# Tavish9/freegaussian

Hardware: AMD Instinct MI355X
Metric: Mpixels/s fwd+bwd @ 1M Gaussians 1080p (higher is better)
Workload: dtype f32; 1 GPU; north-star cfg4: 1000000 Gaussians, 1920x1080, SH degree 3, 1 view per rank per step, view = (rank + step) mod 8 around the 8-view ring, fwd+bwd, RGB, absgrad; layout=uniform, N=1000000, P=2073600, parallelism=view-dp1

## Files before the change

freegaussian_amd/_lib.py:

```python
from __future__ import annotations

import ctypes
import os
from ctypes import c_char_p, c_double, c_float, c_int, c_int64, c_size_t, c_void_p

_HERE = os.path.dirname(os.path.abspath(__file__))
LIB_PATH = os.path.join(_HERE, "libfgraster.so")

P = c_void_p

SIGNATURES = {
    "fg_abi_version": (c_int, []),
    "fg_error_string": (c_char_p, [c_int]),
    "fg_project_fwd": (c_int, [c_int, P, P, P, P, P, c_int, c_int, c_float, c_float, c_float, c_float, c_int,
                               P, P, P, P, P, P, P]),
    "fg_project_bwd": (c_int, [c_int, P, P, P, P, P, c_int, c_int, c_float, P, P, P, P, P, P, P, P, P, P, P]),
    "fg_sh_fwd": (c_int, [c_int, c_int, c_int, P, P, P, P, P, P]),
    "fg_sh_bwd": (c_int, [c_int, c_int, c_int, P, P, P, P, P, P, P, P, P]),
    "fg_scan_workspace_bytes": (c_size_t, [c_int]),
    "fg_scan_tiles": (c_int, [c_int, P, P, P, c_size_t, P]),
    "fg_tile_bin": (c_int, [c_int, P, P, P, P, c_int, c_int, c_int, P, P, P]),
    "fg_sort_workspace_bytes": (c_size_t, [c_int64]),
    "fg_sort_pairs": (c_int, [c_int64, P, P, c_int, P, c_size_t, P]),
    "fg_tile_ranges": (c_int, [c_int64, P, c_int, P, P]),
    "fg_sort32_workspace_bytes": (c_size_t, [c_int64]),
    "fg_sort_pairs32": (c_int, [c_int64, P, P, c_int, P, c_size_t, P]),
    "fg_bin_prepare_workspace_bytes": (c_size_t, [c_int]),
    "fg_bin_prepare": (c_int, [c_int, P, P, P, P, P, P, c_size_t, P]),
    "fg_bin_prepare_rects": (c_int, [c_int, P, P, P, c_int, c_int, c_int, P, P, P, P, c_size_t, P]),
    "fg_bin_prepare_keys": (c_int, [c_int, P, P, P, P, P, P, P, c_size_t, P]),
    "fg_bin_emit_workspace_bytes": (c_size_t, [c_int64]),
    "fg_bin_emit_sort": (c_int, [c_int, c_int64, P, P, P, P, P, c_int, c_int, c_int, P, P, P, P, c_size_t, P]),
    "fg_bin_emit_sort_capacity": (c_int, [c_int, c_int64, P, P, P, P, P, c_int, c_int, c_int, P, P, P, P, c_size_t,
                                          P]),
    "fg_stbin_supported": (c_int, [c_int, c_int, c_int]),
    "fg_stbin_count_workspace_bytes": (c_size_t, [c_int, c_int, c_int]),
    "fg_stbin_count": (c_int, [c_int, P, P, c_int, c_int, P, P, P, c_size_t, P]),
    "fg_stbin_fill_workspace_bytes": (c_size_t, [c_int64]),
    "fg_stbin_fill": (c_int, [c_int, P, P, P, c_int, c_int, c_int64, P, P, P, P, P, c_size_t, c_int, P]),
    "fg_stbin_fill_jobs": (c_int, [c_int, P, P, P, c_int, c_int, c_int64, P, P, P, P, P, c_size_t, c_int, c_int, c_int, P, P,
                                   c_int, P, c_int, P, P]),
    "fg_isect_keys": (c_int, [c_int64, P, P, P, P, P]),
    "fg_densify_stats": (c_int, [c_int, P, P, c_float, P, P, P, P]),
    "fg_adam_step_multi": (c_int, [c_int, P, P]),
    "fg_adam_step": (c_int, [c_int64, P, P, P, P, c_double, c_double, c_double, c_double, c_int64, P]),
    "fg_l1_ssim_workspace_floats": (c_size_t, [c_int, c_int, c_int]),
    "fg_l1_ssim_fwd": (c_int, [c_int, c_int, c_int, P, P, P, P, c_size_t, P, P]),
    "fg_l1_ssim_bwd": (c_int, [c_int, c_int, c_int, P, P, P, P, P, P]),
    "fg_pack_splats": (c_int, [c_int, c_int, P, P, P, P, P, P]),
    "fg_raster_config_init": (None, [P]),
    "fg_raster_fwd": (c_int, [c_int, c_int, c_int, c_int, P, P, P, P, P, P, P, P]),
    "fg_raster_bwd": (c_int, [c_int, c_int, c_int, c_int, P, P, P, P, P, P, P, P, P, P]),
    "fg_raster_composite_fwd": (c_int, [c_int, c_int, c_int, c_int, P, P, P, P, c_int, P, P, P, P, P, P]),
    "fg_raster_composite_bwd": (c_int, [c_int, c_int, c_int, c_int, P, P, P, P, c_int, P, P, P, P, P, P, P, P]),
    "fg_raster_jobs_words": (c_int64, [c_int, c_int, c_int, P]),
    "fg_raster_build_jobs": (c_int, [c_int, c_int, c_int, P, P, P, c_int, P, P]),
    "fg_raster_jobs_fwd": (c_int, [c_int, c_int, c_int, c_int, P, P, P, P, P, c_int, P, P, P, P, P, P, P, c_int64, P, P, P]),
    "fg_raster_seg_ckpt_floats": (c_int64, [c_int, c_int, c_int, c_int, c_int64, P]),
    "fg_raster_jobs_bwd": (c_int, [c_int, c_int, c_int, c_int, P, P, P, P, P, c_int, P, P, P, P, P, P, P, P, P, P, P]),
    "fg_unpack_grads": (c_int, [c_int, c_int, P, P, P, P, P, P, P]),
    "fg_preprocess_fwd": (c_int, [c_int, P, P, P, P, P, c_int, c_int, c_int, c_int, P, c_int, P, P, c_int, c_int,
                                  c_float, c_float, c_float, c_float, c_int, c_int, P, P, P, P, P, P, P, P, P, P, P, P]),
    "fg_viewmat_bwd_workspace_bytes": (c_size_t, [c_int]),
    "fg_viewmat_bwd": (c_int, [c_int, c_int, P, P, P, P, P, P, P, P, c_int, c_int, c_int, c_int, c_int, P, P, c_int, c_int,
                               c_float, c_int, P, P, P, c_int, P, P, P, P, P, c_size_t, P]),
    "fg_sh_pack_fwd": (c_int, [c_int, P, P, P, c_int, c_int, c_int, c_int, P, c_int, P, c_int, P, P, P, P, P, P, P]),
    "fg_preprocess_bwd": (c_int, [c_int, P, P, P, P, P, c_int, c_int, c_int, c_int, c_int, P, P, c_int, c_int,
                                  c_float, c_int, P, P, P, c_int, P, P, P, P, P, P, P, P, P, P]),
    "fg_preprocess_raw_fwd": (c_int, [c_int, P, P, P, P, P, P, P, P, c_int, c_int, c_int, P, c_int, P, P, c_int,
                                      c_int, c_float, c_float, c_float, c_float, c_int, c_int, P, P, P, P, P, P, P,
                                      P, P, P, P, P]),
    "fg_preprocess_raw_bwd": (c_int, [c_int, P, P, P, P, P, P, P, P, c_int, c_int, c_int, c_int, P, P, c_int, c_int,
                                      c_float, c_int, P, P, P, c_int, P, P, P, P, P, P, P, P, P, P, P, P, P]),
    "fg_preprocess_bwd_factored": (c_int, [c_int, P, P, P, P, P, c_int, c_int, c_int, c_int, P, P, c_int, c_int,
                                           c_float, c_int, P, P, P, c_int, P, P, P, P, P, P, P, c_int, P, P, P]),
    "fg_sh_grad_accumulate": (c_int, [c_int, c_int, c_int, c_int, P, P, c_int64, c_int, c_float, P, P]),
    "fg_payload_compact": (c_int, [c_int, c_int, P, P, c_int64, P, P]),
    "fg_payload_expand": (c_int, [c_int, c_int, c_int, P, c_int64, c_int64, P, c_int64, P]),
    "fg_step_layout_query": (c_int, [P, P, P]),
    "fg_step_fwd": (c_int, [P, P, P, P, P, P, P]),
    "fg_step_bwd": (c_int, [P, P, P, P, P, P]),
    "fg_sh_grad_accumulate_split": (c_int, [c_int, c_int, c_int, c_int, P, P, c_int64, c_int, c_float, P, P, P]),
    "fg_preprocess_raw_bwd_factored": (c_int, [c_int, P, P, P, P, P, P, P, P, c_int, c_int, c_int, c_int, P, P, c_int, c_int,
                                               c_float, c_int, P, P, P, c_int, P, P, P, P, P, P, P, P, P, c_int, P, P, P]),
    "fg_densify_flags": (c_int, [c_int, c_int, c_float, c_float, c_float, c_float, c_float, c_float, c_float, P, P, P,
                                 P, P, P, P]),
    "fg_densify_map": (c_int, [c_int, P, P, P, P, P, c_int, c_int, c_int, c_int, P, P, P]),
    "fg_gather_rows": (c_int, [c_int64, c_int, P, P, c_int64, P, P]),
    "fg_split_children": (c_int, [c_int, c_int, P, P, P, P, P, P]),
    "fg_mask_backproject": (c_int, [c_int, P, P, P, P, c_int, c_int, P, P, c_int, c_int, P, P]),
    "fg_camera_flow": (c_int, [c_int, c_int, P, P, P, P, P, P]),
    "fg_reprojection_flow": (c_int, [c_int, c_int, P, P, P, P, c_float, P, P]),
    "fg_flow_fwd": (c_int, [c_int, P, P, P, P, P, P, P, P, P, P]),
    "fg_flow_bwd": (c_int, [c_int, P, P, P, P, P, P, P, P, P, P, P, P, P]),
    "fg_knn_workspace_bytes": (c_size_t, [c_int64]),
    "fg_knn": (c_int, [c_int64, P, c_int, P, P, P, c_size_t, P]),
}

_EXTRA = {"fg_debug_wave_reduce16": (c_int, [P, P, P]), "fg_debug_knn_grid": (c_int, [c_int64, P, c_int, P, P])}

ABI_VERSION = 10
KNN_MAX_K = 8
STBIN_LONG_SEGMENTS = 1
STBIN_TEST_SMALL_SLABS = 4
STEP_NO_FOOTPRINT_MASKS = 2
SH_JAC_FLOATS = 10
_lib = None


class FgRasterError(RuntimeError):
    pass


class RasterConfig(ctypes.Structure):

    _fields_ = [(n, ctypes.c_int32) for n in (
        "size", "ppt_fwd", "ppt_bwd", "tile_order", "bands_nx", "tail4_fwd", "tail2_fwd", "tail4_bwd", "tail2_bwd",
        "split4_fwd", "split2_fwd", "split4_bwd", "split2_bwd", "use_liveness", "seg_parts", "seg_tail", "seg_parts2",
        "seg_tail2", "debug_only_xcd", "debug_k_mod", "balance_bands", "heavy_tiles", "seg_slots", "prio_fwd", "prio_bwd",
        "heavy_wide", "seg_fine")]

    FIELDS = tuple(n for n, _ in _fields_)[1:]

    @classmethod
    def defaults(cls) -> "RasterConfig":
        cfg = cls()
        load().fg_raster_config_init(ctypes.byref(cfg))
        return cfg

    def ptr(self) -> int:
        return ctypes.addressof(self)


STEP_BUFFERS = ("radii", "means2d", "depths", "conics", "comp", "tiles", "splats", "depth_keys", "tile_rects", "tile_masks", "sh_jac",
                "tile_offsets", "list_offsets", "flatten_ids", "jobs", "live", "seg_ckpt", "v_splats", "render", "alphas",
                "last_ids", "clamp_mask", "count_ws", "fill_ws")
STEP_BUFFER = {n: i for i, n in enumerate(STEP_BUFFERS)}


class StepDesc(ctypes.Structure):

    _fields_ = [(n, ctypes.c_int32) for n in (
        "size", "N", "width", "height", "tile_size", "raw", "sh_degree", "k_stored", "n_color", "with_depth", "n_extra",
        "antialiased", "n_clamp", "want_backward", "list_shares", "flags")] + [
        (n, ctypes.c_float) for n in ("eps2d", "near_plane", "far_plane", "radius_clip")] + [("capacity", ctypes.c_int64)]


class StepIO(ctypes.Structure):

    _fields_ = [(n, ctypes.c_void_p) for n in (
        "means", "quats", "d_quats", "scales", "d_scales", "opacities", "colors", "features_rest", "extra", "viewmat", "K",
        "background", "count_out", "v_render", "v_alphas", "v_depths", "v_conics", "v_means", "v_quats", "v_d_quats",
        "v_scales", "v_d_scales", "v_opacities", "v_colors", "v_features_rest", "v_extra", "v_rgb")] + [
        ("v_rgb_floats", ctypes.c_int32), ("ev_raster_begin", ctypes.c_void_p), ("ev_raster_end", ctypes.c_void_p),
        ("ckpt_need_out", ctypes.c_void_p)]


class StepLayout(ctypes.Structure):

    _fields_ = [("keep_bytes", ctypes.c_int64), ("tmp_bytes", ctypes.c_int64),
                ("offset", ctypes.c_int64 * len(STEP_BUFFERS)), ("nbytes", ctypes.c_int64 * len(STEP_BUFFERS)),
                ("jobs_words", ctypes.c_int64), ("seg_ckpt_floats", ctypes.c_int64), ("channels", ctypes.c_int32)]


def load() -> ctypes.CDLL:
    global _lib
    if _lib is not None:
        return _lib
    if not os.path.exists(LIB_PATH):
        raise FgRasterError(
            f"{LIB_PATH} is missing: build it with `python -c 'import __graft_entry__ as g; g.build()'` "
            "or `make -C freegaussian_amd/csrc`.  There is no CPU fallback."
        )
    lib = ctypes.CDLL(os.environ.get("FG_RASTER_LIB", LIB_PATH))
    for name, (res, args) in {**SIGNATURES, **_EXTRA}.items():
        fn = getattr(lib, name)
        fn.restype = res
        fn.argtypes = args
    if lib.fg_abi_version() != ABI_VERSION:
        raise FgRasterError(f"ABI mismatch: library {lib.fg_abi_version()} vs binding {ABI_VERSION}")
    _lib = lib
    return lib


def check(code: int, what: str) -> None:
    if code != 0:
        msg = load().fg_error_string(code).decode()
        raise FgRasterError(f"{what} failed: {msg} ({code})")
```

freegaussian_amd/csrc/stbin.hip:

```cpp
#include <atomic>

#include "fg_common.h"
#include "jobs_build.h"

namespace {

constexpr int SB_BLOCK = 256;
constexpr int SB_CHUNK = 4096;
constexpr int SC_BLOCK = 1024, SC_WAVES = SC_BLOCK / 64, SC_PER = SB_CHUNK / SC_BLOCK;
__host__ __device__ __forceinline__ int chunk_rounds(int N) { return N <= 320 * 1024 ? 1 : (N <= 640 * 1024 ? 2 : SC_PER); }
#ifndef FG_SB_SMALL_WAVES
#define FG_SB_SMALL_WAVES 8
#endif
#ifndef FG_SB_SMALL_KPT
#define FG_SB_SMALL_KPT 6
#endif
constexpr int SB_SMALL_WAVES = FG_SB_SMALL_WAVES, SB_LARGE_WAVES = 16;
constexpr int SB_SMALL_KPT = FG_SB_SMALL_KPT, SB_LARGE_KPT = 8;
constexpr int SB_LARGE_GRID = 512;
constexpr int SB_SMALL_BUCKET_BITS = 11, SB_LARGE_BUCKET_BITS = 12;
constexpr int SB_MAX_LDS_WORDS = 12288;
constexpr int SB_SCATTER_LDS_BYTES = 124 * 1024;
constexpr int SB_MIN_STAGE = 4096;
#ifndef FG_SB_SKEW_MAX
#define FG_SB_SKEW_MAX 96
#endif
constexpr int SB_SKEW_MAX = FG_SB_SKEW_MAX;
constexpr int SB_LONG_MIN = 64 * 16 * 8 - 256;
#ifndef FG_SB_LONG_SPLIT
#define FG_SB_LONG_SPLIT 3072
#endif
constexpr int SB_LONG_SPLIT = FG_SB_LONG_SPLIT;
static_assert(SB_LONG_SPLIT <= SB_LONG_MIN && SB_LONG_SPLIT >= 2 * 1536, "long segments: at least two buckets, at most the large sort's capacity");
constexpr int LG_T = 1536;
constexpr int LG_KMAX = 1008;
constexpr int LG_SA = 32;
constexpr int LG_BLOCK = 512, LG_PER = 8, LG_CHUNK = LG_BLOCK * LG_PER;
constexpr int LG_GRID = 1024, LG_SORT_GRID = 1024;
constexpr int SB_LONG_OVER_GRID = 64;
constexpr int SB_LONG_SLAB = SB_LONG_SPLIT;
__host__ __device__ __forceinline__ int long_buckets(int n) {
  const int k = (n + LG_T - 1) / LG_T;
  return k > LG_KMAX ? LG_KMAX : (k < 2 ? 2 : k);
}
__host__ __device__ __forceinline__ int long_samples(int k, int cap) {
  const int s = LG_SA * k;
  return s > cap ? cap : s;
}
struct LongTables {
  uint64_t* split;
  uint32_t* cnt;
  uint32_t* cursor;
  uint4* tcnt;
  int4* chunk_seg;
  int4* bucket_seg;
  int32_t* over_list;
  int over_cap;
  uint64_t* arena;
};
__device__ __forceinline__ int n_slots_cap(const LongTables& lt) { return lt.over_cap; }

struct Geo {
  int tile_w, tile_h, sw, sh;
};
__host__ __device__ __forceinline__ Geo geo_of(int tile_w, int tile_h) {
  Geo g;
  g.tile_w = tile_w;
  g.tile_h = tile_h;
  g.sw = (tile_w + 1) >> 1;
  g.sh = (tile_h + 1) >> 1;
  return g;
}
__host__ __device__ __forceinline__ int count_band_rows(const Geo& g) {
  const int per = 2 * (g.tile_w + 1) + (g.sw + 1), fixed = (g.tile_w + 1) + (g.sw + 1);
  const int rows = (SB_MAX_LDS_WORDS - fixed) / per;
  return rows < g.sh ? (rows > 0 ? rows : 0) : g.sh;
}
__host__ __device__ __forceinline__ int scatter_band_rows(const Geo& g) {
  const int rows = SB_MAX_LDS_WORDS / g.sw;
  return rows < g.sh ? rows : g.sh;
}

__device__ __forceinline__ uint32_t wave_incl_scan(uint32_t v, int lane) {
#pragma unroll
  for (int d = 1; d < 64; d <<= 1) {
    const uint32_t o = __shfl_up(v, d);
    if (lane >= d) v += o;
  }
  return v;
}

__device__ __forceinline__ void marks_to_counts(int32_t* gt, int ntr, int tile_w, uint32_t* __restrict__ out_t,
                                                int32_t* gs, int nsr, int sw, uint32_t* __restrict__ out_s,
                                                bool rowwise = false) {
  const int lane = fg::lane_id(), wave = threadIdx.x >> 6;
  for (int r = wave; r < ntr + nsr; r += SC_WAVES) {
    const bool tiles = r < ntr;
    int32_t* row = tiles ? gt + r * (tile_w + 1) : gs + (r - ntr) * (sw + 1);
    const int cols = tiles ? tile_w : sw;
    int carry = 0;
    for (int x = 0; x < cols; x += 64) {
      const int v = x + lane < cols ? row[x + lane] : 0;
      const int incl = (int)wave_incl_scan((uint32_t)v, lane) + carry;
      if (x + lane < cols) row[x + lane] = incl;
      carry = __builtin_amdgcn_readlane(incl, 63);
    }
  }
  __syncthreads();
  for (int c = threadIdx.x; c < tile_w + sw; c += SC_BLOCK) {
    const bool tiles = c < tile_w;
    const int x = tiles ? c : c - tile_w, cols = tiles ? tile_w : sw, rows = tiles ? ntr : nsr;
    const int32_t* col = (tiles ? gt : gs) + x;
    uint32_t* out = (tiles ? out_t : out_s) + x;
    int run = 0, row = 0;
    if (rowwise) {
      for (; row + 4 <= rows; row += 4) {
        int v[4];
#pragma unroll
        for (int k = 0; k < 4; ++k) v[k] = col[(row + k) * (cols + 1)];
#pragma unroll
        for (int k = 0; k < 4; ++k) out[(size_t)(row + k) * cols] = (uint32_t)v[k];
      }
      for (; row < rows; ++row) out[(size_t)row * cols] = (uint32_t)col[row * (cols + 1)];
      continue;
    }
    for (; row + 4 <= rows; row += 4) {
      int v[4];
#pragma unroll
      for (int k = 0; k < 4; ++k) v[k] = col[(row + k) * (cols + 1)];
#pragma unroll
      for (int k = 0; k < 4; ++k) {
        run += v[k];
        out[(size_t)(row + k) * cols] = (uint32_t)run;
      }
    }
    for (; row < rows; ++row) {
      run += col[row * (cols + 1)];
      out[(size_t)row * cols] = (uint32_t)run;
    }
  }
}

template <typename F>
__device__ __forceinline__ void for_bit_runs(uint32_t bits, F f) {
  bits &= 0xFFu;
  if (bits == 0u) return;
  {
    const int s = __builtin_ctz(bits), e = 32 - __builtin_clz(bits);
    if (bits == (((1u << (e - s)) - 1u) << s)) {
      f(s, e);
      return;
    }
  }
  while (bits) {
    const int s = __builtin_ctz(bits);
    const int len = __builtin_ctz(~(bits >> s));
    f(s, s + len);
    bits &= ~(((1u << len) - 1u) << s);
  }
}
__global__ void __launch_bounds__(SC_BLOCK)
sb_count_kernel(int N, int per, const int2* __restrict__ rects, const unsigned long long* __restrict__ masks, int tile_w,
                int tile_h, int band_rows, uint32_t* __restrict__ table_t, uint32_t* __restrict__ table_s,
                unsigned long long* __restrict__ area_part) {
  extern __shared__ int32_t s_grid[];
  __shared__ int4 s_cq[SC_WAVES][64];
  __shared__ uint32_t s_cqx[SC_WAVES][64];
  __shared__ unsigned long long s_cmarks[SC_WAVES];
  const Geo g = geo_of(tile_w, tile_h);
  const int chunk = blockIdx.x;
  const int gwt = tile_w + 1, gws = g.sw + 1;
  const int T = tile_w * tile_h, S = g.sw * g.sh;
  const int lane = fg::lane_id(), wave = threadIdx.x >> 6;
  const int chunk_n = per * SC_BLOCK;
  const int g0 = masks ? chunk * chunk_n + wave * (chunk_n / SC_WAVES) + lane : chunk * chunk_n + (int)threadIdx.x;
  const int gstep = masks ? 64 : SC_BLOCK;
  int2 rc[SC_PER];
  unsigned long long mk[SC_PER];
#pragma unroll
  for (int r = 0; r < SC_PER; ++r) {
    const bool in = r < per && g0 + r * gstep < N;
    rc[r] = in ? rects[g0 + r * gstep] : make_int2(0, 0);
    mk[r] = in && masks ? masks[g0 + r * gstep] : 0ull;
  }
  const uint64_t lt_mask = (lane == 0) ? 0ull : (~0ull >> (64 - lane));
  {
    __shared__ unsigned long long s_area[SC_WAVES];
    unsigned long long area = 0;
#pragma unroll
    for (int r = 0; r < SC_PER; ++r) area += (unsigned long long)((rc[r].y & 0xFFFF) * (rc[r].y >> 16));
#pragma unroll
    for (int m = 1; m < 64; m <<= 1) area += __shfl_xor(area, m);
    if (lane == 0) s_area[wave] = area;
    __syncthreads();
    if (threadIdx.x == 0) {
      unsigned long long all = 0;
#pragma unroll
      for (int w = 0; w < SC_WAVES; ++w) all += s_area[w];
      area_part[chunk] = all;
    }
  }
  for (int sr0 = 0; sr0 < g.sh; sr0 += band_rows) {
    const int sr1 = min(sr0 + band_rows, g.sh), tr0 = 2 * sr0, tr1 = min(2 * sr1, tile_h);
    const int ntr = tr1 - tr0, nsr = sr1 - sr0;
    int32_t* gt = s_grid;
    int32_t* gs = s_grid + (ntr + 1) * gwt;
    for (int i = threadIdx.x; i < (ntr + 1) * gwt + (nsr + 1) * gws; i += SC_BLOCK) s_grid[i] = 0;
    __syncthreads();
    if (masks) {
      int4* q = s_cq[wave];
      uint32_t* qx = s_cqx[wave];
      unsigned long long* marks = &s_cmarks[wave];
#pragma unroll
      for (int r = 0; r < SC_PER; ++r) {
        if (r >= per) break;
        const int w = rc[r].y & 0xFFFF, h = rc[r].y >> 16, y0 = rc[r].x >> 16;
        const int Ra = max(y0 >> 1, sr0), Rb = min(((y0 + h - 1) >> 1) + 1, sr1);
        const bool hit = w > 0 && h > 0 && Rb > Ra;
        const uint32_t cnt = hit ? (uint32_t)(Rb - Ra) : 0u;
        const uint32_t incl = wave_incl_scan(cnt, lane);
        const int total = (int)__builtin_amdgcn_readlane((int)incl, 63);
        const uint64_t hm = __ballot(hit);
        const int ci = __popcll(hm & lt_mask);
        if (hit) {
          q[ci] = make_int4(rc[r].x, rc[r].y, (int)(uint32_t)mk[r], (int)(uint32_t)(mk[r] >> 32));
          qx[ci] = ((incl - cnt) << 10) | (uint32_t)Ra;
        }
        __builtin_amdgcn_wave_barrier();
        for (int s0 = 0; s0 < total; s0 += 64) {
          if (lane == 0) *marks = 0ull;
          __builtin_amdgcn_wave_barrier();
          const int endpos = (int)incl - 1 - s0;
          if (hit && endpos >= 0 && endpos < 64) atomicOr(marks, 1ull << endpos);
          __builtin_amdgcn_wave_barrier();
          const uint64_t em = __hip_atomic_load(marks, __ATOMIC_RELAXED, __HIP_MEMORY_SCOPE_WAVEFRONT);
          const int before = __popcll(__ballot(hit && (int)incl <= s0));
          const int slot = s0 + lane;
          if (slot < total) {
            const int lo = before + __popcll(em & lt_mask);
            const int4 o = q[lo];
            const uint32_t ox = qx[lo];
            const unsigned long long m = ((unsigned long long)(uint32_t)o.w << 32) | (uint32_t)o.z;
            const int ow = o.y & 0xFFFF, oh = o.y >> 16, ox0 = o.x & 0xFFFF, oy0 = o.x >> 16;
            const int R = (int)(ox & 1023u) + (slot - (int)(ox >> 10));
            const int sh = 31 - __builtin_clz((unsigned)fg::footprint_block(ow, oh)), bs = 1 << sh;
            uint32_t both = 0;
#pragma unroll
            for (int i = 0; i < 2; ++i) {
              const int ty = 2 * R + i;
              if (ty < oy0 || ty >= oy0 + oh) continue;
              const uint32_t bits = (uint32_t)(m >> (8 * ((ty - oy0) >> sh))) & 0xFFu;
              both |= bits;
              for_bit_runs(bits, [&](int a0, int a1) {
                atomicAdd(&gt[(ty - tr0) * gwt + ox0 + a0 * bs], 1);
                atomicAdd(&gt[(ty - tr0) * gwt + min(ox0 + a1 * bs, ox0 + ow)], -1);
              });
            }
            for_bit_runs(both, [&](int a0, int a1) {
              atomicAdd(&gs[(R - sr0) * gws + ((ox0 + a0 * bs) >> 1)], 1);
              atomicAdd(&gs[(R - sr0) * gws + ((min(ox0 + a1 * bs, ox0 + ow) - 1) >> 1) + 1], -1);
            });
          }
        }
        __builtin_amdgcn_wave_barrier();
      }
    } else {
#pragma unroll
      for (int r = 0; r < SC_PER; ++r) {
        const int w = rc[r].y & 0xFFFF, h = rc[r].y >> 16, x0 = rc[r].x & 0xFFFF, y0 = rc[r].x >> 16;
        const int ya = max(y0, tr0), yb = min(y0 + h, tr1);
        if (w > 0 && yb > ya) {
          const int ra = ya - tr0, rb = yb - tr0;
          atomicAdd(&gt[ra * gwt + x0], 1);
          atomicAdd(&gt[ra * gwt + x0 + w], -1);
          atomicAdd(&gt[rb * gwt + x0], -1);
          atomicAdd(&gt[rb * gwt + x0 + w], 1);
          const int sxa = x0 >> 1, sxb = ((x0 + w - 1) >> 1) + 1;
          const int sya = (ya >> 1) - sr0, syb = ((yb - 1) >> 1) + 1 - sr0;
          atomicAdd(&gs[sya * gws + sxa], 1);
          atomicAdd(&gs[sya * gws + sxb], -1);
          atomicAdd(&gs[syb * gws + sxa], -1);
          atomicAdd(&gs[syb * gws + sxb], 1);
        }
      }
    }
    __syncthreads();
    marks_to_counts(gt, ntr, tile_w, table_t + (size_t)chunk * T + tr0 * tile_w, gs, nsr, g.sw,
                    table_s + (size_t)chunk * S + sr0 * g.sw, masks != nullptr);
    __syncthreads();
  }
}

constexpr int SC_COLS = 16, SC_SLICES = SB_BLOCK / SC_COLS;
__global__ void __launch_bounds__(SB_BLOCK)
sb_columns_kernel(int T, int S, int n_chunks, int wg_t, const uint32_t* __restrict__ table_t,
                  uint32_t* __restrict__ table_s, int32_t* __restrict__ tile_offsets, int32_t* __restrict__ st_offsets) {
  __shared__ uint32_t part[SC_SLICES][SC_COLS];
  const bool tiles = (int)blockIdx.x < wg_t;
  const int n = tiles ? T : S;
  const int cl = threadIdx.x % SC_COLS, qd = threadIdx.x / SC_COLS;
  const int col = ((int)blockIdx.x - (tiles ? 0 : wg_t)) * SC_COLS + cl;
  const int cq = (n_chunks + SC_SLICES - 1) / SC_SLICES, c0 = min(qd * cq, n_chunks), c1 = min(c0 + cq, n_chunks);
  const uint32_t* src = tiles ? table_t : table_s;
  constexpr int U = 16;
  uint32_t v[U], s = 0;
  const bool small = c1 - c0 <= U;
  if (col < n) {
    if (small) {
#pragma unroll
      for (int u = 0; u < U; ++u) v[u] = c0 + u < c1 ? src[(size_t)(c0 + u) * n + col] : 0u;
#pragma unroll
      for (int u = 0; u < U; ++u) s += v[u];
    } else {
      for (int c = c0; c < c1; ++c) s += src[(size_t)c * n + col];
    }
  }
  part[qd][cl] = s;
  __syncthreads();
  uint32_t run = 0, total = 0;
#pragma unroll
  for (int k = 0; k < SC_SLICES; ++k) {
    const uint32_t p = part[k][cl];
    if (k < qd) run += p;
    total += p;
  }
  if (col >= n) return;
  if (tiles) {
    if (qd == 0) tile_offsets[col + 1] = (int32_t)total;
    return;
  }
  if (small) {
#pragma unroll
    for (int u = 0; u < U; ++u) {
      if (c0 + u < c1) table_s[(size_t)(c0 + u) * n + col] = run;
      run += v[u];
    }
  } else {
    for (int c = c0; c < c1; ++c) {
      const uint32_t x = table_s[(size_t)c * n + col];
      table_s[(size_t)c * n + col] = run;
      run += x;
    }
  }
  if (qd == 0) st_offsets[col + 1] = (int32_t)total;
}

constexpr int SO_BLOCK = 1024, SO_WAVES = SO_BLOCK / 64, SO_PER = 8;
__device__ __forceinline__ uint64_t scan_counts_in_place(int n, int32_t* __restrict__ offs, uint32_t* buf,
                                                         uint32_t* wave_tot, uint32_t* largest = nullptr,
                                                         uint32_t over_thr = 0xFFFFFFFFu, uint32_t* n_over = nullptr) {
  const int lane = fg::lane_id(), wave = threadIdx.x >> 6;
  uint32_t carry = 0, big = 0, over = 0;
  uint64_t total = 0;
  for (int base = 0; base < n; base += SO_BLOCK * SO_PER) {
    uint32_t in[SO_PER];
#pragma unroll
    for (int k = 0; k < SO_PER; ++k) {
      const int i = base + k * SO_BLOCK + threadIdx.x;
      in[k] = i < n ? (uint32_t)offs[i + 1] : 0u;
    }
#pragma unroll
    for (int k = 0; k < SO_PER; ++k) {
      buf[k * SO_BLOCK + threadIdx.x] = in[k];
      big = max(big, in[k]);
      over += in[k] > over_thr ? 1u : 0u;
    }
    __syncthreads();
    uint32_t v[SO_PER], sum = 0;
#pragma unroll
    for (int k = 0; k < SO_PER; k += 4) {
      const uint4 x = *reinterpret_cast<const uint4*>(&buf[threadIdx.x * SO_PER + k]);
      v[k] = x.x; v[k + 1] = x.y; v[k + 2] = x.z; v[k + 3] = x.w;
    }
#pragma unroll
    for (int k = 0; k < SO_PER; ++k) sum += v[k];
    const uint32_t incl = wave_incl_scan(sum, lane);
    if (lane == 63) wave_tot[wave] = incl;
    __syncthreads();
    uint32_t run = carry + incl - sum, all = 0;
#pragma unroll
    for (int k = 0; k < SO_WAVES; ++k) {
      const uint32_t t = wave_tot[k];
      if (k < wave) run += t;
      all += t;
    }
#pragma unroll
    for (int k = 0; k < SO_PER; ++k) {
      run += v[k];
      v[k] = run;
    }
#pragma unroll
    for (int k = 0; k < SO_PER; k += 4)
      *reinterpret_cast<uint4*>(&buf[threadIdx.x * SO_PER + k]) = make_uint4(v[k], v[k + 1], v[k + 2], v[k + 3]);
    __syncthreads();
#pragma unroll
    for (int k = 0; k < SO_PER; ++k) {
      const int i = base + k * SO_BLOCK + threadIdx.x;
      if (i < n) offs[i + 1] = (int32_t)buf[k * SO_BLOCK + threadIdx.x];
    }
    carry += all;
    total += all;
    __syncthreads();
  }
  if (threadIdx.x == 0) offs[0] = 0;
  if (largest) {
#pragma unroll
    for (int m = 1; m < 64; m <<= 1) big = max(big, (uint32_t)__shfl_xor((int)big, m));
    __syncthreads();
    if (lane == 0) wave_tot[wave] = big;
    __syncthreads();
#pragma unroll
    for (int k = 0; k < SO_WAVES; ++k) big = max(big, wave_tot[k]);
    *largest = big;
  }
  if (n_over) {
#pragma unroll
    for (int m = 1; m < 64; m <<= 1) over += (uint32_t)__shfl_xor((int)over, m);
    __syncthreads();
    if (lane == 0) wave_tot[wave] = over;
    __syncthreads();
    over = 0;
#pragma unroll
    for (int k = 0; k < SO_WAVES; ++k) over += wave_tot[k];
    *n_over = over;
  }
  return total;
}
__global__ void __launch_bounds__(SO_BLOCK)
sb_offsets_kernel(int T, int S, int32_t* __restrict__ tile_offsets, int32_t* __restrict__ st_offsets,
                  int64_t* __restrict__ count_out, const unsigned long long* __restrict__ area_part, int n_chunks) {
  __shared__ alignas(16) uint32_t buf[SO_BLOCK * SO_PER];
  __shared__ uint32_t wave_tot[SO_WAVES];
  if (blockIdx.x == 1) {
    uint32_t longest = 0, n_over = 0;
    scan_counts_in_place(S, st_offsets, buf, wave_tot, &longest, (uint32_t)SB_LONG_SPLIT, &n_over);
    if (count_out) {
      __shared__ unsigned long long s_sum[SO_WAVES];
      unsigned long long a = 0;
      for (int c = threadIdx.x; c < n_chunks; c += SO_BLOCK) a += area_part[c];
#pragma unroll
      for (int m = 1; m < 64; m <<= 1) a += __shfl_xor(a, m);
      if ((threadIdx.x & 63) == 0) s_sum[threadIdx.x >> 6] = a;
      __syncthreads();
      if (threadIdx.x == 0) {
        unsigned long long all = 0;
#pragma unroll
        for (int w = 0; w < SO_WAVES; ++w) all += s_sum[w];
        __hip_atomic_store(count_out + 14, (int64_t)all, __ATOMIC_RELAXED, __HIP_MEMORY_SCOPE_SYSTEM);
      }
    }
    if (threadIdx.x == 0 && count_out) {
      __hip_atomic_store(count_out + 3, (int64_t)n_over, __ATOMIC_RELAXED, __HIP_MEMORY_SCOPE_SYSTEM);
      __hip_atomic_store(count_out + 1, (int64_t)longest, __ATOMIC_RELAXED, __HIP_MEMORY_SCOPE_SYSTEM);
      __threadfence_system();
    }
    return;
  }
  uint32_t longest_tile = 0;
  const uint64_t total = scan_counts_in_place(T, tile_offsets, buf, wave_tot, &longest_tile);
  if (threadIdx.x == 0 && count_out) {
    __hip_atomic_store(count_out + 2, (int64_t)longest_tile, __ATOMIC_RELAXED, __HIP_MEMORY_SCOPE_SYSTEM);
    __hip_atomic_store(count_out, (int64_t)total, __ATOMIC_RELAXED, __HIP_MEMORY_SCOPE_SYSTEM);
    __threadfence_system();
  }
}

template <int NTH>
__device__ __forceinline__ void build_segment_lists(int S, const int32_t* __restrict__ st_offsets, int small_max,
                                                    int32_t* __restrict__ large_list, int4* __restrict__ long_list,
                                                    bool long_mode, int4* __restrict__ chunk_seg,
                                                    int4* __restrict__ bucket_seg, int32_t* __restrict__ over_list = nullptr) {
  constexpr int NWV = NTH / 64;
  __shared__ int s_large;
  if (long_mode && over_list && threadIdx.x == 0) over_list[0] = over_list[1] = 0;
  __shared__ uint32_t s_tot[3][NWV];
  const int lane = fg::lane_id(), wave = threadIdx.x >> 6;
  if (threadIdx.x == 0) s_large = 0;
  __syncthreads();
  const int per = (S + NTH - 1) / NTH, i0 = min((int)threadIdx.x * per, S), i1 = min(i0 + per, S);
  uint32_t mine[3] = {0, 0, 0};
  for (int i = i0; i < i1; ++i) {
    const int n = st_offsets[i + 1] - st_offsets[i];
    if (long_mode && n > SB_LONG_SPLIT) {
      mine[0] += 1;
      mine[1] += (uint32_t)((n + LG_CHUNK - 1) / LG_CHUNK);
      mine[2] += (uint32_t)long_buckets(n);
    } else if (n > small_max) {
      large_list[1 + atomicAdd(&s_large, 1)] = i;
    }
  }
  uint32_t incl[3];
#pragma unroll
  for (int f = 0; f < 3; ++f) {
    incl[f] = wave_incl_scan(mine[f], lane);
    if (lane == 63) s_tot[f][wave] = incl[f];
  }
  __syncthreads();
  if (threadIdx.x == 0) large_list[0] = s_large;
  if (!long_mode) {
    if (threadIdx.x == 0) long_list[0] = make_int4(0, 0, 0, 0);
    return;
  }
  uint32_t run[3], all[3];
#pragma unroll
  for (int f = 0; f < 3; ++f) {
    run[f] = incl[f] - mine[f];
    all[f] = 0;
#pragma unroll
    for (int w = 0; w < NWV; ++w) {
      const uint32_t t = s_tot[f][w];
      if (w < wave) run[f] += t;
      all[f] += t;
    }
  }
  for (int i = i0; i < i1; ++i) {
    const int n = st_offsets[i + 1] - st_offsets[i];
    if (n > SB_LONG_SPLIT) {
      long_list[1 + run[0]] = make_int4(i, (int)run[1], (int)run[2], n);
      const int nch = (n + LG_CHUNK - 1) / LG_CHUNK, nb = long_buckets(n);
      const int off = st_offsets[i];
      for (int c = 0; c < nch; ++c) chunk_seg[run[1] + c] = make_int4((int)run[2], off, n, c);
      for (int b = 0; b < nb; ++b) bucket_seg[run[2] + b] = make_int4((int)run[2], off, i, b);
      run[0] += 1;
      run[1] += (uint32_t)nch;
      run[2] += (uint32_t)nb;
    }
  }
  if (threadIdx.x == 0) {
    long_list[0] = make_int4((int)all[0], (int)all[1], (int)all[2], 0);
    long_list[1 + all[0]] = make_int4(-1, (int)all[1], (int)all[2], 0);
  }
}
template <bool STAGE>
__global__ void __launch_bounds__(SC_BLOCK)
sb_scatter_kernel(int N, int per, const int2* __restrict__ rects, const unsigned long long* __restrict__ masks,
                  const uint32_t* __restrict__ depth_keys, int tile_w,
                  int tile_h, int band_rows, int stage_cap, const uint32_t* __restrict__ table_s,
                  const int32_t* __restrict__ tile_offsets, const int32_t* __restrict__ st_offsets,
                  uint64_t* __restrict__ entries, long long capacity, int small_max, int32_t* __restrict__ large_list,
                  int4* __restrict__ long_list, int long_mode, int4* __restrict__ chunk_seg,
                  int4* __restrict__ bucket_seg, int job_blocks, fgjobs::JobBuild jb, int32_t* __restrict__ over_list) {
  if constexpr (STAGE) {
    const int first = (int)gridDim.x - 1 - job_blocks;
    if ((int)blockIdx.x == (int)gridDim.x - 1) {
      const Geo gg = geo_of(tile_w, tile_h);
      if ((long long)tile_offsets[tile_w * tile_h] <= capacity)
        build_segment_lists<SC_BLOCK>(gg.sw * gg.sh, st_offsets, small_max, large_list, long_list, long_mode != 0, chunk_seg,
                                      bucket_seg, over_list);
      return;
    }
    if ((int)blockIdx.x >= first) {
      extern __shared__ uint32_t s_dyn[];
      fgjobs::build_jobs_block<SC_BLOCK>((int)blockIdx.x - first, jb, tile_offsets, s_dyn);
      return;
    }
  }
  extern __shared__ uint32_t s_cur[];
  __shared__ uint32_t s_wave_tot[SC_WAVES];
  __shared__ int4 s_q[SC_WAVES][64];
  __shared__ unsigned long long s_qm[SC_WAVES][64];
  __shared__ int32_t s_excl[SC_WAVES][64];
  __shared__ unsigned long long s_marks[SC_WAVES];
  const Geo g = geo_of(tile_w, tile_h);
  const int chunk = blockIdx.x, S = g.sw * g.sh;
  if ((long long)tile_offsets[tile_w * tile_h] > capacity) return;
  const int lane = fg::lane_id(), wave = threadIdx.x >> 6;
  if constexpr (!STAGE) {
    if (chunk == 0)
      build_segment_lists<SC_BLOCK>(S, st_offsets, small_max, large_list, long_list, long_mode != 0, chunk_seg, bucket_seg,
                                    over_list);
  }
  const uint64_t lt_mask = (lane == 0) ? 0ull : (~0ull >> (64 - lane));
  int4* q = s_q[wave];
  unsigned long long* qm = s_qm[wave];
  int32_t* ex = s_excl[wave];
  unsigned long long* marks = &s_marks[wave];
  const int chunk_n = per * SC_BLOCK;
  const int g0 = chunk * chunk_n + wave * (chunk_n / SC_WAVES) + lane;
  int2 rc[SC_PER];
  uint32_t dk[SC_PER];
  unsigned long long mk[SC_PER];
#pragma unroll
  for (int r = 0; r < SC_PER; ++r) {
    const bool in = r < per && g0 + r * 64 < N;
    rc[r] = in ? rects[g0 + r * 64] : make_int2(0, 0);
    dk[r] = in ? depth_keys[g0 + r * 64] : 0u;
    mk[r] = in && masks ? masks[g0 + r * 64] : 0ull;
  }
  const int s_pad = (S + 1) & ~1;
  uint32_t* s_gd = s_cur + s_pad;
  uint64_t* stage = reinterpret_cast<uint64_t*>(s_gd + s_pad);
  uint16_t* stage_st = reinterpret_cast<uint16_t*>(stage + stage_cap);
  uint32_t chunk_pairs = 0;
  if (STAGE) {
    const uint32_t* row = table_s + (size_t)chunk * S;
    const bool last = (chunk + 1) * chunk_n >= N;
    auto count_of = [&](int i) {
      return (last ? (uint32_t)(st_offsets[i + 1] - st_offsets[i]) : row[S + i]) - row[i];
    };
    const int per = (S + SC_BLOCK - 1) / SC_BLOCK, i0 = min((int)threadIdx.x * per, S), i1 = min(i0 + per, S);
    uint32_t sum = 0;
    for (int i = i0; i < i1; ++i) sum += count_of(i);
    const uint32_t incl = wave_incl_scan(sum, lane);
    if (lane == 63) s_wave_tot[wave] = incl;
    __syncthreads();
    uint32_t base = incl - sum;
#pragma unroll
    for (int w = 0; w < SC_WAVES; ++w) {
      const uint32_t t = s_wave_tot[w];
      if (w < wave) base += t;
      chunk_pairs += t;
    }
    for (int i = i0; i < i1; ++i) {
      s_cur[i] = base;
      s_gd[i] = (uint32_t)st_offsets[i] + row[i] - base;
      base += count_of(i);
    }
  }
  for (int sr0 = 0; sr0 < g.sh; sr0 += band_rows) {
    const int sr1 = min(sr0 + band_rows, g.sh), tr0 = 2 * sr0, tr1 = min(2 * sr1, tile_h);
    const int sb0 = sr0 * g.sw, nbs = (sr1 - sr0) * g.sw;
    if (!STAGE) {
      const uint32_t* row = table_s + (size_t)chunk * S + sb0;
      for (int i = threadIdx.x; i < nbs; i += SC_BLOCK) s_cur[i] = (uint32_t)st_offsets[sb0 + i] + row[i];
    }
    __syncthreads();
#pragma unroll
    for (int r = 0; r < SC_PER; ++r) {
      if (r >= per) break;
      const int w = rc[r].y & 0xFFFF, h = rc[r].y >> 16, x0 = rc[r].x & 0xFFFF, y0 = rc[r].x >> 16;
      const int ya = max(y0, tr0), yb = min(y0 + h, tr1);
      const bool hit = w > 0 && yb > ya;
      const int sxa = x0 >> 1, snx = ((x0 + w - 1) >> 1) + 1 - sxa;
      const int sya = ya >> 1, sny = ((yb - 1) >> 1) + 1 - sya;
      const uint32_t cnt = hit ? (uint32_t)(snx * sny) : 0u;
      const uint32_t incl = wave_incl_scan(cnt, lane);
      const int total = (int)__builtin_amdgcn_readlane((int)incl, 63);
      const uint64_t hm = __ballot(hit);
      const int ci = __popcll(hm & lt_mask);
      if (hit) {
        q[ci] = make_int4(g0 + r * 64, (int)dk[r], rc[r].x, rc[r].y);
        if (masks) qm[ci] = mk[r];
        ex[ci] = (int)(incl - cnt);
      }
      __builtin_amdgcn_wave_barrier();
      for (int s0 = 0; s0 < total; s0 += 64) {
        if (lane == 0) *marks = 0ull;
        __builtin_amdgcn_wave_barrier();
        const int endpos = (int)incl - 1 - s0;
        if (hit && endpos >= 0 && endpos < 64) atomicOr(marks, 1ull << endpos);
        __builtin_amdgcn_wave_barrier();
        const uint64_t m = __hip_atomic_load(marks, __ATOMIC_RELAXED, __HIP_MEMORY_SCOPE_WAVEFRONT);
        const int before = __popcll(__ballot(hit && (int)incl <= s0));
        const int slot = s0 + lane;
        if (slot < total) {
          const int lo = before + __popcll(m & lt_mask);
          const int4 o = q[lo];
          const int t = slot - ex[lo];
          const int ow = o.w & 0xFFFF, oh = o.w >> 16, ox0 = o.z & 0xFFFF, oy0 = o.z >> 16;
          const int oxa = ox0 >> 1, onx = ((ox0 + ow - 1) >> 1) + 1 - oxa;
          const int oya = max(oy0, tr0) >> 1;
          int ty = (int)((float)t * __builtin_amdgcn_rcpf((float)onx));
          ty -= (ty * onx > t);
          ty += ((ty + 1) * onx <= t);
          const int tx = t - ty * onx;
          const int local = (oya + ty - sr0) * g.sw + oxa + tx;
          const int c0 = 2 * (oxa + tx), r0 = 2 * (oya + ty);
          const uint32_t cols = (uint32_t)(c0 >= ox0) | ((uint32_t)(c0 + 1 < ox0 + ow) << 1);
          const uint32_t rows = (uint32_t)(r0 >= oy0) | ((uint32_t)(r0 + 1 < oy0 + oh) << 1);
          uint32_t mask = ((rows & 1u) ? cols : 0u) | ((rows & 2u) ? cols << 2 : 0u);
          if (masks) {
            const unsigned long long om = qm[lo];
            const int sh = 31 - __builtin_clz((unsigned)fg::footprint_block(ow, oh));
            const int bx0 = ((c0 - ox0) >> sh) & 7, bx1 = ((c0 + 1 - ox0) >> sh) & 7;
            const int by0 = ((r0 - oy0) >> sh) & 7, by1 = ((r0 + 1 - oy0) >> sh) & 7;
            const uint32_t ra = (uint32_t)(om >> (8 * by0)), rb = (uint32_t)(om >> (8 * by1));
            mask &= ((ra >> bx0) & 1u) | (((ra >> bx1) & 1u) << 1) | (((rb >> bx0) & 1u) << 2) | (((rb >> bx1) & 1u) << 3);
          }
          if (mask != 0u) {
            const uint32_t pos = atomicAdd(&s_cur[local], 1u);
            const uint64_t element = ((uint64_t)(uint32_t)o.y << 32) | ((uint64_t)(uint32_t)o.x << 4) | mask;
            if (!STAGE) {
              entries[pos] = element;
            } else if (pos < (uint32_t)stage_cap) {
              stage[pos] = element;
              stage_st[pos] = (uint16_t)local;
            } else {
              entries[pos + s_gd[local]] = element;
            }
          }
        }
      }
      __builtin_amdgcn_wave_barrier();
    }
    __syncthreads();
  }
  if (STAGE) {
    const uint32_t n_staged = min(chunk_pairs, (uint32_t)stage_cap);
    for (uint32_t i = threadIdx.x; i < n_staged; i += SC_BLOCK) entries[i + s_gd[stage_st[i]]] = stage[i];
  }
}

__device__ __forceinline__ uint64_t same_digit_lanes(unsigned d, int nbits, bool in) {
  const uint64_t in_mask = __ballot(in);
  uint32_t lo = (uint32_t)in_mask, hi = (uint32_t)(in_mask >> 32);
  for (int bit = 0; bit < nbits; ++bit) {
    const int sel = (int)(d << (31 - bit)) >> 31;
    const uint64_t m = __ballot(sel != 0);
    lo = __builtin_amdgcn_bitop3_b32(lo, (uint32_t)m, (uint32_t)sel, 0x90);
    hi = __builtin_amdgcn_bitop3_b32(hi, (uint32_t)(m >> 32), (uint32_t)sel, 0x90);
  }
  return ((uint64_t)hi << 32) | lo;
}
template <int NW>
__device__ __forceinline__ void digit_starts(uint32_t (*wave_cnt)[256], uint32_t* scan_tmp) {
  const int lane = fg::lane_id(), wave = threadIdx.x >> 6;
  const bool own = threadIdx.x < 256;
  uint32_t c[NW], tot = 0, incl = 0;
  if (own) {
#pragma unroll
    for (int w = 0; w < NW; ++w) {
      c[w] = wave_cnt[w][threadIdx.x];
      tot += c[w];
    }
    incl = wave_incl_scan(tot, lane);
    if (lane == 63) scan_tmp[wave] = incl;
  }
  __syncthreads();
  if (own) {
    uint32_t run = incl - tot;
#pragma unroll
    for (int w = 0; w < 4; ++w)
      if (w < wave) run += scan_tmp[w];
#pragma unroll
    for (int w = 0; w < NW; ++w) {
      wave_cnt[w][threadIdx.x] = run;
      run += c[w];
    }
  }
  __syncthreads();
}
template <int NW>
__device__ __forceinline__ void block_min_max(uint32_t lo, uint32_t hi, uint32_t* red, uint32_t& kmin, uint32_t& kmax) {
#pragma unroll
  for (int m = 1; m < 64; m <<= 1) {
    lo = min(lo, (uint32_t)__shfl_xor((int)lo, m));
    hi = max(hi, (uint32_t)__shfl_xor((int)hi, m));
  }
  const int wave = threadIdx.x >> 6;
  if (fg::lane_id() == 0) {
    red[wave] = lo;
    red[NW + wave] = hi;
  }
  __syncthreads();
  kmin = red[0];
  kmax = red[NW];
#pragma unroll
  for (int w = 1; w < NW; ++w) {
    kmin = min(kmin, red[w]);
    kmax = max(kmax, red[NW + w]);
  }
  __syncthreads();
}
template <typename Ptr>
__device__ __forceinline__ int run_position(Ptr cur, int n, int i, uint64_t e, uint32_t kmin, int low) {
  const uint32_t key = ((uint32_t)(e >> 32) - kmin) >> low;
  const bool left = i > 0 && (((uint32_t)(cur[i - 1] >> 32) - kmin) >> low) == key;
// ... 216 lines not shown
#pragma unroll
    for (int k = 0; k < PER; ++k) {
      const uint32_t x = c[k];
      c[k] = run;
      run += x;
    }
    if constexpr (PER >= 4) {
#pragma unroll
      for (int k = 0; k < PER; k += 4) *reinterpret_cast<uint4*>(&sh.bucket[gt * PER + k]) = make_uint4(c[k], c[k + 1], c[k + 2], c[k + 3]);
    } else {
#pragma unroll
      for (int k = 0; k < PER; ++k) sh.bucket[gt * PER + k] = c[k];
    }
    if (gt == NT - 1) sh.bucket[NB] = run;
    __syncthreads();
    return mx;
  };
  const uint32_t fullest = scan_buckets();
  if (!SKEW && defer_skew && fullest > SB_SKEW_MAX) return true;
  if (SKEW && fullest > SB_SKEW_MAX) {
    using Sh = SortShared<NW, KPT, BB>;
    const int ns = min(Sh::NSP, n >> 2);
    SB_FOR_ROUNDS(q)
      if ((valid >> q) & 1u) sh.img[ibase + q * 64] = e[q];
    if constexpr (PER >= 4) {
#pragma unroll
      for (int k = 0; k < PER; k += 4) *reinterpret_cast<uint4*>(&sh.bucket[gt * PER + k]) = make_uint4(0, 0, 0, 0);
    } else {
#pragma unroll
      for (int k = 0; k < PER; ++k) sh.bucket[gt * PER + k] = 0;
    }
    __syncthreads();
    uint64_t x = 0;
    if (gt < ns) {
      x = sh.img[(gt * n) / ns];
      sh.sp[gt] = x;
    }
    __syncthreads();
    int smaller = 0;
    if (gt < ns)
      for (int u = 0; u < ns; ++u) smaller += sh.sp[u] < x;
    __syncthreads();
    if (gt < ns) sh.sp[smaller] = x;
    __syncthreads();
    SB_FOR_ROUNDS(q) {
      uint32_t b = 0;
#pragma unroll
      for (int step = 64; step >= 1; step >>= 1) {
        const uint32_t t = b + (uint32_t)step;
        const uint64_t v = sh.sp[min(t, (uint32_t)ns) - 1];
        b = (t <= (uint32_t)ns && v <= e[q]) ? t : b;
      }
      bk[q] = b;
      if ((valid >> q) & 1u) rk[q] = atomicAdd(&sh.bucket[b], 1u);
    }
    __syncthreads();
    (void)scan_buckets();
  }
  SB_FOR_ROUNDS(q)
    if ((valid >> q) & 1u) sh.img[sh.bucket[bk[q]] + rk[q]] = e[q];
  __syncthreads();
  int pos[KPT];
#pragma unroll
  for (int q = 0; q < KPT; ++q) pos[q] = -1;
  SB_FOR_ROUNDS(q) {
    if ((valid >> q) & 1u) {
      const int s0 = (int)sh.bucket[bk[q]], s1 = (int)sh.bucket[bk[q] + 1];
      if (s1 - s0 > 1) {
        int smaller = 0;
        for (int j = s0; j < s1; ++j) smaller += sh.img[j] < e[q];
        pos[q] = s0 + smaller;
      }
    }
  }
  __syncthreads();
  SB_FOR_ROUNDS(q)
    if (pos[q] >= 0) sh.img[pos[q]] = e[q];
  __syncthreads();
  if constexpr (!EMIT) return false;
  uint32_t idm[KPT], ranks[KPT];
  uint32_t pre[KPT][4], c[4] = {0, 0, 0, 0};
#pragma unroll
  for (int q = 0; q < KPT; ++q) idm[q] = 0;
  SB_FOR_ROUNDS(q)
    if ((valid >> q) & 1u) idm[q] = (uint32_t)sh.img[ibase + q * 64];
  SB_FOR_ROUNDS(q) {
    ranks[q] = 0;
#pragma unroll
    for (int j = 0; j < 4; ++j) {
      const uint64_t bal = __ballot((idm[q] >> j) & 1u);
      ranks[q] |= (uint32_t)__popcll(bal & lt_mask) << (8 * j);
      pre[q][j] = c[j];
      c[j] += (uint32_t)__popcll(bal);
    }
  }
  if (lane == 0) *reinterpret_cast<uint4*>(sh.tcnt[gw]) = make_uint4(c[0], c[1], c[2], c[3]);
  __syncthreads();
  uint32_t base[4];
  {
    uint4 t = make_uint4(0, 0, 0, 0);
    if (lane < gw) t = *reinterpret_cast<const uint4*>(sh.tcnt[lane]);
    uint32_t v[4] = {t.x, t.y, t.z, t.w};
#pragma unroll
    for (int j = 0; j < 4; ++j) {
#pragma unroll
      for (int m = 1; m < (NW > 1 ? NW : 2); m <<= 1) v[j] += (uint32_t)__shfl_xor((int)v[j], m);
      base[j] = (uint32_t)tile_base[j] + (uint32_t)__builtin_amdgcn_readfirstlane((int)v[j]);
    }
  }
  SB_FOR_ROUNDS(q) {
    const uint32_t id = idm[q] >> 4;
#pragma unroll
    for (int j = 0; j < 4; ++j)
      if ((idm[q] >> j) & 1u) flatten_ids[base[j] + pre[q][j] + ((ranks[q] >> (8 * j)) & 0xFFu)] = (int32_t)id;
  }
  return false;
}
#undef SB_FOR_ROUNDS

__device__ __forceinline__ void supertile_tile_bases(int st, int tile_w, int tile_h, const int32_t* __restrict__ tile_offsets,
                                                     int (&tile_base)[4], int (&tile_id)[4]) {
  const Geo g = geo_of(tile_w, tile_h);
  const int sy = st / g.sw, sx = st - sy * g.sw;
#pragma unroll
  for (int j = 0; j < 4; ++j) {
    const int tx = 2 * sx + (j & 1), ty = 2 * sy + (j >> 1);
    const bool inside = tx < tile_w && ty < tile_h;
    tile_id[j] = inside ? ty * tile_w + tx : -1;
    tile_base[j] = inside ? tile_offsets[tile_id[j]] : 0;
  }
}

template <int NW, int KPT, int BB, bool SMALL>
__device__ __forceinline__ bool sort_supertile(SortShared<NW, KPT, BB>& sh, int st, int tile_w, int tile_h,
                                               const int32_t* __restrict__ tile_offsets,
                                               const int32_t* __restrict__ st_offsets, uint64_t* __restrict__ entries,
                                               uint64_t* __restrict__ scratch, bool over, int total,
                                               int32_t* __restrict__ flatten_ids, int32_t* __restrict__ list_offsets,
                                               bool defer_skew = false) {
  constexpr int MAXN = SortShared<NW, KPT, BB>::MAXN;
  uint32_t(*wave_cnt)[256] = reinterpret_cast<uint32_t(*)[256]>(sh.bucket);
  static_assert((1 << BB) >= NW * 256, "the fallback's counters live in the bucket array");
  const int T = tile_w * tile_h;
  int tile_base[4], tile_id[4];
  supertile_tile_bases(st, tile_w, tile_h, tile_offsets, tile_base, tile_id);
#pragma unroll
  for (int j = 0; j < 4; ++j) {
    if (SMALL && tile_id[j] >= 0 && threadIdx.x == 0) {
      list_offsets[tile_id[j]] = over ? 0 : tile_base[j];
      if (tile_id[j] == T - 1) list_offsets[T] = over ? 0 : total;
    }
  }
  const int off = st_offsets[st], n = st_offsets[st + 1] - off;
  if (over || n <= 0) return false;
  if (SMALL && n > MAXN) return false;
  if constexpr (!SMALL) {
    if (n > MAXN) {
      const uint64_t* fin = sort_segment_global<NW>(entries + off, scratch + off, n, wave_cnt, sh.scan_tmp, sh.red);
      emit_tiles<NW>(fin, n, tile_base, flatten_ids, sh.tcnt);
      return false;
    }
  }
  const uint64_t* __restrict__ src = entries + off;
  return sort_emit_lds<NW, KPT, BB, true, !SMALL>(sh, (int)threadIdx.x, [src](int i) { return src[i]; }, n, tile_base,
                                                  flatten_ids, defer_skew);
}

__global__ void __launch_bounds__(1024)
sb_build_jobs_kernel(fgjobs::JobBuild jb, const int32_t* __restrict__ tile_offsets) {
  __shared__ uint32_t s_rows[fgjobs::FG_BAND_MAX_ROWS];
  fgjobs::build_jobs_block<1024>((int)blockIdx.x, jb, tile_offsets, s_rows);
}

template <int NW, int KPT, int BB>
__device__ __forceinline__ void sample_long_segment(SortShared<NW, KPT, BB>& sh, const uint64_t* __restrict__ src, int n,
                                                    int bucket_base, const LongTables& lt) {
  constexpr int NT = 64 * NW;
  const int k = long_buckets(n), s = long_samples(k, SortShared<NW, KPT, BB>::MAXN);
  const uint64_t step = ((uint64_t)n << 16) / (uint64_t)s;
  sort_emit_lds<NW, KPT, BB, false>(sh, (int)threadIdx.x, [src, step](int i) { return src[((uint64_t)i * step) >> 16]; }, s,
                                    nullptr, nullptr);
  for (int t = threadIdx.x; t < k; t += NT) {
    if (t + 1 < k) lt.split[bucket_base + t] = sh.img[(int)(((long long)(t + 1) * s) / k)];
    lt.cnt[bucket_base + t] = 0u;
    lt.cursor[bucket_base + t] = 0u;
    lt.tcnt[bucket_base + t] = make_uint4(0, 0, 0, 0);
  }
  __syncthreads();
}

__global__ void __launch_bounds__(64 * SB_LARGE_WAVES)
sb_sort_large_kernel(int tile_w, int tile_h, const int32_t* __restrict__ tile_offsets,
                     const int32_t* __restrict__ st_offsets, const int32_t* __restrict__ large_list,
                     const int4* __restrict__ long_list, LongTables lt, uint64_t* __restrict__ entries,
                     uint64_t* __restrict__ scratch, long long capacity, int32_t* __restrict__ flatten_ids) {
  __shared__ SortShared<SB_LARGE_WAVES, SB_LARGE_KPT, SB_LARGE_BUCKET_BITS> sh;
  static_assert(SortShared<SB_LARGE_WAVES, SB_LARGE_KPT, SB_LARGE_BUCKET_BITS>::MAXN == SB_LONG_MIN, "long = beyond this launch's LDS sort");
  constexpr int job_blocks = 0;
  const int total = tile_offsets[tile_w * tile_h];
  if ((long long)total > capacity) return;
  const int n_long = long_list[0].x, count = large_list[0];
  for (int k = (int)blockIdx.x - job_blocks; k < n_long + count; k += (int)gridDim.x - job_blocks) {
    if (k < n_long) {
      const int4 ls = long_list[1 + k];
      sample_long_segment(sh, entries + st_offsets[ls.x], ls.w, ls.z, lt);
    } else {
      sort_supertile<SB_LARGE_WAVES, SB_LARGE_KPT, SB_LARGE_BUCKET_BITS, false>(
          sh, large_list[1 + k - n_long], tile_w, tile_h, tile_offsets, st_offsets, entries, scratch, false, total,
          flatten_ids, nullptr);
    }
    __syncthreads();
  }
}

__device__ __forceinline__ int long_bucket_of(const uint64_t* s_split, int k, uint64_t e) {
  int b = 0;
#pragma unroll
  for (int step = 512; step >= 1; step >>= 1) {
    const int t = b + step;
    const uint64_t v = s_split[min(t, k - 1) - 1];
    b = (t <= k - 1 && v <= e) ? t : b;
  }
  return b;
}
static_assert(LG_KMAX <= 1024, "long_bucket_of bisects 10 levels");

static_assert(LG_CHUNK < 65536, "16-bit per-chunk tile counters");

__global__ void __launch_bounds__(LG_BLOCK)
sb_long_scatter_kernel(const int32_t* __restrict__ tile_offsets, int n_tiles, long long capacity,
                       const int32_t* __restrict__ st_offsets, const int4* __restrict__ long_list,
                       const uint64_t* __restrict__ entries, uint64_t* __restrict__ scratch, LongTables lt, int slab_limit) {
  __shared__ uint64_t s_split[LG_KMAX];
  __shared__ uint32_t s_hist[LG_KMAX], s_base[LG_KMAX];
  __shared__ unsigned long long s_tc[LG_KMAX];
  if ((long long)tile_offsets[n_tiles] > capacity) return;
  const int4 hdr = long_list[0];
  int cur = -1;
  for (int w = blockIdx.x; w < hdr.y; w += gridDim.x) {
    const int4 ci = lt.chunk_seg[w];
    const int slot0 = ci.x, n = ci.z, k = long_buckets(n), c = ci.w;
    const uint64_t* __restrict__ src = entries + ci.y;
    if (slot0 != cur) {
      __syncthreads();
      for (int t = threadIdx.x; t < k - 1; t += LG_BLOCK) s_split[t] = lt.split[slot0 + t];
      cur = slot0;
    }
    for (int t = threadIdx.x; t < k; t += LG_BLOCK) {
      s_hist[t] = 0u;
      s_tc[t] = 0ull;
    }
    __syncthreads();
    uint64_t e[LG_PER];
    int bk[LG_PER];
    uint32_t rk[LG_PER];
#pragma unroll
    for (int q = 0; q < LG_PER; ++q) {
      const int i = c * LG_CHUNK + q * LG_BLOCK + (int)threadIdx.x;
      e[q] = src[min(i, n - 1)];
    }
#pragma unroll
    for (int q = 0; q < LG_PER; ++q) {
      const int i = c * LG_CHUNK + q * LG_BLOCK + (int)threadIdx.x;
      bk[q] = -1;
      rk[q] = 0u;
      if (i < n) {
        bk[q] = long_bucket_of(s_split, k, e[q]);
        rk[q] = atomicAdd(&s_hist[bk[q]], 1u);
        const uint32_t m = (uint32_t)e[q] & 15u;
        atomicAdd(&s_tc[bk[q]], (unsigned long long)(m & 1u) | ((unsigned long long)((m >> 1) & 1u) << 16) |
                                    ((unsigned long long)((m >> 2) & 1u) << 32) | ((unsigned long long)((m >> 3) & 1u) << 48));
      }
    }
    __syncthreads();
    for (int t = threadIdx.x; t < k; t += LG_BLOCK) {
      const uint32_t h = s_hist[t];
      if (h) {
        s_base[t] = atomicAdd(&lt.cursor[slot0 + t], h);
        const unsigned long long tc = s_tc[t];
        uint32_t* tg = reinterpret_cast<uint32_t*>(&lt.tcnt[slot0 + t]);
#pragma unroll
        for (int j = 0; j < 4; ++j) {
          const uint32_t v = (uint32_t)(tc >> (16 * j)) & 0xFFFFu;
          if (v) atomicAdd(&tg[j], v);
        }
      }
    }
    __syncthreads();
#pragma unroll
    for (int q = 0; q < LG_PER; ++q)
      if (bk[q] >= 0) {
        const uint32_t pos = s_base[bk[q]] + rk[q];
        if (pos < (uint32_t)slab_limit) scratch[(size_t)(slot0 + bk[q]) * SB_LONG_SLAB + pos] = e[q];
      }
    __syncthreads();
  }
}

__global__ void __launch_bounds__(64 * SB_SMALL_WAVES)
sb_sort_small_kernel(int tile_w, int tile_h, const int32_t* __restrict__ tile_offsets,
                     const int32_t* __restrict__ st_offsets, uint64_t* __restrict__ entries,
                     uint64_t* __restrict__ scratch, long long capacity, int32_t* __restrict__ flatten_ids,
                     int32_t* __restrict__ list_offsets, int32_t* __restrict__ over_list, int job_blocks,
                     fgjobs::JobBuild jb, const int4* __restrict__ long_list, LongTables lt) {
  __shared__ SortShared<SB_SMALL_WAVES, SB_SMALL_KPT, SB_SMALL_BUCKET_BITS> sh;
  if ((int)blockIdx.x < job_blocks) {
    static_assert(sizeof(sh.img) >= fgjobs::FG_BAND_MAX_ROWS * sizeof(uint32_t), "row sums in the element buffer");
    fgjobs::build_jobs_block<64 * SB_SMALL_WAVES>((int)blockIdx.x + 8, jb, tile_offsets, reinterpret_cast<uint32_t*>(sh.img));
    return;
  }
  const int st = (int)blockIdx.x - job_blocks;
  if (st >= ((tile_w + 1) >> 1) * ((tile_h + 1) >> 1)) return;
  const int total = tile_offsets[tile_w * tile_h];
  const bool skewed = sort_supertile<SB_SMALL_WAVES, SB_SMALL_KPT, SB_SMALL_BUCKET_BITS, true>(
      sh, st, tile_w, tile_h, tile_offsets, st_offsets, entries, scratch, (long long)total > capacity, total, flatten_ids,
      list_offsets, over_list != nullptr);
  if (skewed && threadIdx.x == 0) over_list[2 + atomicAdd(over_list, 1)] = -(st + 1);
  if (over_list && (long long)total <= capacity) {
    using Sh = SortShared<SB_SMALL_WAVES, SB_SMALL_KPT, SB_SMALL_BUCKET_BITS>;
    static_assert(Sh::MAXN == SB_LONG_SPLIT, "in long mode no segment is left for the large launch");
    const int n = st_offsets[st + 1] - st_offsets[st];
    if (n > Sh::MAXN) {
      __shared__ int s_long;
      if (threadIdx.x == 0) s_long = -1;
      __syncthreads();
      const int n_long = long_list[0].x;
      for (int t = threadIdx.x; t < n_long; t += 64 * SB_SMALL_WAVES)
        if (long_list[1 + t].x == st) s_long = t;
      __syncthreads();
      if (s_long >= 0) {
        const int4 ls = long_list[1 + s_long];
        sample_long_segment(sh, entries + st_offsets[st], ls.w, ls.z, lt);
      }
    }
  }
}

__global__ void __launch_bounds__(64 * SB_SMALL_WAVES) __attribute__((amdgpu_waves_per_eu(8, 8)))
sb_long_sort_kernel(int tile_w, int tile_h, long long capacity, const int32_t* __restrict__ tile_offsets,
                    const int32_t* __restrict__ st_offsets, const int4* __restrict__ long_list, LongTables lt,
                    const uint64_t* __restrict__ entries, const uint64_t* __restrict__ scratch,
                    int32_t* __restrict__ flatten_ids, int slab_limit) {
  using Sh = SortShared<SB_SMALL_WAVES, SB_SMALL_KPT, SB_SMALL_BUCKET_BITS>;
  __shared__ Sh sh;
  __shared__ int s_tile_base[4];
  constexpr int NT = 64 * SB_SMALL_WAVES;
  static_assert(2 * LG_T <= Sh::MAXN && SB_LONG_SLAB == Sh::MAXN, "a bucket's slab is what the LDS sort takes: twice the target");
  if ((long long)tile_offsets[tile_w * tile_h] > capacity) return;
  const int lane = fg::lane_id(), wave = threadIdx.x >> 6;
  const int n_slots = long_list[0].z, n_items = n_slots + lt.over_list[0];
  for (int item = blockIdx.x; item < n_items; item += gridDim.x) {
    const uint64_t* src;
    int n, st;
    uint32_t pre[4] = {0, 0, 0, 0};
    if (item >= n_slots) {
      st = -lt.over_list[2 + item - n_slots] - 1;
      const int off = st_offsets[st];
      n = st_offsets[st + 1] - off;
      src = entries + off;
    } else {
      const int4 bi = lt.bucket_seg[item];
      st = bi.z;
      const int b = bi.w;
      for (int t = threadIdx.x; t < b; t += NT) {
        const uint4 tc = lt.tcnt[bi.x + t];
        pre[0] += tc.x; pre[1] += tc.y; pre[2] += tc.z; pre[3] += tc.w;
      }
#pragma unroll
      for (int f = 0; f < 4; ++f) {
#pragma unroll
        for (int m = 1; m < 64; m <<= 1) pre[f] += (uint32_t)__shfl_xor((int)pre[f], m);
        if (lane == 0) sh.bucket[f * SB_SMALL_WAVES + wave] = pre[f];
      }
      __syncthreads();
#pragma unroll
      for (int f = 0; f < 4; ++f) {
        pre[f] = 0;
#pragma unroll
        for (int w = 0; w < SB_SMALL_WAVES; ++w) pre[f] += sh.bucket[f * SB_SMALL_WAVES + w];
      }
      n = (int)lt.cursor[item];
      src = scratch + (size_t)item * SB_LONG_SLAB;
      if (n > slab_limit) {
        if (threadIdx.x == 0) lt.over_list[2 + n_slots_cap(lt) + atomicAdd(lt.over_list + 1, 1)] = item;
        n = 0;
      }
    }
    {
      int tile_base[4], tile_id[4];
      supertile_tile_bases(st, tile_w, tile_h, tile_offsets, tile_base, tile_id);
      __syncthreads();
      if (threadIdx.x < 4) s_tile_base[threadIdx.x] = tile_base[threadIdx.x] + (int)pre[threadIdx.x];
    }
    if (n > 0)
      sort_emit_lds<SB_SMALL_WAVES, SB_SMALL_KPT, SB_SMALL_BUCKET_BITS>(sh, (int)threadIdx.x, [src](int i) { return src[i]; }, n,
                                                                         s_tile_base, flatten_ids);
    __syncthreads();
  }
}

__global__ void __launch_bounds__(64 * SB_LARGE_WAVES)
sb_long_overflow_kernel(int tile_w, int tile_h, long long capacity, const int32_t* __restrict__ tile_offsets,
                        const int32_t* __restrict__ st_offsets, LongTables lt, uint64_t* __restrict__ entries,
                        uint64_t* __restrict__ scratch, int32_t* __restrict__ flatten_ids, int whole_limit) {
  using Sh = SortShared<SB_LARGE_WAVES, SB_LARGE_KPT, SB_LARGE_BUCKET_BITS>;
  __shared__ Sh sh;
  __shared__ int s_tile_base[4];
  __shared__ uint32_t s_n;
  __shared__ int s_mine;
  constexpr int NT = 64 * SB_LARGE_WAVES;
  if ((long long)tile_offsets[tile_w * tile_h] > capacity) return;
  const int lane = fg::lane_id(), wave = threadIdx.x >> 6;
  const int count = lt.over_list[1];
  uint32_t(*wave_cnt)[256] = reinterpret_cast<uint32_t(*)[256]>(sh.bucket);
  for (int v = blockIdx.x; v < count; v += gridDim.x) {
    const int slot = lt.over_list[2 + n_slots_cap(lt) + v];
    const int4 bi = lt.bucket_seg[slot];
    const int st = bi.z, b = bi.w, off = bi.y, n_seg = st_offsets[st + 1] - st_offsets[st], k = long_buckets(n_seg);
    const uint64_t lo = b > 0 ? lt.split[bi.x + b - 1] : 0ull, hi = b + 1 < k ? lt.split[bi.x + b] : ~0ull;
    uint64_t* tmp = lt.arena + (size_t)blockIdx.x * Sh::MAXN;
    int tile_base[4], tile_id[4];
    supertile_tile_bases(st, tile_w, tile_h, tile_offsets, tile_base, tile_id);
    const uint32_t limit = whole_limit >= 0 ? (uint32_t)whole_limit : (st & 1) ? (uint32_t)Sh::MAXN : (uint32_t)(LG_T + 192);
    int big = 0;
    for (int t = threadIdx.x; t < k; t += NT) big |= lt.cursor[bi.x + t] > limit ? 1 : 0;
    if (threadIdx.x == 0) s_n = 0u;
    const int whole = __syncthreads_or(big);
    if (whole) {
      if (threadIdx.x == 0) s_mine = atomicCAS(lt.cnt + bi.x, 0u, 0xFFFFFFFFu) == 0u ? 1 : 0;
      __syncthreads();
      if (s_mine) {
        const uint64_t* fin = sort_segment_global<SB_LARGE_WAVES>(entries + off, scratch + off, n_seg, wave_cnt,
                                                                   sh.scan_tmp, sh.red);
        emit_tiles<SB_LARGE_WAVES>(fin, n_seg, tile_base, flatten_ids, sh.tcnt);
      }
      __syncthreads();
      continue;
    }
    for (int i = threadIdx.x; i < n_seg; i += NT) {
      const uint64_t e = entries[(size_t)off + i];
      if (e >= lo && (b + 1 >= k || e < hi)) {
        const uint32_t pos = atomicAdd(&s_n, 1u);
        if (pos < (uint32_t)Sh::MAXN) tmp[pos] = e;
      }
    }
    __syncthreads();
    const int n_b = min((int)s_n, Sh::MAXN);
    uint32_t pre[4] = {0, 0, 0, 0};
    for (int t = threadIdx.x; t < b; t += NT) {
      const uint4 tc = lt.tcnt[bi.x + t];
      pre[0] += tc.x; pre[1] += tc.y; pre[2] += tc.z; pre[3] += tc.w;
    }
#pragma unroll
    for (int f = 0; f < 4; ++f) {
#pragma unroll
      for (int m = 1; m < 64; m <<= 1) pre[f] += (uint32_t)__shfl_xor((int)pre[f], m);
      if (lane == 0) sh.bucket[f * SB_LARGE_WAVES + wave] = pre[f];
    }
    __syncthreads();
#pragma unroll
    for (int f = 0; f < 4; ++f) {
      pre[f] = 0;
#pragma unroll
      for (int w = 0; w < SB_LARGE_WAVES; ++w) pre[f] += sh.bucket[f * SB_LARGE_WAVES + w];
    }
    __syncthreads();
    if (threadIdx.x < 4) s_tile_base[threadIdx.x] = tile_base[threadIdx.x] + (int)pre[threadIdx.x];
    const uint64_t* src = tmp;
    sort_emit_lds<SB_LARGE_WAVES, SB_LARGE_KPT, SB_LARGE_BUCKET_BITS>(sh, (int)threadIdx.x, [src](int i) { return src[i]; }, n_b,
                                                                       s_tile_base, flatten_ids);
    __syncthreads();
  }
}

size_t al256(size_t x) { return (x + 255) & ~(size_t)255; }
int n_chunks_of(int N) {
  const int c = chunk_rounds(N) * SC_BLOCK;
  return (N + c - 1) / c;
}

struct CountWs {
  uint32_t *table_t, *table_s;
  int32_t* st_offsets;
  int32_t* large_list;
  int4* long_list;
  unsigned long long* area_part;
  size_t bytes;
};
template <typename T>
T* ws_at(void* base, size_t offset) {
  return base ? reinterpret_cast<T*>(static_cast<char*>(base) + offset) : nullptr;
}
CountWs count_ws(void* base, int N, const Geo& g) {
  const size_t nc = (size_t)n_chunks_of(N > 0 ? N : 1), T = (size_t)g.tile_w * g.tile_h, S = (size_t)g.sw * g.sh;
  CountWs w;
  size_t o = 0;
  w.table_t = ws_at<uint32_t>(base, o);
  o += al256(nc * T * 4);
  w.table_s = ws_at<uint32_t>(base, o);
  o += al256(nc * S * 4);
  w.st_offsets = ws_at<int32_t>(base, o);
  o += al256((S + 1) * 4);
  w.large_list = ws_at<int32_t>(base, o);
  o += al256((S + 1) * 4);
  w.long_list = ws_at<int4>(base, o);
  o += al256((S + 2) * 16);
  w.area_part = ws_at<unsigned long long>(base, o);
  o += al256(nc * 8);
  w.bytes = o;
  return w;
}
size_t count_lds_bytes(const Geo& g) {
  const int nsr = count_band_rows(g);
  return ((size_t)(2 * nsr + 1) * (g.tile_w + 1) + (size_t)(nsr + 1) * (g.sw + 1)) * 4;
}

}

extern "C" int fg_stbin_supported(int N, int tile_w, int tile_h) {
  if (N < 0 || N >= (1 << 28) || tile_w <= 0 || tile_h <= 0 || tile_w > 1023 || tile_h > 1023) return 0;
  const Geo g = geo_of(tile_w, tile_h);
  return count_band_rows(g) > 0 && scatter_band_rows(g) > 0 ? 1 : 0;
}

extern "C" size_t fg_stbin_count_workspace_bytes(int N, int tile_w, int tile_h) {
  if (N < 0 || tile_w <= 0 || tile_h <= 0) return 0;
  return count_ws(nullptr, N, geo_of(tile_w, tile_h)).bytes;
}

extern "C" int fg_stbin_count(int N, const int32_t* tile_rects, const uint64_t* tile_masks, int tile_w, int tile_h,
                              int32_t* tile_offsets, int64_t* count_out, void* workspace, size_t workspace_bytes,
                              fg_stream_t stream) {
  if (N <= 0 || tile_w <= 0 || tile_h <= 0 || !tile_rects || !tile_offsets || !workspace) return FG_ERR_INVALID_ARG;
  if (!fg_stbin_supported(N, tile_w, tile_h)) return FG_ERR_UNSUPPORTED;
  const Geo g = geo_of(tile_w, tile_h);
  const CountWs w = count_ws(workspace, N, g);
  if (workspace_bytes < w.bytes) return FG_ERR_WORKSPACE;
  hipStream_t s = fg_hip_stream(stream);
  const int T = tile_w * tile_h, S = g.sw * g.sh, nc = n_chunks_of(N);
  hipLaunchKernelGGL(sb_count_kernel, dim3(nc), dim3(SC_BLOCK), count_lds_bytes(g), s, N, chunk_rounds(N),
                     reinterpret_cast<const int2*>(tile_rects), reinterpret_cast<const unsigned long long*>(tile_masks), tile_w,
                     tile_h, count_band_rows(g), w.table_t, w.table_s, w.area_part);
  const int wg_t = (T + SC_COLS - 1) / SC_COLS, wg_s = (S + SC_COLS - 1) / SC_COLS;
  hipLaunchKernelGGL(sb_columns_kernel, dim3(wg_t + wg_s), dim3(SB_BLOCK), 0, s, T, S, nc, wg_t, w.table_t, w.table_s,
                     tile_offsets, w.st_offsets);
  hipLaunchKernelGGL(sb_offsets_kernel, dim3(2), dim3(SO_BLOCK), 0, s, T, S, tile_offsets, w.st_offsets, count_out, w.area_part, nc);
  FG_RETURN_IF_LAUNCH_FAILED();
  return FG_OK;
}

namespace {
size_t long_buckets_max(size_t capacity) { return capacity / LG_T + capacity / SB_LONG_SPLIT + 2; }
struct FillWs {
  uint64_t *entries, *scratch;
  LongTables lt;
  size_t bytes;
};
FillWs fill_ws(void* base, size_t capacity) {
  const size_t kb = long_buckets_max(capacity);
  FillWs w;
  size_t o = 0;
  w.entries = ws_at<uint64_t>(base, o);
  o += al256(capacity * 8);
  w.scratch = ws_at<uint64_t>(base, o);
  o += al256((kb * (size_t)SB_LONG_SLAB > capacity ? kb * (size_t)SB_LONG_SLAB : capacity) * 8);
  w.lt.split = ws_at<uint64_t>(base, o);
  o += al256(kb * 8);
  w.lt.tcnt = ws_at<uint4>(base, o);
  o += al256(kb * 16);
  w.lt.cnt = ws_at<uint32_t>(base, o);
  o += al256(kb * 4);
  w.lt.cursor = ws_at<uint32_t>(base, o);
  o += al256(kb * 4);
  w.lt.bucket_seg = ws_at<int4>(base, o);
  o += al256(kb * 16);
  w.lt.over_cap = (int)(capacity / SB_SKEW_MAX + 2);
  w.lt.over_list = ws_at<int32_t>(base, o);
  o += al256((2 + (size_t)w.lt.over_cap + kb) * 4);
  w.lt.chunk_seg = ws_at<int4>(base, o);
  o += al256((capacity / LG_CHUNK + capacity / SB_LONG_SPLIT + 2) * 16);
  w.lt.arena = ws_at<uint64_t>(base, o);
  o += al256((size_t)SB_LONG_OVER_GRID * SB_LONG_MIN * 8);
  w.bytes = o;
  return w;
}
}

extern "C" size_t fg_stbin_fill_workspace_bytes(int64_t capacity) {
  return fill_ws(nullptr, (size_t)(capacity > 0 ? capacity : 1)).bytes;
}

namespace {

int stbin_fill(int N, const uint32_t* depth_keys, const int32_t* tile_rects, const uint64_t* tile_masks, int tile_w, int tile_h,
               int64_t capacity,
               const int32_t* tile_offsets, const void* count_workspace, int32_t* flatten_ids, int32_t* list_offsets,
               void* workspace, size_t workspace_bytes, const fgjobs::JobBuild* jobs, int flags, fg_stream_t stream) {
  if (N <= 0 || capacity <= 0 || tile_w <= 0 || tile_h <= 0) return FG_ERR_INVALID_ARG;
  if (!depth_keys || !tile_rects || !tile_offsets || !count_workspace || !flatten_ids || !list_offsets || !workspace)
    return FG_ERR_INVALID_ARG;
  if (flags & ~(FG_STBIN_LONG_SEGMENTS | FG_STBIN_TEST_SMALL_SLABS)) return FG_ERR_INVALID_ARG;
  if (!fg_stbin_supported(N, tile_w, tile_h)) return FG_ERR_UNSUPPORTED;
  if (workspace_bytes < fg_stbin_fill_workspace_bytes(capacity)) return FG_ERR_WORKSPACE;
  hipStream_t s = fg_hip_stream(stream);
  const Geo g = geo_of(tile_w, tile_h);
  const CountWs w = count_ws(const_cast<void*>(count_workspace), N, g);
  const FillWs fw = fill_ws(workspace, (size_t)capacity);
  const int nc = n_chunks_of(N);
  uint64_t* entries = fw.entries;
  uint64_t* scratch = fw.scratch;
  const int band_rows = scatter_band_rows(g), S = g.sw * g.sh, T = tile_w * tile_h;
  const int long_mode = (flags & FG_STBIN_LONG_SEGMENTS) ? 1 : 0;
  constexpr int small_max = SortShared<SB_SMALL_WAVES, SB_SMALL_KPT, SB_SMALL_BUCKET_BITS>::MAXN;
  const int s_pad = (S + 1) & ~1;
  int stage_cap = band_rows == g.sh && S <= 65535 ? ((int)SB_SCATTER_LDS_BYTES - 8 * s_pad) / 10 : 0;
  stage_cap = stage_cap >= SB_MIN_STAGE ? (stage_cap & ~63) : 0;
  bool want_jobs = jobs && (jobs->jobs_fwd || jobs->jobs_bwd), bwd_jobs_in_sort = false;
  if (stage_cap) {
    static std::atomic<uint64_t> attr_devices{0};
    int dev = 0;
    if (hipGetDevice(&dev) != hipSuccess || dev < 0 || dev >= 64) {
      stage_cap = 0;
    } else if (!((attr_devices.load(std::memory_order_relaxed) >> dev) & 1u)) {
      if (hipFuncSetAttribute(reinterpret_cast<const void*>(sb_scatter_kernel<true>),
                              hipFuncAttributeMaxDynamicSharedMemorySize, (int)SB_SCATTER_LDS_BYTES) == hipSuccess) {
        attr_devices.fetch_or(1ull << dev, std::memory_order_relaxed);
      } else {
        (void)hipGetLastError();
        stage_cap = 0;
      }
    }
  }
  if (stage_cap) {
    const size_t lds = (size_t)8 * s_pad + (size_t)10 * stage_cap;
    hipLaunchKernelGGL(sb_scatter_kernel<true>, dim3(nc + (want_jobs ? 8 : 0) + 1), dim3(SC_BLOCK), lds, s, N, chunk_rounds(N),
                       reinterpret_cast<const int2*>(tile_rects), reinterpret_cast<const unsigned long long*>(tile_masks),
                       depth_keys, tile_w, tile_h, band_rows, stage_cap, w.table_s,
                       tile_offsets, w.st_offsets, entries, (long long)capacity, small_max, w.large_list, w.long_list,
                       long_mode, fw.lt.chunk_seg, fw.lt.bucket_seg, want_jobs ? 8 : 0, want_jobs ? *jobs : fgjobs::JobBuild{},
                       fw.lt.over_list);
    want_jobs = false;
    bwd_jobs_in_sort = jobs && jobs->jobs_bwd;
  } else {
    hipLaunchKernelGGL(sb_scatter_kernel<false>, dim3(nc), dim3(SC_BLOCK), (size_t)band_rows * g.sw * 4, s, N, chunk_rounds(N),
                       reinterpret_cast<const int2*>(tile_rects), reinterpret_cast<const unsigned long long*>(tile_masks),
                       depth_keys, tile_w, tile_h, band_rows, 0, w.table_s,
                       tile_offsets, w.st_offsets, entries, (long long)capacity, small_max, w.large_list, w.long_list,
                       long_mode, fw.lt.chunk_seg, fw.lt.bucket_seg, 0, fgjobs::JobBuild{}, fw.lt.over_list);
  }
  if (want_jobs) hipLaunchKernelGGL(sb_build_jobs_kernel, dim3(fgjobs::FG_JOB_BLOCKS), dim3(1024), 0, s, *jobs, tile_offsets);
  if (!long_mode)
    hipLaunchKernelGGL(sb_sort_large_kernel, dim3(S < SB_LARGE_GRID ? S : SB_LARGE_GRID), dim3(64 * SB_LARGE_WAVES), 0, s,
                       tile_w, tile_h, tile_offsets, w.st_offsets, w.large_list, w.long_list, fw.lt, entries, scratch,
                       (long long)capacity, flatten_ids);
  hipLaunchKernelGGL(sb_sort_small_kernel, dim3(S + (bwd_jobs_in_sort ? 8 : 0)), dim3(64 * SB_SMALL_WAVES), 0, s, tile_w, tile_h,
                     tile_offsets, w.st_offsets, entries, scratch, (long long)capacity, flatten_ids, list_offsets,
                     long_mode ? fw.lt.over_list : nullptr, bwd_jobs_in_sort ? 8 : 0,
                     bwd_jobs_in_sort ? *jobs : fgjobs::JobBuild{}, w.long_list, fw.lt);
  const int slab_limit = (flags & FG_STBIN_TEST_SMALL_SLABS) ? LG_T + 64 : SB_LONG_SLAB;
  if (long_mode) {
    hipLaunchKernelGGL(sb_long_scatter_kernel, dim3(LG_GRID), dim3(LG_BLOCK), 0, s, tile_offsets, T, (long long)capacity,
                       w.st_offsets, w.long_list, entries, scratch, fw.lt, slab_limit);
    hipLaunchKernelGGL(sb_long_sort_kernel, dim3(LG_SORT_GRID), dim3(64 * SB_SMALL_WAVES), 0, s, tile_w, tile_h,
                       (long long)capacity, tile_offsets, w.st_offsets, w.long_list, fw.lt, entries, scratch, flatten_ids, slab_limit);
    hipLaunchKernelGGL(sb_long_overflow_kernel, dim3(SB_LONG_OVER_GRID), dim3(64 * SB_LARGE_WAVES), 0, s, tile_w, tile_h, (long long)capacity,
                       tile_offsets, w.st_offsets, fw.lt, entries, scratch, flatten_ids,
                       (flags & FG_STBIN_TEST_SMALL_SLABS) ? -1 : SortShared<SB_LARGE_WAVES, SB_LARGE_KPT, SB_LARGE_BUCKET_BITS>::MAXN);
  }
  FG_RETURN_IF_LAUNCH_FAILED();
  return FG_OK;
}

}

extern "C" int fg_stbin_fill(int N, const uint32_t* depth_keys, const int32_t* tile_rects, const uint64_t* tile_masks,
                             int tile_w, int tile_h,
                             int64_t capacity, const int32_t* tile_offsets, const void* count_workspace,
                             int32_t* flatten_ids, int32_t* list_offsets, void* workspace, size_t workspace_bytes,
                             int flags, fg_stream_t stream) {
  return stbin_fill(N, depth_keys, tile_rects, tile_masks, tile_w, tile_h, capacity, tile_offsets, count_workspace, flatten_ids,
                    list_offsets, workspace, workspace_bytes, nullptr, flags, stream);
}

extern "C" int fg_stbin_fill_jobs(int N, const uint32_t* depth_keys, const int32_t* tile_rects, const uint64_t* tile_masks,
                                  int tile_w, int tile_h, int64_t capacity, const int32_t* tile_offsets, const void* count_workspace,
                                  int32_t* flatten_ids, int32_t* list_offsets, void* workspace, size_t workspace_bytes,
                                  int width, int height, int tile_size, int32_t* jobs_fwd, int32_t* jobs_bwd,
                                  int bwd_list_shares, const fg_raster_config* config, int flags, int64_t* ckpt_need_out,
                                  fg_stream_t stream) {
  if (width <= 0 || height <= 0 || tile_size <= 0) return FG_ERR_INVALID_ARG;
  if ((width + tile_size - 1) / tile_size != tile_w || (height + tile_size - 1) / tile_size != tile_h)
    return FG_ERR_INVALID_ARG;
  fgjobs::JobBuild jb;
  const int rc = fgjobs::plan_jobs(width, height, tile_size, jobs_fwd, jobs_bwd, bwd_list_shares, config, &jb);
  if (rc != FG_OK) return rc;
  jb.need_out = reinterpret_cast<long long*>(ckpt_need_out);
  return stbin_fill(N, depth_keys, tile_rects, tile_masks, tile_w, tile_h, capacity, tile_offsets, count_workspace, flatten_ids,
                    list_offsets, workspace, workspace_bytes, &jb, flags, stream);
}
```

freegaussian_amd/csrc/step.hip:

```cpp
#include <string.h>

#include "fg_common.h"

namespace {

size_t al256(size_t x) { return (x + 255) & ~(size_t)255; }

int channels_of(const fg_step_desc& d) {
  const int ncol = d.sh_degree >= 0 ? 3 : d.n_color;
  return ncol + (d.with_depth ? 1 : 0) + d.n_extra;
}

bool desc_ok(const fg_step_desc* d) {
  if (!d || d->size < (int32_t)sizeof(fg_step_desc)) return false;
  if (d->N <= 0 || d->width <= 0 || d->height <= 0 || d->tile_size != 16 || d->capacity <= 0) return false;
  if (d->raw && d->sh_degree < 0) return false;
  const int c = channels_of(*d);
  return c >= 1 && c <= FG_MAX_CHANNELS && d->n_clamp >= 0 && d->n_clamp <= c;
}

template <typename T>
T* at(void* base, const fg_step_layout* L, int which) {
  return L->nbytes[which] > 0 ? reinterpret_cast<T*>(static_cast<char*>(base) + L->offset[which]) : nullptr;
}

}

extern "C" int fg_step_layout_query(const fg_step_desc* d, const fg_raster_config* config, fg_step_layout* out) {
  if (!desc_ok(d) || !out) return FG_ERR_INVALID_ARG;
  const int N = d->N, W = d->width, H = d->height;
  const int tile_w = (W + 15) / 16, tile_h = (H + 15) / 16, T = tile_w * tile_h, C = channels_of(*d);
  if (!fg_stbin_supported(N, tile_w, tile_h)) return FG_ERR_UNSUPPORTED;
  memset(out, 0, sizeof(*out));
  out->channels = C;
  out->jobs_words = fg_raster_jobs_words(W, H, 16, config);
  if (out->jobs_words <= 0) return FG_ERR_UNSUPPORTED;
  out->seg_ckpt_floats = d->want_backward && d->list_shares ? fg_raster_seg_ckpt_floats(C, W, H, 16, d->capacity, config) : 0;
  size_t n[FG_STEP_BUFFERS] = {0};
  n[FG_STEP_RADII] = (size_t)N * 4;
  n[FG_STEP_MEANS2D] = (size_t)N * 8;
  n[FG_STEP_DEPTHS] = (size_t)N * 4;
  n[FG_STEP_CONICS] = (size_t)N * 12;
  n[FG_STEP_COMP] = d->antialiased ? (size_t)N * 4 : 0;
  n[FG_STEP_TILES] = (size_t)N * 4;
  n[FG_STEP_SPLATS] = (size_t)N * FG_SPLAT_FLOATS * 4;
  n[FG_STEP_DEPTH_KEYS] = (size_t)N * 4;
  n[FG_STEP_TILE_RECTS] = (size_t)N * 8;
  n[FG_STEP_TILE_MASKS] = (d->flags & FG_STEP_NO_FOOTPRINT_MASKS) ? 0 : (size_t)N * 8;
  n[FG_STEP_SH_JAC] = d->sh_degree >= 1 && d->want_backward ? (size_t)N * FG_SH_JAC_FLOATS * 4 : 0;
  n[FG_STEP_TILE_OFFSETS] = (size_t)(T + 1) * 4;
  n[FG_STEP_LIST_OFFSETS] = (size_t)(T + 1) * 4;
  n[FG_STEP_FLATTEN_IDS] = (size_t)d->capacity * 4;
  n[FG_STEP_JOBS] = (size_t)out->jobs_words * 4 * 2;
  n[FG_STEP_LIVE] = d->want_backward ? (size_t)d->capacity * 4 : 0;
  n[FG_STEP_SEG_CKPT] = (size_t)out->seg_ckpt_floats * 4;
  n[FG_STEP_V_SPLATS] = d->want_backward ? (size_t)N * FG_SPLAT_FLOATS * 4 : 0;
  n[FG_STEP_RENDER] = (size_t)W * H * C * 4;
  n[FG_STEP_ALPHAS] = (size_t)W * H * 4;
  n[FG_STEP_LAST_IDS] = (size_t)W * H * 4;
  n[FG_STEP_CLAMP_MASK] = d->n_clamp > 0 ? (size_t)W * H : 0;
  size_t o = 0;
  for (int b = 0; b < FG_STEP_COUNT_WS; ++b) {
    out->offset[b] = (int64_t)o;
    out->nbytes[b] = (int64_t)n[b];
    o += al256(n[b]);
  }
  out->keep_bytes = (int64_t)(o ? o : 256);
  n[FG_STEP_COUNT_WS] = fg_stbin_count_workspace_bytes(N, tile_w, tile_h);
  n[FG_STEP_FILL_WS] = fg_stbin_fill_workspace_bytes(d->capacity);
  o = 0;
  for (int b = FG_STEP_COUNT_WS; b < FG_STEP_BUFFERS; ++b) {
    out->offset[b] = (int64_t)o;
    out->nbytes[b] = (int64_t)n[b];
    o += al256(n[b]);
  }
  out->tmp_bytes = (int64_t)o;
  return FG_OK;
}

extern "C" int fg_step_fwd(const fg_step_desc* d, const fg_raster_config* config, const fg_step_io* io, void* keep,
                           void* tmp, const fg_step_layout* L, fg_stream_t stream) {
  if (!desc_ok(d) || !io || !keep || !tmp || !L) return FG_ERR_INVALID_ARG;
  const int N = d->N, W = d->width, H = d->height, C = channels_of(*d);
  if (C != L->channels || L->keep_bytes <= 0) return FG_ERR_INVALID_ARG;
  const int tile_w = (W + 15) / 16, tile_h = (H + 15) / 16;
  int32_t* radii = at<int32_t>(keep, L, FG_STEP_RADII);
  float* means2d = at<float>(keep, L, FG_STEP_MEANS2D);
  float* depths = at<float>(keep, L, FG_STEP_DEPTHS);
  float* conics = at<float>(keep, L, FG_STEP_CONICS);
  float* comp = at<float>(keep, L, FG_STEP_COMP);
  int32_t* tiles = at<int32_t>(keep, L, FG_STEP_TILES);
  float* splats = at<float>(keep, L, FG_STEP_SPLATS);
  uint32_t* depth_keys = at<uint32_t>(keep, L, FG_STEP_DEPTH_KEYS);
  int32_t* tile_rects = at<int32_t>(keep, L, FG_STEP_TILE_RECTS);
  uint64_t* tile_masks = at<uint64_t>(keep, L, FG_STEP_TILE_MASKS);
  float* sh_jac = at<float>(keep, L, FG_STEP_SH_JAC);
  int rc;
  if (d->raw)
    rc = fg_preprocess_raw_fwd(N, io->means, io->quats, io->d_quats, io->scales, io->d_scales, io->opacities, io->colors,
                               io->features_rest, d->sh_degree, d->k_stored, d->with_depth, io->extra, d->n_extra, io->viewmat,
                               io->K, W, H, d->eps2d, d->near_plane, d->far_plane, d->radius_clip, 16, d->antialiased, radii,
                               means2d, depths, conics, comp, tiles, splats, depth_keys, tile_rects, tile_masks, sh_jac, stream);
  else
    rc = fg_preprocess_fwd(N, io->means, io->quats, io->scales, io->opacities, io->colors, d->sh_degree, d->k_stored,
                           d->n_color, d->with_depth, io->extra, d->n_extra, io->viewmat, io->K, W, H, d->eps2d, d->near_plane,
                           d->far_plane, d->radius_clip, 16, d->antialiased, radii, means2d, depths, conics, comp, tiles,
                           splats, depth_keys, tile_rects, tile_masks, sh_jac, stream);
  if (rc != FG_OK) return rc;
  int32_t* tile_offsets = at<int32_t>(keep, L, FG_STEP_TILE_OFFSETS);
  int32_t* list_offsets = at<int32_t>(keep, L, FG_STEP_LIST_OFFSETS);
  void* count_ws = at<char>(tmp, L, FG_STEP_COUNT_WS);
  rc = fg_stbin_count(N, tile_rects, tile_masks, tile_w, tile_h, tile_offsets, io->count_out, count_ws,
                      (size_t)L->nbytes[FG_STEP_COUNT_WS], stream);
  if (rc != FG_OK) return rc;
  int32_t* flatten_ids = at<int32_t>(keep, L, FG_STEP_FLATTEN_IDS);
  int32_t* jobs = at<int32_t>(keep, L, FG_STEP_JOBS);
  float* seg_ckpt = at<float>(keep, L, FG_STEP_SEG_CKPT);
  rc = fg_stbin_fill_jobs(N, depth_keys, tile_rects, tile_masks, tile_w, tile_h, d->capacity, tile_offsets, count_ws, flatten_ids,
                          list_offsets, at<char>(tmp, L, FG_STEP_FILL_WS), (size_t)L->nbytes[FG_STEP_FILL_WS], W, H, 16, jobs,
                          jobs + L->jobs_words, seg_ckpt != nullptr, config, d->flags & (FG_STBIN_LONG_SEGMENTS | FG_STBIN_TEST_SMALL_SLABS), io->ckpt_need_out,
                          stream);
  if (rc != FG_OK) return rc;
  float* v_splats = at<float>(keep, L, FG_STEP_V_SPLATS);
  if (io->ev_raster_begin && hipEventRecord(static_cast<hipEvent_t>(io->ev_raster_begin), fg_hip_stream(stream)) != hipSuccess)
    return FG_ERR_LAUNCH;
  rc = fg_raster_jobs_fwd(C, W, H, 16, splats, list_offsets, flatten_ids, jobs, io->background, d->n_clamp,
                          at<float>(keep, L, FG_STEP_RENDER), at<float>(keep, L, FG_STEP_ALPHAS),
                          at<int32_t>(keep, L, FG_STEP_LAST_IDS), at<uint8_t>(keep, L, FG_STEP_CLAMP_MASK), seg_ckpt,
                          at<uint32_t>(keep, L, FG_STEP_LIVE), v_splats, v_splats ? (int64_t)N * FG_SPLAT_FLOATS : 0,
                          io->ckpt_need_out ? io->ckpt_need_out + 9 : nullptr, config, stream);
  if (io->ev_raster_end && hipEventRecord(static_cast<hipEvent_t>(io->ev_raster_end), fg_hip_stream(stream)) != hipSuccess)
    return FG_ERR_LAUNCH;
  return rc;
}

extern "C" int fg_step_bwd(const fg_step_desc* d, const fg_raster_config* config, const fg_step_io* io, void* keep,
                           const fg_step_layout* L, fg_stream_t stream) {
  if (!desc_ok(d) || !io || !keep || !L || !d->want_backward) return FG_ERR_INVALID_ARG;
  if (!io->v_render || !io->v_means || !io->v_quats || !io->v_scales || !io->v_opacities) return FG_ERR_INVALID_ARG;
  const int N = d->N, W = d->width, H = d->height, C = channels_of(*d);
  float* v_splats = at<float>(keep, L, FG_STEP_V_SPLATS);
  const float* splats = at<float>(keep, L, FG_STEP_SPLATS);
  int32_t* jobs = at<int32_t>(keep, L, FG_STEP_JOBS);
  if (io->ev_raster_begin && hipEventRecord(static_cast<hipEvent_t>(io->ev_raster_begin), fg_hip_stream(stream)) != hipSuccess)
    return FG_ERR_LAUNCH;
  int rc = fg_raster_jobs_bwd(C, W, H, 16, splats, at<int32_t>(keep, L, FG_STEP_LIST_OFFSETS),
                              at<int32_t>(keep, L, FG_STEP_FLATTEN_IDS), jobs + L->jobs_words, io->background, d->n_clamp,
                              at<uint8_t>(keep, L, FG_STEP_CLAMP_MASK), at<float>(keep, L, FG_STEP_ALPHAS),
                              at<int32_t>(keep, L, FG_STEP_LAST_IDS), io->v_render, io->v_alphas, v_splats,
                              at<float>(keep, L, FG_STEP_SEG_CKPT), at<float>(keep, L, FG_STEP_RENDER),
                              at<uint32_t>(keep, L, FG_STEP_LIVE), config, stream);
  if (io->ev_raster_end && hipEventRecord(static_cast<hipEvent_t>(io->ev_raster_end), fg_hip_stream(stream)) != hipSuccess)
    return FG_ERR_LAUNCH;
  if (rc != FG_OK) return rc;
  const int32_t* radii = at<int32_t>(keep, L, FG_STEP_RADII);
  const float* sh_jac = at<float>(keep, L, FG_STEP_SH_JAC);
  if (d->raw) {
    if (io->v_rgb)
      return fg_preprocess_raw_bwd_factored(N, io->means, io->quats, io->d_quats, io->scales, io->d_scales, io->opacities,
                                            io->colors, io->features_rest, d->sh_degree, d->k_stored, d->with_depth, d->n_extra,
                                            io->viewmat, io->K, W, H, d->eps2d, d->antialiased, radii, v_splats, v_splats,
                                            FG_SPLAT_FLOATS, io->v_depths, io->v_conics, io->v_means, io->v_quats, io->v_d_quats,
                                            io->v_scales, io->v_d_scales, io->v_opacities, io->v_rgb, io->v_rgb_floats,
                                            io->v_extra, sh_jac, stream);
    return fg_preprocess_raw_bwd(N, io->means, io->quats, io->d_quats, io->scales, io->d_scales, io->opacities, io->colors,
                                 io->features_rest, d->sh_degree, d->k_stored, d->with_depth, d->n_extra, io->viewmat, io->K, W,
                                 H, d->eps2d, d->antialiased, radii, v_splats, v_splats, FG_SPLAT_FLOATS, io->v_depths,
                                 io->v_conics, io->v_means, io->v_quats, io->v_d_quats, io->v_scales, io->v_d_scales, io->v_opacities,
                                 io->v_colors, io->v_features_rest, io->v_extra, sh_jac, stream);
  }
  if (io->v_rgb)
    return fg_preprocess_bwd_factored(N, io->means, io->quats, io->scales, io->opacities, io->colors, d->sh_degree, d->k_stored,
                                      d->with_depth, d->n_extra, io->viewmat, io->K, W, H, d->eps2d, d->antialiased, radii,
                                      v_splats, v_splats, FG_SPLAT_FLOATS, io->v_depths, io->v_conics, io->v_means, io->v_quats,
                                      io->v_scales, io->v_opacities, io->v_rgb, io->v_rgb_floats, io->v_extra, sh_jac, stream);
  return fg_preprocess_bwd(N, io->means, io->quats, io->scales, io->opacities, io->colors, d->sh_degree, d->k_stored, d->n_color,
                           d->with_depth, d->n_extra, io->viewmat, io->K, W, H, d->eps2d, d->antialiased, radii, v_splats,
                           v_splats, FG_SPLAT_FLOATS, io->v_depths, io->v_conics, io->v_means, io->v_quats, io->v_scales, io->v_opacities,
                           io->v_colors, io->v_extra, sh_jac, stream);
}
```

freegaussian_amd/ops.py:

```python
from __future__ import annotations

from typing import Optional, Tuple

import ctypes
import os
import threading
import time

import torch

from . import _lib

TILE_SIZE = 16
SPLAT_FLOATS = 16
MAX_CHANNELS = 8


_STORAGE_USE_COUNT = getattr(torch._C, "_storage_Use_Count", None)


def _ptr(t: Optional[torch.Tensor]):
    return None if t is None else t.data_ptr()


def _stream():
    return torch._C._cuda_getCurrentRawStream(torch.cuda.current_device())


class StageTimer:

    def __init__(self, only=None, prewarm=0):
        self.events = {}
        self.only = only
        self._pool = []
        for _ in range(prewarm):
            a, b = torch.cuda.Event(enable_timing=True), torch.cuda.Event(enable_timing=True)
            a.record(), b.record()
            self._pool.append((a, b))

    def record(self, name):
        if self.only is not None and name not in self.only:
            return None
        pair = self._pool.pop() if self._pool else (torch.cuda.Event(enable_timing=True), torch.cuda.Event(enable_timing=True))
        self.events.setdefault(name, []).append(pair)
        return pair

    @staticmethod
    def handles(pair):
        for e in pair:
            if not e.cuda_event:
                e.record()
        return int(pair[0].cuda_event), int(pair[1].cuda_event)

    def summary(self):
        torch.cuda.synchronize()
        return {k: sum(a.elapsed_time(b) for a, b in v) / len(v) for k, v in self.events.items()}


def _env_flag(name: str, default: bool) -> bool:
    v = os.environ.get(name)
    return default if v is None else v != "0"


def launch_policy(**fields) -> "_lib.RasterConfig":
    cfg = _lib.RasterConfig.defaults()
    for k, v in fields.items():
        if k not in _lib.RasterConfig.FIELDS:
            raise ValueError(f"unknown launch-policy field {k!r}")
        setattr(cfg, k, int(v))
    return cfg


def launch_policy_from_env(env=None) -> "_lib.RasterConfig":
    env = os.environ if env is None else env
    f = {}

    def pair(name, a, b):
        v = env.get(name)
        if v is not None:
            parts = v.split(",")
            f[a] = int(parts[0])
            f[b] = int(parts[1]) if len(parts) > 1 else 0

    for name, field in (("FG_RASTER_PPT_FWD", "ppt_fwd"), ("FG_RASTER_PPT_BWD", "ppt_bwd"), ("FG_RASTER_BANDS", "bands_nx"),
                        ("FG_RASTER_SEG_PARTS", "seg_parts"), ("FG_RASTER_SEG_TAIL", "seg_tail"),
                        ("FG_DEBUG_ONLY_XCD", "debug_only_xcd"), ("FG_DEBUG_K_MOD", "debug_k_mod"),
                        ("FG_RASTER_BALANCE", "balance_bands"), ("FG_RASTER_HEAVY_WIDE", "heavy_wide"),
                        ("FG_RASTER_SEG_FINE", "seg_fine")):
        if env.get(name) is not None:
            f[field] = int(env[name])
    for name, field in (("FG_RASTER_PRIO_FWD", "prio_fwd"), ("FG_RASTER_PRIO_BWD", "prio_bwd")):
        if env.get(name) is not None:
            parts = [int(x) for x in env[name].split(",")]
            f[field] = parts[0] | ((parts[1] if len(parts) > 1 else 0) << 16)
    pair("FG_RASTER_TAIL_FWD", "tail4_fwd", "tail2_fwd")
    pair("FG_RASTER_TAIL_BWD", "tail4_bwd", "tail2_bwd")
    pair("FG_RASTER_SPLIT_FWD", "split4_fwd", "split2_fwd")
    pair("FG_RASTER_SPLIT_BWD", "split4_bwd", "split2_bwd")
    pair("FG_RASTER_SEG_GRADE", "seg_parts2", "seg_tail2")
    if env.get("FG_RASTER_LIVE") == "0":
        f["use_liveness"] = 0
    if env.get("FG_TILE_ORDER"):
        f["tile_order"] = {"r": 0, "b": 1, "c": 2, "s": 3, "x": 4, "y": 5}.get(env["FG_TILE_ORDER"][0], 1)
    return launch_policy(**f)


class RasterContext:

    def __init__(self, policy=None, env=None):
        e = os.environ if env is None else env
        self.policy = policy if policy is not None else launch_policy_from_env(e)
        self.stage_timer: Optional[StageTimer] = None
        self.speculative_binning = e.get("FG_SPECULATIVE_BINNING", "1") != "0"
        self.static_capacity: Optional[int] = None
        self.last_overflow: Optional[torch.Tensor] = None
        self.isect_capacity: dict = {}
        self.isect_n: dict = {}
        self.isect_recent: dict = {}
        self.capacity_redos = 0
        self.stagewise_raster_calls = 0
        self.full_ckpt_allocs = 0
        self.seg_slots_known = False
        self.tight_rects = e.get("FG_TIGHT_RECTS", "1") != "0"
        self.exact_tiles = e.get("FG_EXACT_TILES", "1") != "0"
        self.masks_always = e.get("FG_EXACT_TILES", "1") == "always"
        self.mask_keep_max = float(e.get("FG_MASK_KEEP_MAX", "1.01"))
        self.mask_keep = {}
        self.binning = e.get("FG_BINNING", "supertile")
        if self.binning not in ("supertile", "depthfirst"):
            raise ValueError(f"FG_BINNING={self.binning!r}: supertile | depthfirst")
        self.long_segments = e.get("FG_LONG_SEGMENTS", "auto")
        if self.long_segments not in ("auto", "always", "never"):
            raise ValueError(f"FG_LONG_SEGMENTS={self.long_segments!r}: auto | always | never")
        self.long_segment = int(e.get("FG_LONG_SEGMENT", "7936"))
        self.longest_segment_seen = 0
        self.long_many = int(e.get("FG_LONG_MANY", str(1 << 30)))
        self.long_cooldown = 64
        self.long_shapes = {}
        self.long_calls = 0
        self.test_small_slabs = False
        self.heavy_tiles = e.get("FG_HEAVY_TILES", "auto")
        if self.heavy_tiles not in ("auto", "always", "never"):
            raise ValueError(f"FG_HEAVY_TILES={self.heavy_tiles!r}: auto | always | never")
        self.heavy_tile_len = int(e.get("FG_HEAVY_TILE_LEN", "768"))
        self.heavy_flag_len = int(e.get("FG_HEAVY_FLAG_LEN", "2560"))
        self.heavy_cooldown = 64
        self.heavy_shapes = {}
        self.last_walk = 0
        self.long_walks = {}
        self.workspace_pool = e.get("FG_WORKSPACE_POOL", "1") != "0"
        self._workspaces = {}
        self.pool_fallback_calls = 0
        self.pool_new_buffers = 0
        self.plan_changes = 0
        self.plan_change_reasons = {}
        self._last_plan = {}
        if self.workspace_pool and _STORAGE_USE_COUNT is None:
            import warnings

            warnings.warn("freegaussian_amd: torch._C._storage_Use_Count is missing in this torch build -- the workspace pool is "
                          "off and every step allocates its 0.4-0.8 GB workspaces through the caching allocator (a device "
                          "allocation behind every refinement); RasterContext.pool_fallback_calls counts them", RuntimeWarning)
        sp = [int(x) for x in e.get("FG_UNEVEN_SPLIT_FWD", "8,5").split(",")]
        self.uneven_split_fwd = (sp[0], sp[1] if len(sp) > 1 else 0)
        self.uneven_split2_bwd = int(e.get("FG_UNEVEN_SPLIT2_BWD", "4"))
        self.uneven_interleave = e.get("FG_UNEVEN_INTERLEAVE", "1") != "0"
        self.heavy_calls = 0
        self._policy_copies = {}
        self.compact_slots = e.get("FG_COMPACT_SLOTS", "1") != "0"
        self.even_bands = e.get("FG_EVEN_BANDS", "1") != "0"
        self.even_calls = {}
        self.equal_stood = {}
        self.shape_calls = {}
        self.uneven_left = {}
        self.last_seg_slots = 0
        self.ckpt_need = {}
        self.ckpt_pending = {}
        self.direct_count = e.get("FG_DIRECT_COUNT", "1") != "0"
        self.fill_in_forward = e.get("FG_FILL_IN_FORWARD", "1") != "0"
        self.seg_ckpt_budget_bytes = int(float(e.get("FG_SEG_CKPT_BUDGET_MB", "2048")) * (1 << 20))
        self.overlap_pack = e.get("FG_OVERLAP_PACK", "0") == "1"
        self.sh_jacobian = e.get("FG_SH_JAC", "1") != "0"
        self.jobs_in_fill = e.get("FG_JOBS_IN_FILL", "1") != "0"
        self.step_calls = e.get("FG_STEP_CALLS", "1") != "0"
        self.grad_alloc = None
        self.color_grad_sink = None

    def workspace(self, kind: str, numel: int, dtype, dev) -> torch.Tensor:
        use_count = _STORAGE_USE_COUNT
        if not self.workspace_pool or use_count is None or (dev.type == "cuda" and torch.cuda.is_current_stream_capturing()):
            self.pool_fallback_calls += int(self.workspace_pool and use_count is None)
            return torch.empty(numel, dtype=dtype, device=dev)
        item = torch.empty(0, dtype=dtype).element_size()
        nbytes = numel * item
        stream_key = _stream() if dev.type == "cuda" else 0
        pool = self._workspaces.setdefault((kind, str(dev), stream_key), [])
        for i, (buf, idle) in enumerate(pool):
            if nbytes <= buf.numel() <= int(1.3 * nbytes) + (32 << 20) and use_count(buf.untyped_storage()._cdata) == idle:
                pool.append(pool.pop(i))
                return buf[:nbytes].view(dtype)
        buf = torch.empty((int(nbytes * 1.05) + (2 << 20) - 1) // (2 << 20) * (2 << 20), dtype=torch.uint8, device=dev)
        self.pool_new_buffers += 1
        pool.append((buf, use_count(buf.untyped_storage()._cdata)))
        if len(pool) > 4:
            for i, (old, idle) in enumerate(pool[:-1]):
                if use_count(old.untyped_storage()._cdata) == idle:
                    pool.pop(i)
                    break
            else:
                pool.pop(0)
        return buf[:nbytes].view(dtype)

    def masks_on(self, lkey) -> bool:
        if not self.exact_tiles:
            return False
        st = self.mask_keep.get(lkey)
        if self.masks_always or st is None or not st[0]:
            return True
        if sum(st[0]) / len(st[0]) <= self.mask_keep_max:
            return True
        if not self.even_shape(lkey):
            return True
        return st[1] >= 63

    def note_mask_ratio(self, lkey, masked: bool, n_isects: int, area: int) -> None:
        st = self.mask_keep.get(lkey)
        if st is None:
            if len(self.mask_keep) >= 256:
                self.mask_keep.pop(next(iter(self.mask_keep)))
            st = self.mask_keep[lkey] = [[], 0]
        if masked and area > 0:
            st[0].append(n_isects / area)
            del st[0][:-4]
            st[1] = 0
        else:
            st[1] += 1

    def heavy_lens(self, lkey):
        if lkey in self.long_walks:
            return self.heavy_flag_len, self.heavy_tile_len
        return max(self.heavy_flag_len, 3072), max(self.heavy_tile_len, 3072)

    def release_workspaces(self) -> int:
        freed = sum(buf.numel() for pool in self._workspaces.values() for buf, _ in pool)
        self._workspaces.clear()
        return freed

    def uneven_shape(self, lkey) -> bool:
        return self.uneven_left.get(lkey, 0) > 0

    def cfg(self, heavy: bool = False, seg_slots: int = 0, even: bool = False, uneven: bool = False, heavy_len: int = 0) -> int:
        return self.cfg_variant(heavy, seg_slots, even, uneven, heavy_len)[0]

    def cfg_variant(self, heavy: bool = False, seg_slots: int = 0, even: bool = False, uneven: bool = False, heavy_len: int = 0):
        heavy_len = (int(heavy_len) or self.heavy_tile_len) if heavy and self.policy.heavy_tiles <= 0 else 0
        if self.policy.seg_slots > 0:
            seg_slots = 0
        seg_slots = max(int(seg_slots), 0)
        even = bool(even) and self.policy.balance_bands in (-1, 1)
        split = self.uneven_split_fwd if uneven and not even and self.policy.split4_fwd < 0 and self.uneven_split_fwd[0] > 0 else None
        variant = (heavy_len, seg_slots, even, split)
        if not heavy_len and seg_slots <= 0 and not even and split is None:
            return self.policy.ptr(), variant
        key = (bytes(self.policy), heavy_len, int(seg_slots), even, split, self.uneven_split2_bwd, self.uneven_interleave)
        copy = self._policy_copies.get(key)
        if copy is None:
            copy = type(self.policy).from_buffer_copy(self.policy)
            if split is not None:
                copy.split4_fwd, copy.split2_fwd = split
                if self.policy.split4_bwd < 0 and self.uneven_split2_bwd > 0:
                    copy.split4_bwd, copy.split2_bwd = 20, self.uneven_split2_bwd
                if self.uneven_interleave and self.policy.balance_bands in (-1, 1):
                    copy.balance_bands = 3
            if heavy_len:
                copy.heavy_tiles = heavy_len
            if seg_slots > 0:
                copy.seg_slots = int(seg_slots)
            if even:
                copy.balance_bands = 2
            self._policy_copies[key] = copy
        return copy.ptr(), variant

    def capacity_for(self, key, N: int):
        if not self.speculative_binning:
            return None
        cap = self.isect_capacity.get(key)
        if cap is None:
            return None
        n_ref = self.isect_n.get(key, N)
        if n_ref == N:
            return cap
        if not (n_ref <= 2 * N and N <= 2 * n_ref):
            return None
        recent = self.isect_recent.get(key)
        if not recent:
            return min(int(cap * (N / n_ref) * 1.05) + 4096, 2**31 - 1)
        scaled = list_capacity_for([int(n * (N / n_i) * 1.05) for n, n_i in recent])
        return cap if scaled <= cap <= scaled + scaled // 4 else scaled

    def even_shape(self, lkey) -> bool:
        if not self.even_bands:
            return False
        if self.even_calls.get(lkey, 0) >= 8:
            return True
        n = self.shape_calls.get(lkey, 0)
        return self.equal_stood.get(lkey, 0) >= 8 and n % 64 != 0

    def seg_slots_for(self, lkey, capacity: int, n_tiles: int, N: int = 0) -> int:
        hist = self.ckpt_need.get(lkey) if self.compact_slots else None
        self.seg_slots_known = bool(hist)
        if not hist:
            return 0
        need = max(nd if (N <= 0 or n_i == N) else int(nd * (N / n_i) * 1.05) + 8 for nd, n_i in hist)
        per = int(need * 1.125) + 32
        slots = -(-8 * per // 4096) * 4096
        self.last_seg_slots = slots if slots < 0.9 * (capacity // 64 + n_tiles + 2) else 0
        return self.last_seg_slots


_default_context: Optional[RasterContext] = None
_tls = threading.local()


def _get_default() -> RasterContext:
    global _default_context
    if _default_context is None:
        _default_context = RasterContext()
    return _default_context


def current() -> RasterContext:
    stack = getattr(_tls, "stack", None)
    return stack[-1] if stack else _get_default()


class use:

    def __init__(self, ctx: Optional[RasterContext]):
        self.ctx = ctx

    def __enter__(self):
        if self.ctx is not None:
            if not hasattr(_tls, "stack"):
                _tls.stack = []
            _tls.stack.append(self.ctx)
        return self.ctx if self.ctx is not None else current()

    def __exit__(self, *exc):
        if self.ctx is not None:
            _tls.stack.pop()
        return False


def __getattr__(name):
    if name == "default_context":
        return _get_default()
    raise AttributeError(name)


def _call(name: str, *args, on=None, stage=None) -> None:
    fn = getattr(_lib.load(), name)
    stage_timer = current().stage_timer
    ev = stage_timer.record(stage or name) if stage_timer is not None else None
    if ev:
        ev[0].record(on) if on is not None else ev[0].record()
    rc = fn(*args)
    if ev:
        ev[1].record(on) if on is not None else ev[1].record()
    _lib.check(rc, name)


def _f32(t: torch.Tensor, name: str) -> torch.Tensor:
    if not t.is_cuda:
        raise _lib.FgRasterError(f"{name} must be a CUDA/HIP tensor: the raster path has no CPU fallback")
    if t.dtype != torch.float32:
        t = t.float()
    return t.contiguous()




class _Project(torch.autograd.Function):
    @staticmethod
    def forward(ctx, means, quats, scales, viewmat, K, width, height, eps2d, near, far, radius_clip, tile_size,
                calc_comp):
        ctx.rctx = current()
        lib = _lib.load()
        N = means.shape[0]
        dev = means.device
        radii = torch.empty(N, dtype=torch.int32, device=dev)
        means2d = torch.empty(N, 2, dtype=torch.float32, device=dev)
        depths = torch.empty(N, dtype=torch.float32, device=dev)
        conics = torch.empty(N, 3, dtype=torch.float32, device=dev)
        comp = torch.empty(N, dtype=torch.float32, device=dev) if calc_comp else None
        tiles = torch.empty(N, dtype=torch.int32, device=dev)
        _call("fg_project_fwd", N, _ptr(means), _ptr(quats), _ptr(scales), _ptr(viewmat), _ptr(K), width, height,
                               eps2d, near, far, radius_clip, tile_size, _ptr(radii), _ptr(means2d), _ptr(depths),
                               _ptr(conics), _ptr(comp), _ptr(tiles), _stream())
        ctx.save_for_backward(means, quats, scales, viewmat, K, radii, conics, comp)
        ctx.args = (width, height, eps2d)
        ctx.mark_non_differentiable(radii, tiles)
        if comp is None:
            comp = torch.empty(0, device=dev)
            ctx.mark_non_differentiable(comp)
        return radii, means2d, depths, conics, comp, tiles

    @staticmethod
    def backward(ctx, *grads):
        with use(ctx.rctx):
            return _Project._backward(ctx, *grads)

    @staticmethod
    def _backward(ctx, _v_radii, v_means2d, v_depths, v_conics, v_comp, _v_tiles):
        lib = _lib.load()
        means, quats, scales, viewmat, K, radii, conics, comp = ctx.saved_tensors
        width, height, eps2d = ctx.args
        N = means.shape[0]
        dev = means.device

        def z(shape):
            return torch.zeros(shape, dtype=torch.float32, device=dev)

        v_means2d = z((N, 2)) if v_means2d is None else v_means2d.contiguous()
        v_depths = z((N,)) if v_depths is None else v_depths.contiguous()
        v_conics = z((N, 3)) if v_conics is None else v_conics.contiguous()
        v_comp = None if (comp is None or v_comp is None or v_comp.numel() == 0) else v_comp.contiguous()
        v_means = torch.empty_like(means)
        v_quats = torch.empty_like(quats)
        v_scales = torch.empty_like(scales)
        _call("fg_project_bwd", N, _ptr(means), _ptr(quats), _ptr(scales), _ptr(viewmat), _ptr(K), width, height,
                               eps2d, _ptr(radii), _ptr(conics), _ptr(comp), _ptr(v_means2d), _ptr(v_depths),
                               _ptr(v_conics), _ptr(v_comp), _ptr(v_means), _ptr(v_quats), _ptr(v_scales),
                               _stream())
        return (v_means, v_quats, v_scales) + (None,) * 10


def project(means, quats, scales, viewmat, K, width, height, eps2d=0.3, near_plane=0.01, far_plane=1e10,
            radius_clip=0.0, tile_size=TILE_SIZE, calc_compensations=False):
    means, quats, scales = _f32(means, "means"), _f32(quats, "quats"), _f32(scales, "scales")
    viewmat, K = _f32(viewmat, "viewmat"), _f32(K, "K")
    return _Project.apply(means, quats, scales, viewmat, K, int(width), int(height), float(eps2d),
                          float(near_plane), float(far_plane), float(radius_clip), int(tile_size),
                          bool(calc_compensations))
# ... 772 lines not shown
        depths = torch.empty(N, dtype=torch.float32, device=dev)
        conics = torch.empty(N, 3, dtype=torch.float32, device=dev)
        comp = torch.empty(N, dtype=torch.float32, device=dev) if antialiased else None
        tiles = torch.empty(N, dtype=torch.int32, device=dev)
        splats = torch.empty(N, SPLAT_FLOATS, dtype=torch.float32, device=dev)
        depth_keys, tile_rects, tile_masks = _binning_side_outputs(N, tile_size, width, height, dev)
        sh_jac = None
        if sh_degree >= 1 and ctx.rctx.sh_jacobian:
            sh_jac = torch.empty(N, _lib.SH_JAC_FLOATS, dtype=torch.float32, device=dev)
        if ctx.rctx.color_grad_sink is not None:
            ctx.rctx.color_grad_sink("view", viewmat, dev)
        _call("fg_preprocess_raw_fwd", N, _ptr(means), _ptr(quats), _ptr(d_quats), _ptr(log_scales), _ptr(d_scales),
              _ptr(opacity_logits), _ptr(features_dc), _ptr(features_rest), sh_degree, k_stored, int(with_depth),
              _ptr(extra), n_extra, _ptr(viewmat), _ptr(K), width, height, eps2d, near, far, radius_clip, tile_size,
              int(antialiased), _ptr(radii), _ptr(means2d), _ptr(depths), _ptr(conics), _ptr(comp), _ptr(tiles),
              _ptr(splats), _ptr(depth_keys), _ptr(tile_rects), _ptr(tile_masks), _ptr(sh_jac), _stream())
        if depth_keys is not None:
            splats._fg_bin = (depth_keys, tile_rects, tile_masks)
        ctx.save_for_backward(means, quats, d_quats, log_scales, d_scales, opacity_logits, features_dc,
                              features_rest, extra, viewmat, K, radii, sh_jac)
        ctx.set_materialize_grads(False)
        ctx.cfg = cfg
        ctx.mark_non_differentiable(radii, tiles)
        return radii, means2d, depths, conics, tiles, splats

    @staticmethod
    def backward(ctx, *grads):
        with use(ctx.rctx):
            return _PreprocessRaw._backward(ctx, *grads)

    @staticmethod
    def _backward(ctx, _v_radii, v_means2d, v_depths, v_conics, _v_tiles, v_splats):
        (means, quats, d_quats, log_scales, d_scales, opacity_logits, features_dc, features_rest, extra, viewmat, K,
         radii, sh_jac) = ctx.saved_tensors
        (width, height, eps2d, near, far, radius_clip, tile_size, antialiased, sh_degree, with_depth) = ctx.cfg
        N = means.shape[0]
        dev = means.device
        k_stored = 1 + features_rest.shape[1]
        n_extra = 0 if extra is None else extra.shape[1]
        if v_splats is None:
            v_splats = torch.zeros(N, SPLAT_FLOATS, dtype=torch.float32, device=dev)
        if v_means2d is None:
            v_means2d = torch.zeros(N, 2, dtype=torch.float32, device=dev)
        v_means, v_quats, v_ls = _alloc_grad(means), _alloc_grad(quats), _alloc_grad(log_scales)
        v_ol = _alloc_grad(opacity_logits)
        v_dq = torch.empty_like(d_quats) if d_quats is not None else None
        v_ds = torch.empty_like(d_scales) if d_scales is not None else None
        v_extra = torch.empty_like(extra) if extra is not None else None
        v_means2d = v_means2d.reshape(N, 2)
        if v_means2d.stride(1) == 1 and v_means2d.stride(0) >= 2:
            m2_stride = v_means2d.stride(0)
        else:
            v_means2d, m2_stride = v_means2d.contiguous(), 2
        v_splats = v_splats.contiguous()

        def pose_grad():
            if not ctx.needs_input_grad[9]:
                return None
            return _viewmat_grad(True, means, quats, d_quats, log_scales, d_scales, opacity_logits, features_dc, features_rest,
                                 sh_degree, k_stored, 3, with_depth, n_extra, viewmat, K, width, height, eps2d, antialiased, radii,
                                 v_splats, v_means2d, m2_stride, None if v_depths is None else v_depths.contiguous(),
                                 None if v_conics is None else v_conics.contiguous(), sh_jac)

        color_grad_sink = ctx.rctx.color_grad_sink
        if color_grad_sink is not None:
            v_rgb = color_grad_sink("alloc", N, dev, means)
            _call("fg_preprocess_raw_bwd_factored", N, _ptr(means), _ptr(quats), _ptr(d_quats), _ptr(log_scales),
                  _ptr(d_scales), _ptr(opacity_logits), _ptr(features_dc), _ptr(features_rest), sh_degree, k_stored,
                  int(with_depth), n_extra, _ptr(viewmat), _ptr(K), width, height, eps2d, int(antialiased), _ptr(radii),
                  _ptr(v_splats.contiguous()), _ptr(v_means2d), m2_stride,
                  _ptr(None if v_depths is None else v_depths.contiguous()),
                  _ptr(None if v_conics is None else v_conics.contiguous()), _ptr(v_means), _ptr(v_quats), _ptr(v_dq),
                  _ptr(v_ls), _ptr(v_ds), _ptr(v_ol), _ptr(v_rgb), int(v_rgb.shape[1]), _ptr(v_extra), _ptr(sh_jac),
                  _stream())
            color_grad_sink("ready", v_rgb, means, viewmat, sh_degree, k_stored)
            return v_means, v_quats, v_dq, v_ls, v_ds, v_ol, None, None, v_extra, pose_grad(), None, None
        v_dc, v_rest = _alloc_grad(features_dc), _alloc_grad(features_rest)
        _call("fg_preprocess_raw_bwd", N, _ptr(means), _ptr(quats), _ptr(d_quats), _ptr(log_scales), _ptr(d_scales),
              _ptr(opacity_logits), _ptr(features_dc), _ptr(features_rest), sh_degree, k_stored, int(with_depth),
              n_extra, _ptr(viewmat), _ptr(K), width, height, eps2d, int(antialiased), _ptr(radii),
              _ptr(v_splats.contiguous()), _ptr(v_means2d), m2_stride,
              _ptr(None if v_depths is None else v_depths.contiguous()),
              _ptr(None if v_conics is None else v_conics.contiguous()), _ptr(v_means), _ptr(v_quats), _ptr(v_dq),
              _ptr(v_ls), _ptr(v_ds), _ptr(v_ol), _ptr(v_dc), _ptr(v_rest), _ptr(v_extra), _ptr(sh_jac),
              _stream())
        return v_means, v_quats, v_dq, v_ls, v_ds, v_ol, v_dc, v_rest, v_extra, pose_grad(), None, None


def preprocess_raw(means, quats, log_scales, opacity_logits, features_dc, features_rest, viewmat, K, width, height,
                   sh_degree, d_quats=None, d_scales=None, extra=None, eps2d=0.3, near_plane=0.01, far_plane=1e10,
                   radius_clip=0.0, tile_size=TILE_SIZE, antialiased=False, with_depth=False):
    means, quats, log_scales = _f32(means, "means"), _f32(quats, "quats"), _f32(log_scales, "scales")
    opacity_logits = _f32(opacity_logits.reshape(-1), "opacities")
    features_dc, features_rest = _f32(features_dc, "features_dc"), _f32(features_rest, "features_rest")
    viewmat, K = _f32(viewmat, "viewmat"), _f32(K, "K")
    N = means.shape[0]
    if features_dc.shape != (N, 3) or features_rest.dim() != 3 or features_rest.shape[0] != N:
        raise ValueError("features_dc[N,3] features_rest[N,K-1,3] expected")
    if sh_degree is None or not 0 <= sh_degree <= 3 or (sh_degree + 1) ** 2 > 1 + features_rest.shape[1]:
        raise ValueError("the raw-parameter path needs 0 <= sh_degree <= 3 within the stored coefficients")
    d_quats = None if d_quats is None else _f32(d_quats, "d_quats")
    d_scales = None if d_scales is None else _f32(d_scales, "d_scales")
    extra = None if extra is None else _f32(extra, "extra_channels")
    cfg = (int(width), int(height), float(eps2d), float(near_plane), float(far_plane), float(radius_clip),
           int(tile_size), bool(antialiased), int(sh_degree), bool(with_depth))
    return _PreprocessRaw.apply(means, quats, d_quats, log_scales, d_scales, opacity_logits, features_dc,
                                features_rest, extra, viewmat, K, cfg)


class _RasterSplats(torch.autograd.Function):

    @staticmethod
    def forward(ctx, splats, means2d, channels, width, height, tile_size, tile_offsets, flatten_ids, absgrad,
                background=None, n_clamp=0, expect_backward=False):
        ctx.rctx = current()
        dev = splats.device
        _wait_ready(splats)
        render = torch.empty(height, width, channels, dtype=torch.float32, device=dev)
        alphas = torch.empty(height, width, 1, dtype=torch.float32, device=dev)
        last_ids = torch.empty(height, width, dtype=torch.int32, device=dev)
        composite = background is not None or n_clamp > 0
        clamp_mask = torch.empty(height, width, dtype=torch.uint8, device=dev) if n_clamp > 0 else None
        prebuilt = getattr(tile_offsets, "_fg_jobs", None)
        key = (ctx.rctx, int(channels), int(width), int(height), int(tile_size))
        if prebuilt is not None and prebuilt[2] != key:
            prebuilt = None
        cfgp = prebuilt[3] if prebuilt is not None else ctx.rctx.cfg()
        words = int(_lib.load().fg_raster_jobs_words(int(width), int(height), int(tile_size), cfgp))
        jobs = seg_ckpt = live = v_splats = None
        if words > 0:
            n_ck = _seg_ckpt_floats(ctx.rctx, channels, width, height, tile_size, flatten_ids.numel(), cfgp)
            if n_ck > 0:
                seg_ckpt = torch.empty(n_ck, dtype=torch.float32, device=dev)
            live = torch.empty(max(int(flatten_ids.numel()), 1), dtype=torch.int32, device=dev)
            if ctx.rctx.fill_in_forward and expect_backward:
                v_splats = torch.empty(splats.shape[0], SPLAT_FLOATS, dtype=torch.float32, device=dev)
            if prebuilt is not None and prebuilt[1] == (seg_ckpt is not None):
                jobs = prebuilt[0]
            else:
                if prebuilt is not None:
                    cfgp = ctx.rctx.cfg()
                    words = int(_lib.load().fg_raster_jobs_words(int(width), int(height), int(tile_size), cfgp))
                jobs = torch.empty(2, words, dtype=torch.int32, device=dev)
                _call("fg_raster_build_jobs", width, height, tile_size, _ptr(tile_offsets), _ptr(jobs[0]), _ptr(jobs[1]),
                      int(seg_ckpt is not None), cfgp, _stream())
            _call("fg_raster_jobs_fwd", channels, width, height, tile_size, _ptr(splats), _ptr(tile_offsets),
                  _ptr(flatten_ids), _ptr(jobs[0]), _ptr(background), int(n_clamp), _ptr(render), _ptr(alphas),
                  _ptr(last_ids), _ptr(clamp_mask), _ptr(seg_ckpt), _ptr(live), _ptr(v_splats),
                  0 if v_splats is None else v_splats.numel(), None, cfgp, _stream(),
                  stage="fg_raster_composite_fwd" if composite else "fg_raster_fwd")
        elif composite:
            _call("fg_raster_composite_fwd", channels, width, height, tile_size, _ptr(splats), _ptr(tile_offsets),
                  _ptr(flatten_ids), _ptr(background), int(n_clamp), _ptr(render), _ptr(alphas), _ptr(last_ids),
                  _ptr(clamp_mask), cfgp, _stream())
        else:
            _call("fg_raster_fwd", channels, width, height, tile_size, _ptr(splats), _ptr(tile_offsets),
                  _ptr(flatten_ids), _ptr(render), _ptr(alphas), _ptr(last_ids), cfgp, _stream())
        ctx.save_for_backward(splats, tile_offsets, flatten_ids, alphas, last_ids, background, clamp_mask, seg_ckpt,
                              render if seg_ckpt is not None else None, live)
        ctx.jobs_bwd = jobs[1] if jobs is not None else None
        ctx.cfgp = cfgp
        ctx.v_splats_zeroed = v_splats
        ctx.set_materialize_grads(False)
        ctx.composite = (composite, int(n_clamp))
        ctx.geom = (channels, width, height, tile_size, absgrad, tuple(means2d.shape))
        ctx.means2d_ref = means2d if absgrad else None
        ctx.mark_non_differentiable(last_ids)
        return render, alphas, last_ids

    @staticmethod
    def backward(ctx, *grads):
        with use(ctx.rctx):
            return _RasterSplats._backward(ctx, *grads)

    @staticmethod
    def _backward(ctx, v_render, v_alphas, _v_last):
        (splats, tile_offsets, flatten_ids, alphas, last_ids, background, clamp_mask, seg_ckpt,
         image, live) = ctx.saved_tensors
        C, width, height, tile_size, absgrad, m2_shape = ctx.geom
        composite, n_clamp = ctx.composite
        N = splats.shape[0]
        v_render = torch.zeros(height, width, C, device=splats.device) if v_render is None else v_render
        v_alphas = None if v_alphas is None else v_alphas.contiguous()
        v_splats, ctx.v_splats_zeroed = ctx.v_splats_zeroed, None
        if v_splats is None:
            v_splats = torch.zeros(N, SPLAT_FLOATS, dtype=torch.float32, device=splats.device)
        if ctx.jobs_bwd is not None:
            _call("fg_raster_jobs_bwd", C, width, height, tile_size, _ptr(splats), _ptr(tile_offsets),
                  _ptr(flatten_ids), _ptr(ctx.jobs_bwd), _ptr(background), n_clamp, _ptr(clamp_mask), _ptr(alphas),
                  _ptr(last_ids), _ptr(v_render.contiguous()), _ptr(v_alphas), _ptr(v_splats), _ptr(seg_ckpt),
                  _ptr(image), _ptr(live), ctx.cfgp, _stream(),
                  stage="fg_raster_composite_bwd" if composite else "fg_raster_bwd")
            ctx.jobs_bwd = None
        elif composite:
            _call("fg_raster_composite_bwd", C, width, height, tile_size, _ptr(splats), _ptr(tile_offsets),
                  _ptr(flatten_ids), _ptr(background), n_clamp, _ptr(clamp_mask), _ptr(alphas), _ptr(last_ids),
                  _ptr(v_render.contiguous()), _ptr(v_alphas), _ptr(v_splats), ctx.cfgp, _stream())
        else:
            _call("fg_raster_bwd", C, width, height, tile_size, _ptr(splats), _ptr(tile_offsets), _ptr(flatten_ids),
                  _ptr(alphas), _ptr(last_ids), _ptr(v_render.contiguous()), _ptr(v_alphas),
                  _ptr(v_splats), ctx.cfgp, _stream())
        if ctx.rctx.color_grad_sink is not None and C >= 3:
            ctx.rctx.color_grad_sink("records", splats, v_splats)
        v_means2d = v_splats[:, 0:2].view(m2_shape)
        if absgrad and ctx.means2d_ref is not None:
            ctx.means2d_ref.absgrad = v_splats[:, 6:8].view(m2_shape)
            ctx.means2d_ref = None
        return v_splats, v_means2d, None, None, None, None, None, None, None, None, None, None


def rasterize_splats(splats, means2d, channels, width, height, tile_size, tile_offsets, flatten_ids, absgrad=False,
                     background=None, n_clamp=0):
    if background is not None:
        background = background.detach().to(device=splats.device, dtype=torch.float32).contiguous()
        if background.numel() != channels:
            raise ValueError(f"background must have {channels} values")
    if not 0 <= n_clamp <= channels:
        raise ValueError("n_clamp out of range")
    if tile_size != TILE_SIZE:
        raise ValueError("tile_size must be 16")
    if not 1 <= channels <= MAX_CHANNELS:
        raise ValueError(f"1..{MAX_CHANNELS} composited channels supported, got {channels}")
    expect_backward = torch.is_grad_enabled() and (splats.requires_grad or means2d.requires_grad)
    return _RasterSplats.apply(splats, means2d, int(channels), int(width), int(height), int(tile_size), tile_offsets,
                               flatten_ids, bool(absgrad), background, int(n_clamp), expect_backward)



_STEP_PLANS: dict = {}


def _step_plan(key, cfgp):
    plan = _STEP_PLANS.get(key)
    if plan is None:
        (dev, N, W, H, raw, sh_degree, k_stored, n_color, with_depth, n_extra, antialiased, n_clamp, want_backward,
         list_shares, flags, capacity, eps2d, near, far, radius_clip, _variant, _policy_bytes) = key
        d = _lib.StepDesc()
        d.size = ctypes.sizeof(_lib.StepDesc)
        d.N, d.width, d.height, d.tile_size, d.raw, d.sh_degree, d.k_stored, d.n_color = N, W, H, TILE_SIZE, raw, sh_degree, k_stored, n_color
        d.with_depth, d.n_extra, d.antialiased, d.n_clamp, d.want_backward, d.list_shares, d.flags = (
            with_depth, n_extra, antialiased, n_clamp, want_backward, list_shares, flags)
        d.eps2d, d.near_plane, d.far_plane, d.radius_clip, d.capacity = eps2d, near, far, radius_clip, capacity
        L = _lib.StepLayout()
        rc = _lib.load().fg_step_layout_query(ctypes.addressof(d), cfgp, ctypes.addressof(L))
        plan = (d, L, rc)
        if len(_STEP_PLANS) >= 512:
            _STEP_PLANS.pop(next(iter(_STEP_PLANS)))
        _STEP_PLANS[key] = plan
    return plan


def step_path_available(rctx, N, width, height, tile_size, dev) -> bool:
    if not rctx.step_calls or tile_size != TILE_SIZE or N <= 0:
        return False
    if (rctx.binning != "supertile" or not rctx.tight_rects or not rctx.direct_count or not rctx.jobs_in_fill
            or rctx.overlap_pack or not rctx.speculative_binning or not rctx.fill_in_forward or not rctx.sh_jacobian
            or rctx.static_capacity is not None or rctx.color_grad_sink is not None):
        return False
    st = rctx.stage_timer
    if st is not None and (st.only is None or not set(st.only) <= {"fg_raster_fwd", "fg_raster_bwd"}):
        return False
    tile_w, tile_h = (width + 15) // 16, (height + 15) // 16
    if rctx.capacity_for((dev, tile_w, tile_h, "fg_stbin"), N) is None:
        return False
    skey = (width, height, N >> 20, bytes(rctx.policy))
    ok = _STEP_SIZES.get(skey)
    if ok is None:
        lib = _lib.load()
        ok = bool(lib.fg_stbin_supported(N, tile_w, tile_h)) and int(lib.fg_raster_jobs_words(width, height, TILE_SIZE, rctx.cfg())) > 0
        if len(_STEP_SIZES) >= 512:
            _STEP_SIZES.clear()
        _STEP_SIZES[skey] = ok
    return ok


_STEP_SIZES: dict = {}


class _RasterStep(torch.autograd.Function):

    @staticmethod
    def forward(ctx, means, quats, d_quats, scales, d_scales, opacities, colors, features_rest, extra, viewmat, K,
                background, opts):
        rctx = current()
        ctx.rctx = rctx
        (raw, width, height, eps2d, near, far, radius_clip, antialiased, sh_degree, with_depth, n_clamp, absgrad,
         want_backward, batched) = opts
        N, dev = means.shape[0], means.device
        lib = _lib.load()
        tile_w, tile_h = (width + 15) // 16, (height + 15) // 16
        if raw:
            k_stored, n_color = 1 + features_rest.shape[1], 3
        elif sh_degree >= 0:
            k_stored, n_color = colors.shape[1], 3
        else:
            k_stored, n_color = 0, (0 if colors is None else colors.shape[1])
        n_extra = 0 if extra is None else extra.shape[1]
        channels = n_color + int(with_depth) + n_extra
        lkey, ckey = (dev, tile_w, tile_h), (dev, tile_w, tile_h, "fg_stbin")
        long_mode = rctx.long_segments == "always" or (rctx.long_segments == "auto" and rctx.long_shapes.get(lkey, 0) > 0)
        heavy = rctx.heavy_tiles == "always" or (rctx.heavy_tiles == "auto" and rctx.heavy_shapes.get(lkey, 0) > 0)
        capacity = rctx.capacity_for(ckey, N)
        masked = rctx.masks_on(lkey)
        while True:
            seg_slots = rctx.seg_slots_for(lkey, capacity, tile_w * tile_h, N) if channels == 3 and want_backward else 0
            cfgp, variant = rctx.cfg_variant(heavy, seg_slots, rctx.even_shape(lkey), rctx.uneven_shape(lkey), rctx.heavy_lens(lkey)[1])
            shares = want_backward and _seg_ckpt_floats(rctx, channels, width, height, TILE_SIZE, capacity, cfgp) > 0
            key = (dev, N, width, height, int(raw), sh_degree, k_stored, n_color, int(with_depth), n_extra, int(antialiased),
                   n_clamp, int(want_backward), int(shares),
                   ((_lib.STBIN_LONG_SEGMENTS | (_lib.STBIN_TEST_SMALL_SLABS if rctx.test_small_slabs else 0)) if long_mode else 0)
                   | (0 if masked else _lib.STEP_NO_FOOTPRINT_MASKS), capacity, eps2d,
                   near, far, radius_clip, variant, bytes(rctx.policy))
            d, L, rc = _step_plan(key, cfgp)
            _lib.check(rc, "fg_step_layout_query")
            last = rctx._last_plan.get(lkey)
            if last is not None and last != key:
                rctx.plan_changes += 1
                for name, i in (("N", 1), ("shares", 13), ("long_mode", 14), ("capacity", 15), ("variant", 20)):
                    if last[i] != key[i]:
                        rctx.plan_change_reasons[name] = rctx.plan_change_reasons.get(name, 0) + 1
            rctx._last_plan[lkey] = key
            keep = rctx.workspace("keep", (L.keep_bytes + 3) >> 2, torch.float32, dev)
            tmp = rctx.workspace("tmp", max(L.tmp_bytes, 8), torch.uint8, dev)
            count_slot, count_ptr = _count_slot()
            io = _lib.StepIO()
            io.means, io.quats, io.d_quats, io.scales, io.d_scales = _ptr(means), _ptr(quats), _ptr(d_quats), _ptr(scales), _ptr(d_scales)
            io.opacities, io.colors, io.features_rest, io.extra = _ptr(opacities), _ptr(colors), _ptr(features_rest), _ptr(extra)
            io.viewmat, io.K, io.background, io.count_out = _ptr(viewmat), _ptr(K), _ptr(background), count_ptr
            io.ckpt_need_out = count_ptr + 32 if shares else None
            st = rctx.stage_timer
            ev = st.record("fg_raster_fwd") if st is not None else None
            if ev:
                io.ev_raster_begin, io.ev_raster_end = StageTimer.handles(ev)
            _lib.check(lib.fg_step_fwd(ctypes.addressof(d), cfgp, ctypes.addressof(io), keep.data_ptr(), tmp.data_ptr(),
                                       ctypes.addressof(L), _stream()), "fg_step_fwd")
            rctx.long_calls += int(long_mode)
            rctx.heavy_calls += int(heavy and shares)
            rctx.full_ckpt_allocs += int(shares and rctx.compact_slots and seg_slots == 0 and not rctx.seg_slots_known and channels == 3)
            k32, i32 = keep, keep.view(torch.int32)
            strided, off, nb = torch.as_strided, L.offset, L.nbytes
            SB = _lib.STEP_BUFFER

            def view(base, name, shape, stride):
                i = SB[name]
                return None if nb[i] == 0 else strided(base, shape, stride, off[i] >> 2)

            if batched:
                render = view(k32, "render", (1, height, width, channels), (height * width * channels, width * channels, channels, 1))
                alphas = view(k32, "alphas", (1, height, width, 1), (height * width, width, 1, 1))
                means2d = view(k32, "means2d", (1, N, 2), (2 * N, 2, 1))
            else:
                render = view(k32, "render", (height, width, channels), (width * channels, channels, 1))
                alphas = view(k32, "alphas", (height, width, 1), (width, 1, 1))
                means2d = view(k32, "means2d", (N, 2), (2, 1))
            depths, conics = view(k32, "depths", (N,), (1,)), view(k32, "conics", (N, 3), (3, 1))
            radii, tiles = view(i32, "radii", (N,), (1,)), view(i32, "tiles", (N,), (1,))
            last_ids = view(i32, "last_ids", (height, width), (width, 1))
            splats = view(k32, "splats", (N, SPLAT_FLOATS), (SPLAT_FLOATS, 1))
            list_offsets = view(i32, "list_offsets", (tile_w * tile_h + 1,), (1,))
            n_isects = _note_counts(rctx, lkey, ckey, count_slot, shares, N, walks=shares, masked=masked)
            if n_isects <= capacity:
                break
            rctx.capacity_redos += 1
            capacity = max(n_isects, 1)
        flatten_ids = view(i32, "flatten_ids", (n_isects,), (1,))
        ctx.save_for_backward(means, quats, d_quats, scales, d_scales, opacities, colors, features_rest, extra, viewmat, K,
                              background, keep)
        ctx.plan = (d, L, cfgp, raw, N, sh_degree, absgrad)
        ctx.set_materialize_grads(False)
        ctx.mark_non_differentiable(last_ids, radii, tiles, splats, flatten_ids, list_offsets)
        return render, alphas, means2d, depths, conics, last_ids, radii, tiles, splats, flatten_ids, list_offsets

    @staticmethod
    def backward(ctx, *grads):
        with use(ctx.rctx):
            return _RasterStep._backward(ctx, *grads)

    @staticmethod
    def _backward(ctx, v_render, v_alphas, v_means2d, v_depths, v_conics, *_unused):
        (means, quats, d_quats, scales, d_scales, opacities, colors, features_rest, extra, viewmat, K, background,
         keep) = ctx.saved_tensors
        d, L, cfgp, raw, N, sh_degree, absgrad = ctx.plan
        rctx = ctx.rctx
        if not d.want_backward:
            raise _lib.FgRasterError("this step was rendered without gradient buffers (no input required a gradient)")

        v_splats = torch.as_strided(keep.data, (N, SPLAT_FLOATS), (SPLAT_FLOATS, 1), L.offset[_lib.STEP_BUFFER["v_splats"]] >> 2)
        ref = getattr(ctx, "means2d_ref", None)
        m2 = ref() if ref is not None else None
        earlier_m2_grad = None
        if getattr(ctx, "v_splats_consumed", False):
            if m2 is not None and m2.grad is not None:
                aliased = m2.grad.untyped_storage().data_ptr() == keep.untyped_storage().data_ptr()
                earlier_m2_grad = m2.grad.clone() if aliased else m2.grad
                if aliased and getattr(m2, "absgrad", None) is not None:
                    m2.absgrad = m2.absgrad.clone()
            v_splats.zero_()
        ctx.v_splats_consumed = True
        if v_means2d is not None:
            v_splats[:, 0:2] += v_means2d.reshape(N, 2)
        if v_render is None:
            H, W = d.height, d.width
            v_render = torch.zeros(H, W, L.channels, dtype=torch.float32, device=keep.device)
        io = _lib.StepIO()
        io.means, io.quats, io.d_quats, io.scales, io.d_scales = _ptr(means), _ptr(quats), _ptr(d_quats), _ptr(scales), _ptr(d_scales)
        io.opacities, io.colors, io.features_rest, io.extra = _ptr(opacities), _ptr(colors), _ptr(features_rest), _ptr(extra)
        io.viewmat, io.K, io.background = _ptr(viewmat), _ptr(K), _ptr(background)
        keepalive = [v_render.contiguous(), None if v_alphas is None else v_alphas.contiguous(),
                     None if v_depths is None else v_depths.contiguous(), None if v_conics is None else v_conics.contiguous()]
        io.v_render, io.v_alphas, io.v_depths, io.v_conics = (_ptr(t) for t in keepalive)
        v_means, v_quats, v_scales, v_opac = _alloc_grad(means), _alloc_grad(quats), _alloc_grad(scales), _alloc_grad(opacities)
        v_dq = torch.empty_like(d_quats) if d_quats is not None else None
        v_ds = torch.empty_like(d_scales) if d_scales is not None else None
        v_colors = _alloc_grad(colors) if colors is not None else None
        v_rest = _alloc_grad(features_rest) if features_rest is not None else None
        v_extra = torch.empty_like(extra) if extra is not None else None
        io.v_means, io.v_quats, io.v_d_quats, io.v_scales, io.v_d_scales = _ptr(v_means), _ptr(v_quats), _ptr(v_dq), _ptr(v_scales), _ptr(v_ds)
        io.v_opacities, io.v_colors, io.v_features_rest, io.v_extra = _ptr(v_opac), _ptr(v_colors), _ptr(v_rest), _ptr(v_extra)
        st = rctx.stage_timer
        ev = st.record("fg_raster_bwd") if st is not None else None
        if ev:
            io.ev_raster_begin, io.ev_raster_end = StageTimer.handles(ev)
        _lib.check(_lib.load().fg_step_bwd(ctypes.addressof(d), cfgp, ctypes.addressof(io), keep.data_ptr(),
                                           ctypes.addressof(L), _stream()), "fg_step_bwd")
        v_viewmat = None
        if ctx.needs_input_grad[9]:
            SBF = _lib.STEP_BUFFER

            def kept(name, dtype, shape):
                i = SBF[name]
                if L.nbytes[i] == 0:
                    return None
                base = keep.data if dtype is torch.float32 else keep.data.view(torch.int32)
                return torch.as_strided(base, shape, (shape[1], 1) if len(shape) == 2 else (1,), L.offset[i] >> 2)

            k_stored = (1 + features_rest.shape[1]) if raw else (colors.shape[1] if sh_degree >= 0 else 0)
            n_color = 3 if (raw or sh_degree >= 0) else (0 if colors is None else colors.shape[1])
            v_viewmat = _viewmat_grad(raw, means, quats, d_quats, scales, d_scales, opacities, colors, features_rest, sh_degree,
                                      k_stored, n_color, d.with_depth, d.n_extra, viewmat, K, d.width, d.height, d.eps2d,
                                      d.antialiased, kept("radii", torch.int32, (N,)), v_splats, v_splats, SPLAT_FLOATS,
                                      keepalive[2], keepalive[3], kept("sh_jac", torch.float32, (N, _lib.SH_JAC_FLOATS)))
        if m2 is not None:
            m2.grad = v_splats[:, 0:2].view(m2.shape)
            if earlier_m2_grad is not None:
                m2.grad = earlier_m2_grad + m2.grad
            if absgrad:
                m2.absgrad = v_splats[:, 6:8].view(m2.shape)
        return v_means, v_quats, v_dq, v_scales, v_ds, v_opac, v_colors, v_rest, v_extra, v_viewmat, None, None, None


def raster_step(means, quats, scales, opacities, colors, viewmat, K, width, height, *, raw=False, d_quats=None, d_scales=None,
                features_rest=None, extra=None, background=None, n_clamp=0, eps2d=0.3, near_plane=0.01, far_plane=1e10,
                radius_clip=0.0, antialiased=False, sh_degree=-1, with_depth=False, absgrad=False, batched=False):
    f = [None if t is None else _f32(t, "input") for t in (means, quats, d_quats, scales, d_scales, opacities, colors,
                                                           features_rest, extra, viewmat, K)]
    if f[5].dim() != 1:
        f[5] = f[5].reshape(-1)
    bg = None if background is None else background.detach().to(device=f[0].device, dtype=torch.float32).contiguous()
    want_backward = torch.is_grad_enabled() and any(t is not None and t.requires_grad for t in f[:10])
    opts = (bool(raw), int(width), int(height), float(eps2d), float(near_plane), float(far_plane), float(radius_clip),
            bool(antialiased), int(sh_degree), bool(with_depth), int(n_clamp), bool(absgrad), bool(want_backward),
            bool(batched))
    out = _RasterStep.apply(*f, bg, opts)
    return out + (out[0].grad_fn,)




def camera_flow(depth: torch.Tensor, K: torch.Tensor, veloc: torch.Tensor, omega: torch.Tensor) -> torch.Tensor:
    lib = _lib.load()
    depth, K = _f32(depth, "depth"), _f32(K, "K")
    veloc, omega = _f32(veloc, "veloc"), _f32(omega, "omega")
    H, W = depth.shape
    flow = torch.empty(H, W, 2, dtype=torch.float32, device=depth.device)
    _call("fg_camera_flow", W, H, _ptr(depth), _ptr(K), _ptr(veloc), _ptr(omega), _ptr(flow), _stream())
    return flow


def reprojection_flow(depth0: torch.Tensor, depth1: torch.Tensor, K: torch.Tensor, M: torch.Tensor,
                      sign: float = -1.0) -> torch.Tensor:
    depth0, depth1, K, M = _f32(depth0, "depth0"), _f32(depth1, "depth1"), _f32(K, "K"), _f32(M, "M")
    H, W = depth0.shape
    if depth1.shape != depth0.shape or M.numel() != 12:
        raise ValueError("depth maps of equal shape and a 3x4 matrix expected")
    flow = torch.empty(H, W, 2, dtype=torch.float32, device=depth0.device)
    _call("fg_reprojection_flow", W, H, _ptr(depth0), _ptr(depth1), _ptr(K), _ptr(M), float(sign), _ptr(flow), _stream())
    return flow


class _GaussianFlow(torch.autograd.Function):
    @staticmethod
    def forward(ctx, means2d, depths, vel, radii, K, veloc, omega):
        ctx.rctx = current()
        lib = _lib.load()
        N = depths.shape[0]
        u_gs = torch.empty(N, 2, dtype=torch.float32, device=depths.device)
        u_cam = torch.empty_like(u_gs)
        _call("fg_flow_fwd", N, _ptr(means2d), _ptr(depths), _ptr(radii), _ptr(vel), _ptr(K), _ptr(veloc), _ptr(omega),
                            _ptr(u_gs), _ptr(u_cam), _stream())
        ctx.save_for_backward(means2d, depths, vel, radii, K, veloc, omega)
        return u_gs, u_cam

    @staticmethod
    def backward(ctx, *grads):
        with use(ctx.rctx):
            return _GaussianFlow._backward(ctx, *grads)

    @staticmethod
    def _backward(ctx, v_gs, v_cam):
        lib = _lib.load()
        means2d, depths, vel, radii, K, veloc, omega = ctx.saved_tensors
        N = depths.shape[0]
        v_gs = torch.zeros(N, 2, device=depths.device) if v_gs is None else v_gs.contiguous()
        v_cam = torch.zeros(N, 2, device=depths.device) if v_cam is None else v_cam.contiguous()
        v_m = torch.empty_like(means2d)
        v_d = torch.empty_like(depths)
        v_v = torch.empty_like(vel)
        _call("fg_flow_bwd", N, _ptr(means2d), _ptr(depths), _ptr(radii), _ptr(vel), _ptr(K), _ptr(veloc), _ptr(omega),
                            _ptr(v_gs), _ptr(v_cam), _ptr(v_m), _ptr(v_d), _ptr(v_v), _stream())
        return v_m, v_d, v_v, None, None, None, None


def gaussian_flow(means2d, depths, vel, K, veloc, omega, radii=None) -> Tuple[torch.Tensor, torch.Tensor]:
    means2d, depths, vel = _f32(means2d, "means2d"), _f32(depths, "depths"), _f32(vel, "vel")
    K, veloc, omega = _f32(K, "K"), _f32(veloc, "veloc"), _f32(omega, "omega")
    return _GaussianFlow.apply(means2d.reshape(-1, 2), depths, vel, radii, K, veloc, omega)
```

include/fgraster.h:

```cpp
#ifndef FGRASTER_H
#define FGRASTER_H

#include <stddef.h>
#include <stdint.h>

#ifdef __cplusplus
extern "C" {
#endif

typedef void* fg_stream_t;

#define FG_OK 0
#define FG_ERR_INVALID_ARG (-1)
#define FG_ERR_LAUNCH (-2)
#define FG_ERR_WORKSPACE (-3)
#define FG_ERR_UNSUPPORTED (-4)

#define FG_MAX_CHANNELS 8
#define FG_SPLAT_FLOATS 16
#define FG_SH_JAC_FLOATS 10
#define FG_ABI_VERSION 10
#define FG_COUNT_OUT_WORDS 16

int fg_abi_version(void);
const char* fg_error_string(int code);

int fg_project_fwd(int N, const float* means, const float* quats, const float* scales,
                   const float* viewmat, const float* K, int width, int height, float eps2d,
                   float near_plane, float far_plane, float radius_clip, int tile_size,
                   int32_t* radii, float* means2d, float* depths, float* conics,
                   float* compensations, int32_t* tiles_touched, fg_stream_t stream);

int fg_project_bwd(int N, const float* means, const float* quats, const float* scales,
                   const float* viewmat, const float* K, int width, int height, float eps2d,
                   const int32_t* radii, const float* conics, const float* compensations,
                   const float* v_means2d, const float* v_depths, const float* v_conics,
                   const float* v_compensations, float* v_means, float* v_quats,
                   float* v_scales, fg_stream_t stream);

int fg_sh_fwd(int N, int degree, int k_stored, const float* means, const float* viewmat,
              const float* coeffs, const int32_t* radii, float* colors, fg_stream_t stream);
int fg_sh_bwd(int N, int degree, int k_stored, const float* means, const float* viewmat,
              const float* coeffs, const int32_t* radii, const float* colors,
              const float* v_colors, float* v_coeffs, float* v_means, fg_stream_t stream);

size_t fg_scan_workspace_bytes(int N);
int fg_scan_tiles(int N, const int32_t* tiles_touched, int64_t* cum_tiles, void* workspace,
                  size_t workspace_bytes, fg_stream_t stream);
int fg_tile_bin(int N, const float* means2d, const int32_t* radii, const float* depths,
                const int64_t* cum_tiles, int tile_size, int tile_w, int tile_h,
                int64_t* isect_ids, int32_t* flatten_ids, fg_stream_t stream);

size_t fg_sort_workspace_bytes(int64_t n);
int fg_sort_pairs(int64_t n, int64_t* keys, int32_t* vals, int end_bit, void* workspace,
                  size_t workspace_bytes, fg_stream_t stream);
int fg_tile_ranges(int64_t n, const int64_t* sorted_keys, int n_tiles, int32_t* tile_offsets,
                   fg_stream_t stream);

size_t fg_sort32_workspace_bytes(int64_t n);
int fg_sort_pairs32(int64_t n, uint32_t* keys, int32_t* vals, int end_bit, void* workspace,
                    size_t workspace_bytes, fg_stream_t stream);

size_t fg_bin_prepare_workspace_bytes(int N);
int fg_bin_prepare(int N, const float* depths, const int32_t* radii, const int32_t* tiles_touched,
                   int32_t* order, int64_t* cum_tiles, void* workspace, size_t workspace_bytes,
                   fg_stream_t stream);
int fg_bin_prepare_rects(int N, const float* depths, const int32_t* radii, const float* means2d,
                         int tile_size, int tile_w, int tile_h, int32_t* order, int64_t* cum_tiles,
                         int32_t* rects_sorted, void* workspace, size_t workspace_bytes,
                         fg_stream_t stream);
int fg_bin_prepare_keys(int N, uint32_t* depth_keys, const int32_t* tile_rects, int32_t* order,
                        int64_t* cum_tiles, int32_t* rects_sorted, int64_t* count_out, void* workspace,
                        size_t workspace_bytes, fg_stream_t stream);
int fg_stbin_supported(int N, int tile_w, int tile_h);
size_t fg_stbin_count_workspace_bytes(int N, int tile_w, int tile_h);
int fg_stbin_count(int N, const int32_t* tile_rects, const uint64_t* tile_masks, int tile_w, int tile_h,
                   int32_t* tile_offsets, int64_t* count_out, void* workspace, size_t workspace_bytes, fg_stream_t stream);
size_t fg_stbin_fill_workspace_bytes(int64_t capacity);
#define FG_STBIN_LONG_SEGMENTS 1
#define FG_STEP_NO_FOOTPRINT_MASKS 2
#define FG_STBIN_TEST_SMALL_SLABS 4
int fg_stbin_fill(int N, const uint32_t* depth_keys, const int32_t* tile_rects, const uint64_t* tile_masks, int tile_w,
                  int tile_h, int64_t capacity, const int32_t* tile_offsets, const void* count_workspace,
                  int32_t* flatten_ids, int32_t* list_offsets, void* workspace, size_t workspace_bytes,
                  int flags, fg_stream_t stream);

size_t fg_bin_emit_workspace_bytes(int64_t n_isects);
int fg_bin_emit_sort(int N, int64_t n_isects, const float* means2d, const int32_t* radii,
                     const int32_t* order, const int64_t* cum_tiles, const int32_t* rects_sorted,
                     int tile_size, int tile_w, int tile_h, uint32_t* tile_keys, int32_t* flatten_ids,
                     int32_t* tile_offsets, void* workspace, size_t workspace_bytes, fg_stream_t stream);
int fg_bin_emit_sort_capacity(int N, int64_t capacity, const float* means2d, const int32_t* radii,
                              const int32_t* order, const int64_t* cum_tiles,
                              const int32_t* rects_sorted, int tile_size, int tile_w, int tile_h,
                              uint32_t* tile_keys, int32_t* flatten_ids, int32_t* tile_offsets,
                              void* workspace, size_t workspace_bytes, fg_stream_t stream);
int fg_isect_keys(int64_t n_isects, const uint32_t* tile_keys, const int32_t* flatten_ids,
                  const float* depths, int64_t* isect_ids, fg_stream_t stream);

int fg_pack_splats(int N, int channels, const float* means2d, const float* conics,
                   const float* opacities, const float* features, float* splats,
                   fg_stream_t stream);
typedef struct fg_raster_config {
  int32_t size;
  int32_t ppt_fwd;
  int32_t ppt_bwd;
  int32_t tile_order;
  int32_t bands_nx;
  int32_t tail4_fwd;
  int32_t tail2_fwd;
  int32_t tail4_bwd;
  int32_t tail2_bwd;
  int32_t split4_fwd;
  int32_t split2_fwd;
  int32_t split4_bwd;
  int32_t split2_bwd;
  int32_t use_liveness;
  int32_t seg_parts;
  int32_t seg_tail;
  int32_t seg_parts2;
  int32_t seg_tail2;
  int32_t debug_only_xcd;
  int32_t debug_k_mod;
  int32_t balance_bands;
  int32_t heavy_tiles;
  int32_t seg_slots;
  int32_t prio_fwd;
  int32_t prio_bwd;
  int32_t heavy_wide;
  int32_t seg_fine;
} fg_raster_config;
void fg_raster_config_init(fg_raster_config* config);

int fg_raster_fwd(int channels, int width, int height, int tile_size, const float* splats,
                  const int32_t* tile_offsets, const int32_t* flatten_ids, float* render,
                  float* alphas, int32_t* last_ids, const fg_raster_config* config,
                    fg_stream_t stream);
int fg_raster_bwd(int channels, int width, int height, int tile_size, const float* splats,
                  const int32_t* tile_offsets, const int32_t* flatten_ids,
                  const float* alphas, const int32_t* last_ids, const float* v_render,
                  const float* v_alphas, float* v_splats, const fg_raster_config* config,
                    fg_stream_t stream);
int fg_raster_composite_fwd(int channels, int width, int height, int tile_size, const float* splats,
                            const int32_t* tile_offsets, const int32_t* flatten_ids,
                            const float* background, int n_clamp, float* image, float* alphas,
                            int32_t* last_ids, uint8_t* clamp_mask, const fg_raster_config* config,
                    fg_stream_t stream);
int fg_raster_composite_bwd(int channels, int width, int height, int tile_size, const float* splats,
                            const int32_t* tile_offsets, const int32_t* flatten_ids,
                            const float* background, int n_clamp, const uint8_t* clamp_mask,
                            const float* alphas, const int32_t* last_ids, const float* v_image,
                            const float* v_alphas, float* v_splats, const fg_raster_config* config,
                    fg_stream_t stream);
int64_t fg_raster_jobs_words(int width, int height, int tile_size, const fg_raster_config* config);
int fg_raster_build_jobs(int width, int height, int tile_size, const int32_t* tile_offsets,
                         int32_t* jobs_fwd, int32_t* jobs_bwd, int bwd_list_shares, const fg_raster_config* config,
                    fg_stream_t stream);
int fg_stbin_fill_jobs(int N, const uint32_t* depth_keys, const int32_t* tile_rects, const uint64_t* tile_masks,
                       int tile_w, int tile_h, int64_t capacity, const int32_t* tile_offsets, const void* count_workspace,
                       int32_t* flatten_ids, int32_t* list_offsets, void* workspace, size_t workspace_bytes,
                       int width, int height, int tile_size, int32_t* jobs_fwd, int32_t* jobs_bwd,
                       int bwd_list_shares, const fg_raster_config* config, int flags, int64_t* ckpt_need_out,
                       fg_stream_t stream);
int fg_raster_jobs_fwd(int channels, int width, int height, int tile_size, const float* splats,
                       const int32_t* tile_offsets, const int32_t* flatten_ids, const int32_t* jobs,
                       const float* background, int n_clamp, float* image, float* alphas,
                       int32_t* last_ids, uint8_t* clamp_mask, float* seg_ckpt, uint32_t* live_words,
                       float* zero_buf, int64_t zero_floats, int64_t* walk_out, const fg_raster_config* config,
                       fg_stream_t stream);
int64_t fg_raster_seg_ckpt_floats(int channels, int width, int height, int tile_size, int64_t n_isects, const fg_raster_config* config);
int fg_raster_jobs_bwd(int channels, int width, int height, int tile_size, const float* splats,
                       const int32_t* tile_offsets, const int32_t* flatten_ids, const int32_t* jobs,
                       const float* background, int n_clamp, const uint8_t* clamp_mask,
                       const float* alphas, const int32_t* last_ids, const float* v_image,
                       const float* v_alphas, float* v_splats, const float* seg_ckpt, const float* image,
                       const uint32_t* live_words, const fg_raster_config* config,
                    fg_stream_t stream);
int fg_unpack_grads(int N, int channels, const float* v_splats, float* v_means2d,
                    float* v_means2d_abs, float* v_conics, float* v_opacities,
                    float* v_features, fg_stream_t stream);

int fg_preprocess_fwd(int N, const float* means, const float* quats, const float* scales,
                      const float* opacities, const float* colors, int sh_degree, int k_stored,
                      int n_color, int with_depth, const float* extra, int n_extra,
                      const float* viewmat, const float* K, int width, int height, float eps2d,
                      float near_plane, float far_plane, float radius_clip, int tile_size,
                      int antialiased, int32_t* radii, float* means2d, float* depths, float* conics,
                      float* compensations, int32_t* tiles_touched, float* splats,
                      uint32_t* depth_keys, int32_t* tile_rects, uint64_t* tile_masks, float* sh_jac, fg_stream_t stream);
size_t fg_viewmat_bwd_workspace_bytes(int N);
int fg_viewmat_bwd(int N, int raw, const float* means, const float* quats, const float* d_quats, const float* scales,
                   const float* d_scales, const float* opacities, const float* colors, const float* features_rest,
                   int sh_degree, int k_stored, int n_color, int with_depth, int n_extra, const float* viewmat,
                   const float* K, int width, int height, float eps2d, int antialiased, const int32_t* radii,
                   const float* v_splats, const float* v_means2d, int v_means2d_stride, const float* v_depths,
                   const float* v_conics, const float* sh_jac, float* out, void* workspace, size_t workspace_bytes,
                   fg_stream_t stream);
int fg_sh_pack_fwd(int N, const float* means, const float* opacities, const float* colors, int sh_degree,
                   int k_stored, int n_color, int with_depth, const float* extra, int n_extra,
                   const float* viewmat, int antialiased, const int32_t* radii, const float* means2d,
                   const float* depths, const float* conics, const float* compensations, float* splats,
                   fg_stream_t stream);
int fg_preprocess_bwd(int N, const float* means, const float* quats, const float* scales,
                      const float* opacities, const float* colors, int sh_degree, int k_stored,
                      int n_color, int with_depth, int n_extra, const float* viewmat, const float* K,
                      int width, int height, float eps2d, int antialiased, const int32_t* radii,
                      const float* v_splats, const float* v_means2d, int v_means2d_stride,
                      const float* v_depths, const float* v_conics, float* v_means, float* v_quats,
                      float* v_scales, float* v_opacities, float* v_colors, float* v_extra,
                      const float* sh_jac, fg_stream_t stream);

int fg_preprocess_raw_fwd(int N, const float* means, const float* quats, const float* d_quats,
                          const float* log_scales, const float* d_scales,
                          const float* opacity_logits, const float* features_dc,
                          const float* features_rest, int sh_degree, int k_stored, int with_depth,
                          const float* extra, int n_extra, const float* viewmat, const float* K,
                          int width, int height, float eps2d, float near_plane, float far_plane,
                          float radius_clip, int tile_size, int antialiased, int32_t* radii,
                          float* means2d, float* depths, float* conics, float* compensations,
                          int32_t* tiles_touched, float* splats, uint32_t* depth_keys,
                          int32_t* tile_rects, uint64_t* tile_masks, float* sh_jac, fg_stream_t stream);
int fg_preprocess_raw_bwd(int N, const float* means, const float* quats, const float* d_quats,
                          const float* log_scales, const float* d_scales,
                          const float* opacity_logits, const float* features_dc,
                          const float* features_rest, int sh_degree, int k_stored, int with_depth,
                          int n_extra, const float* viewmat, const float* K, int width, int height,
                          float eps2d, int antialiased, const int32_t* radii, const float* v_splats,
                          const float* v_means2d, int v_means2d_stride, const float* v_depths,
                          const float* v_conics, float* v_means, float* v_quats, float* v_d_quats,
                          float* v_log_scales, float* v_d_scales, float* v_opacity_logits,
                          float* v_features_dc, float* v_features_rest, float* v_extra,
                          const float* sh_jac, fg_stream_t stream);

int fg_preprocess_bwd_factored(int N, const float* means, const float* quats, const float* scales,
                               const float* opacities, const float* colors, int sh_degree, int k_stored,
                               int with_depth, int n_extra, const float* viewmat, const float* K,
                               int width, int height, float eps2d, int antialiased, const int32_t* radii,
                               const float* v_splats, const float* v_means2d, int v_means2d_stride,
                               const float* v_depths, const float* v_conics, float* v_means,
                               float* v_quats, float* v_scales, float* v_opacities, float* v_rgb,
                               int v_rgb_floats, float* v_extra, const float* sh_jac, fg_stream_t stream);
int fg_sh_grad_accumulate(int N, int n_views, int sh_degree, int k_stored, const float* means,
                          const float* payload, int64_t view_stride, int payload_floats, float scale,
                          float* v_coeffs, fg_stream_t stream);
int fg_preprocess_raw_bwd_factored(
    int N, const float* means, const float* quats, const float* d_quats, const float* log_scales, const float* d_scales,
    const float* opacity_logits, const float* features_dc, const float* features_rest, int sh_degree, int k_stored,
    int with_depth, int n_extra, const float* viewmat, const float* K, int width, int height, float eps2d, int antialiased,
    const int32_t* radii, const float* v_splats, const float* v_means2d, int v_means2d_stride, const float* v_depths,
    const float* v_conics, float* v_means, float* v_quats, float* v_d_quats, float* v_log_scales, float* v_d_scales,
    float* v_opacity_logits, float* v_rgb, int v_rgb_floats, float* v_extra, const float* sh_jac, fg_stream_t stream);
int fg_sh_grad_accumulate_split(int N, int n_views, int sh_degree, int k_stored, const float* means,
                                const float* payload, int64_t view_stride, int payload_floats, float scale,
                                float* v_features_dc, float* v_features_rest, fg_stream_t stream);
int fg_payload_compact(int N, int payload_floats, const float* dense, const int32_t* incl_scan, int64_t capacity,
                       float* out, fg_stream_t stream);
int fg_payload_expand(int N, int payload_floats, int n_views, const float* compact, int64_t block_stride,
                      int64_t capacity, float* dense, int64_t dense_stride, fg_stream_t stream);

enum {
  FG_STEP_RADII, FG_STEP_MEANS2D, FG_STEP_DEPTHS, FG_STEP_CONICS, FG_STEP_COMP, FG_STEP_TILES, FG_STEP_SPLATS,
  FG_STEP_DEPTH_KEYS, FG_STEP_TILE_RECTS, FG_STEP_TILE_MASKS, FG_STEP_SH_JAC, FG_STEP_TILE_OFFSETS, FG_STEP_LIST_OFFSETS, FG_STEP_FLATTEN_IDS,
  FG_STEP_JOBS, FG_STEP_LIVE, FG_STEP_SEG_CKPT, FG_STEP_V_SPLATS, FG_STEP_RENDER, FG_STEP_ALPHAS, FG_STEP_LAST_IDS,
  FG_STEP_CLAMP_MASK, FG_STEP_COUNT_WS, FG_STEP_FILL_WS, FG_STEP_BUFFERS
};
typedef struct fg_step_desc {
  int32_t size;
  int32_t N, width, height, tile_size;
  int32_t raw;
  int32_t sh_degree;
  int32_t k_stored, n_color, with_depth, n_extra, antialiased;
  int32_t n_clamp;
  int32_t want_backward;
  int32_t list_shares;
  int32_t flags;
  float eps2d, near_plane, far_plane, radius_clip;
  int64_t capacity;
} fg_step_desc;
typedef struct fg_step_io {
  const float *means, *quats, *d_quats, *scales, *d_scales, *opacities, *colors, *features_rest, *extra, *viewmat, *K,
      *background;
  int64_t* count_out;
  const float *v_render, *v_alphas, *v_depths, *v_conics;
  float *v_means, *v_quats, *v_d_quats, *v_scales, *v_d_scales, *v_opacities, *v_colors, *v_features_rest, *v_extra;
  float* v_rgb;
  int32_t v_rgb_floats;
  void *ev_raster_begin, *ev_raster_end;
  int64_t* ckpt_need_out;
} fg_step_io;
typedef struct fg_step_layout {
  int64_t keep_bytes, tmp_bytes;
  int64_t offset[FG_STEP_BUFFERS], nbytes[FG_STEP_BUFFERS];
  int64_t jobs_words, seg_ckpt_floats;
  int32_t channels;
} fg_step_layout;
int fg_step_layout_query(const fg_step_desc* desc, const fg_raster_config* config, fg_step_layout* out);
int fg_step_fwd(const fg_step_desc* desc, const fg_raster_config* config, const fg_step_io* io, void* keep, void* tmp,
                const fg_step_layout* layout, fg_stream_t stream);
int fg_step_bwd(const fg_step_desc* desc, const fg_raster_config* config, const fg_step_io* io, void* keep,
                const fg_step_layout* layout, fg_stream_t stream);

int fg_densify_stats(int N, const float* absgrad, const int32_t* radii, float max_dim, float* xys_grad_norm,
                     float* vis_counts, float* max_2dsize, fg_stream_t stream);
int fg_densify_flags(int N, int do_densify, float max_dim, float densify_grad_thresh,
                     float densify_size_thresh, float split_screen_size, float cull_alpha_thresh,
                     float cull_scale_thresh, float cull_screen_size, const float* xys_grad_norm,
                     const float* vis_counts, const float* max_2dsize, const float* log_scales,
                     const float* opacity_logits, uint8_t* flags, fg_stream_t stream);
int fg_densify_map(int N, const uint8_t* flags, const int32_t* pos_old, const int32_t* pos_child,
                   const int32_t* pos_dup, const int32_t* rank_split, int n_old, int n_child,
                   int n_split_total, int n_split_samples, int32_t* src_index, int32_t* sample_index,
                   fg_stream_t stream);
int fg_gather_rows(int64_t n_rows, int row_floats, const float* src, const int32_t* src_index,
                   int64_t zero_from, float* dst, fg_stream_t stream);
int fg_split_children(int first_row, int n_rows, const int32_t* sample_index, const float* samples,
                      float* means, float* log_scales, const float* quats, fg_stream_t stream);

int fg_mask_backproject(int N, const float* means2d, const float* depths, const int32_t* radii,
                        const float* depth_map, int width, int height, const uint8_t* atrb_masks,
                        const uint8_t* mask_valids, int n_labels_stored, int n_attributes,
                        uint8_t* gaussian_masks, fg_stream_t stream);

int fg_camera_flow(int width, int height, const float* depth, const float* K,
                   const float* veloc, const float* omega, float* flow, fg_stream_t stream);
int fg_reprojection_flow(int width, int height, const float* depth0, const float* depth1,
                         const float* K, const float* M, float sign, float* flow, fg_stream_t stream);
int fg_flow_fwd(int N, const float* means2d, const float* depths, const int32_t* radii,
                const float* vel, const float* K, const float* veloc, const float* omega,
                float* u_gs, float* u_cam, fg_stream_t stream);
int fg_flow_bwd(int N, const float* means2d, const float* depths, const int32_t* radii,
                const float* vel, const float* K, const float* veloc, const float* omega,
                const float* v_u_gs, const float* v_u_cam, float* v_means2d, float* v_depths,
                float* v_vel, fg_stream_t stream);

size_t fg_l1_ssim_workspace_floats(int height, int width, int channels);
int fg_l1_ssim_fwd(int height, int width, int channels, const float* pred, const float* gt, float* maps,
                   float* workspace, size_t workspace_floats, float* out, fg_stream_t stream);
int fg_l1_ssim_bwd(int height, int width, int channels, const float* pred, const float* gt, const float* maps,
                   const float* v_out, float* v_pred, fg_stream_t stream);

int fg_adam_step(int64_t n, float* param, const float* grad, float* exp_avg, float* exp_avg_sq, double lr, double beta1,
                 double beta2, double eps, int64_t step, fg_stream_t stream);
#define FG_ADAM_MAX_TENSORS 16
typedef struct fg_adam_tensor {
  float* param;
  const float* grad;
  float* exp_avg;
  float* exp_avg_sq;
  int64_t n;
  double lr, beta1, beta2, eps;
  int64_t step;
} fg_adam_tensor;
int fg_adam_step_multi(int count, const fg_adam_tensor* tensors, fg_stream_t stream);

#define FG_KNN_MAX_K 8
size_t fg_knn_workspace_bytes(int64_t n);
int fg_knn(int64_t n, const float* xyz, int k, float* dist2_out, int32_t* idx_out, void* workspace,
           size_t workspace_bytes, fg_stream_t stream);

#ifdef __cplusplus
}
#endif
#endif
```

Before: 2768 Mpix/s.

## Fuse offset scan into columns kernel and skip large-sort launch when unneeded

The standalone offsets-scan kernel is replaced by a last-block-done ticket scheme inside the columns kernel, so the final block scans tile and supertile offsets and one launch plus its dependency gap disappear. Separately, the host learns per shape whether any supertile exceeds the small-sort limit. After several clean calls it drops the large-sort kernel launch and redoes the step if the guess proves wrong. In that mode the small-sort kernel zero-fills the lists of oversized segments so they stay defined. The costs are a cross-block ticket protocol that relies on agent-scope atomics, a shrunk 256-thread scan, and occasional redo work.

```diff
diff --git a/freegaussian_amd/_lib.py b/freegaussian_amd/_lib.py
--- a/freegaussian_amd/_lib.py
+++ b/freegaussian_amd/_lib.py
@@ -104,6 +104,7 @@
 STBIN_LONG_SEGMENTS = 1
 STBIN_TEST_SMALL_SLABS = 4
 STEP_NO_FOOTPRINT_MASKS = 2
+STBIN_NO_LARGE_SORT = 8
 SH_JAC_FLOATS = 10
 _lib = None
 
diff --git a/freegaussian_amd/csrc/stbin.hip b/freegaussian_amd/csrc/stbin.hip
--- a/freegaussian_amd/csrc/stbin.hip
+++ b/freegaussian_amd/csrc/stbin.hip
@@ -6,6 +6,8 @@
 namespace {
 
 constexpr int SB_BLOCK = 256;
+constexpr int SB_TICKET_GROUP = 32, SB_TICKET_STRIDE = 32;
+__host__ __device__ __forceinline__ int ticket_groups(int workgroups) { return (workgroups + SB_TICKET_GROUP - 1) / SB_TICKET_GROUP; }
 constexpr int SB_CHUNK = 4096;
 constexpr int SC_BLOCK = 1024, SC_WAVES = SC_BLOCK / 64, SC_PER = SB_CHUNK / SC_BLOCK;
 __host__ __device__ __forceinline__ int chunk_rounds(int N) { return N <= 320 * 1024 ? 1 : (N <= 640 * 1024 ? 2 : SC_PER); }
@@ -162,13 +164,15 @@
 __global__ void __launch_bounds__(SC_BLOCK)
 sb_count_kernel(int N, int per, const int2* __restrict__ rects, const unsigned long long* __restrict__ masks, int tile_w,
                 int tile_h, int band_rows, uint32_t* __restrict__ table_t, uint32_t* __restrict__ table_s,
-                unsigned long long* __restrict__ area_part) {
+                unsigned long long* __restrict__ area_part, uint32_t* __restrict__ tickets, int ticket_lines) {
   extern __shared__ int32_t s_grid[];
   __shared__ int4 s_cq[SC_WAVES][64];
   __shared__ uint32_t s_cqx[SC_WAVES][64];
   __shared__ unsigned long long s_cmarks[SC_WAVES];
   const Geo g = geo_of(tile_w, tile_h);
   const int chunk = blockIdx.x;
+  if (chunk == 0)
+    for (int i = threadIdx.x; i < ticket_lines; i += SC_BLOCK) tickets[i * SB_TICKET_STRIDE] = 0u;
   const int gwt = tile_w + 1, gws = g.sw + 1;
   const int T = tile_w * tile_h, S = g.sw * g.sh;
   const int lane = fg::lane_id(), wave = threadIdx.x >> 6;
@@ -291,11 +295,131 @@
   }
 }
 
+#ifndef FG_SB_SCAN_PER
+#define FG_SB_SCAN_PER 32
+#endif
+constexpr int SO_BLOCK = SB_BLOCK, SO_WAVES = SO_BLOCK / 64, SO_PER = FG_SB_SCAN_PER;
+__device__ __forceinline__ int so_slot(int j) { return j + (j >> 5); }
+constexpr int SO_WORDS = SO_BLOCK * SO_PER + ((SO_BLOCK * SO_PER) >> 5);
+__device__ __forceinline__ uint64_t scan_counts_in_place(int n, int32_t* offs, uint32_t* buf, uint32_t* wave_tot,
+                                                         uint32_t* largest = nullptr, uint32_t over_thr = 0xFFFFFFFFu,
+                                                         uint32_t* n_over = nullptr) {
+  const int lane = fg::lane_id(), wave = threadIdx.x >> 6;
+  uint32_t carry = 0, big = 0, over = 0;
+  uint64_t total = 0;
+  for (int base = 0; base < n; base += SO_BLOCK * SO_PER) {
+    uint32_t in[SO_PER];
+#pragma unroll
+    for (int k = 0; k < SO_PER; ++k) {
+      const int i = base + k * SO_BLOCK + threadIdx.x;
+      in[k] = i < n ? (uint32_t)__hip_atomic_load(&offs[i + 1], __ATOMIC_RELAXED, __HIP_MEMORY_SCOPE_AGENT) : 0u;
+    }
+#pragma unroll
+    for (int k = 0; k < SO_PER; ++k) {
+      buf[so_slot(k * SO_BLOCK + threadIdx.x)] = in[k];
+      big = max(big, in[k]);
+      over += in[k] > over_thr ? 1u : 0u;
+    }
+    __syncthreads();
+    uint32_t v[SO_PER], sum = 0;
+#pragma unroll
+    for (int k = 0; k < SO_PER; ++k) {
+      v[k] = buf[so_slot(threadIdx.x * SO_PER + k)];
+      sum += v[k];
+    }
+    const uint32_t incl = wave_incl_scan(sum, lane);
+    if (lane == 63) wave_tot[wave] = incl;
+    __syncthreads();
+    uint32_t run = carry + incl - sum, all = 0;
+#pragma unroll
+    for (int k = 0; k < SO_WAVES; ++k) {
+      const uint32_t t = wave_tot[k];
+      if (k < wave) run += t;
+      all += t;
+    }
+#pragma unroll
+    for (int k = 0; k < SO_PER; ++k) {
+      run += v[k];
+      buf[so_slot(threadIdx.x * SO_PER + k)] = run;
+    }
+    __syncthreads();
+#pragma unroll
+    for (int k = 0; k < SO_PER; ++k) {
+      const int i = base + k * SO_BLOCK + threadIdx.x;
+      if (i < n) offs[i + 1] = (int32_t)buf[so_slot(k * SO_BLOCK + threadIdx.x)];
+    }
+    carry += all;
+    total += all;
+    __syncthreads();
+  }
+  if (threadIdx.x == 0) offs[0] = 0;
+  if (largest || n_over) {
+#pragma unroll
+    for (int m = 1; m < 64; m <<= 1) {
+      big = max(big, (uint32_t)__shfl_xor((int)big, m));
+      over += (uint32_t)__shfl_xor((int)over, m);
+    }
+    __syncthreads();
+    if (lane == 0) {
+      wave_tot[wave] = big;
+      wave_tot[SO_WAVES + wave] = over;
+    }
+    __syncthreads();
+    over = 0;
+#pragma unroll
+    for (int k = 0; k < SO_WAVES; ++k) {
+      big = max(big, wave_tot[k]);
+      over += wave_tot[SO_WAVES + k];
+    }
+    if (largest) *largest = big;
+    if (n_over) *n_over = over;
+  }
+  return total;
+}
+__device__ __forceinline__ void finish_tile_offsets(int T, int32_t* tile_offsets, int64_t* __restrict__ count_out, uint32_t* buf,
+                                                    uint32_t* wave_tot) {
+  uint32_t longest_tile = 0;
+  const uint64_t total = scan_counts_in_place(T, tile_offsets, buf, wave_tot, &longest_tile);
+  if (threadIdx.x == 0 && count_out) {
+    __hip_atomic_store(count_out + 2, (int64_t)longest_tile, __ATOMIC_RELAXED, __HIP_MEMORY_SCOPE_SYSTEM);
+    __hip_atomic_store(count_out, (int64_t)total, __ATOMIC_RELAXED, __HIP_MEMORY_SCOPE_SYSTEM);
+  }
+}
+__device__ __forceinline__ void finish_supertile_offsets(int S, int32_t* st_offsets, int64_t* __restrict__ count_out,
+                                                         const unsigned long long* __restrict__ area_part, int n_chunks,
+                                                         uint32_t* buf, uint32_t* wave_tot) {
+  unsigned long long a = 0;
+  if (count_out)
+    for (int c = threadIdx.x; c < n_chunks; c += SO_BLOCK) a += area_part[c];
+  uint32_t longest = 0, n_over = 0;
+  scan_counts_in_place(S, st_offsets, buf, wave_tot, &longest, (uint32_t)SB_LONG_SPLIT, &n_over);
+  if (!count_out) return;
+  unsigned long long* s_sum = reinterpret_cast<unsigned long long*>(buf);
+#pragma unroll
+  for (int m = 1; m < 64; m <<= 1) a += __shfl_xor(a, m);
+  __syncthreads();
+  if ((threadIdx.x & 63) == 0) s_sum[threadIdx.x >> 6] = a;
+  __syncthreads();
+  if (threadIdx.x == 0) {
+    unsigned long long all = 0;
+#pragma unroll
+    for (int w = 0; w < SO_WAVES; ++w) all += s_sum[w];
+    __hip_atomic_store(count_out + 14, (int64_t)all, __ATOMIC_RELAXED, __HIP_MEMORY_SCOPE_SYSTEM);
+    __hip_atomic_store(count_out + 3, (int64_t)n_over, __ATOMIC_RELAXED, __HIP_MEMORY_SCOPE_SYSTEM);
+    __hip_atomic_store(count_out + 1, (int64_t)longest, __ATOMIC_RELAXED, __HIP_MEMORY_SCOPE_SYSTEM);
+  }
+}
+
 constexpr int SC_COLS = 16, SC_SLICES = SB_BLOCK / SC_COLS;
+static_assert(SC_COLS <= 64, "the totals' writers are lanes of the wavefront whose lane 0 draws the ticket");
 __global__ void __launch_bounds__(SB_BLOCK)
 sb_columns_kernel(int T, int S, int n_chunks, int wg_t, const uint32_t* __restrict__ table_t,
-                  uint32_t* __restrict__ table_s, int32_t* __restrict__ tile_offsets, int32_t* __restrict__ st_offsets) {
+                  uint32_t* __restrict__ table_s, int32_t* tile_offsets, int32_t* st_offsets, uint32_t* tickets,
+                  int64_t* __restrict__ count_out, const unsigned long long* __restrict__ area_part) {
   __shared__ uint32_t part[SC_SLICES][SC_COLS];
+  __shared__ alignas(16) uint32_t s_scan[SO_WORDS];
+  __shared__ uint32_t s_wave_tot[2 * SO_WAVES];
+  __shared__ int s_last;
   const bool tiles = (int)blockIdx.x < wg_t;
   const int n = tiles ? T : S;
   const int cl = threadIdx.x % SC_COLS, qd = threadIdx.x / SC_COLS;
@@ -324,145 +448,46 @@
     if (k < qd) run += p;
     total += p;
   }
-  if (col >= n) return;
-  if (tiles) {
-    if (qd == 0) tile_offsets[col + 1] = (int32_t)total;
-    return;
-  }
-  if (small) {
-#pragma unroll
-    for (int u = 0; u < U; ++u) {
-      if (c0 + u < c1) table_s[(size_t)(c0 + u) * n + col] = run;
-      run += v[u];
-    }
-  } else {
-    for (int c = c0; c < c1; ++c) {
-      const uint32_t x = table_s[(size_t)c * n + col];
-      table_s[(size_t)c * n + col] = run;
-      run += x;
-    }
-  }
-  if (qd == 0) st_offsets[col + 1] = (int32_t)total;
-}
-
-constexpr int SO_BLOCK = 1024, SO_WAVES = SO_BLOCK / 64, SO_PER = 8;
-__device__ __forceinline__ uint64_t scan_counts_in_place(int n, int32_t* __restrict__ offs, uint32_t* buf,
-                                                         uint32_t* wave_tot, uint32_t* largest = nullptr,
-                                                         uint32_t over_thr = 0xFFFFFFFFu, uint32_t* n_over = nullptr) {
-  const int lane = fg::lane_id(), wave = threadIdx.x >> 6;
-  uint32_t carry = 0, big = 0, over = 0;
-  uint64_t total = 0;
-  for (int base = 0; base < n; base += SO_BLOCK * SO_PER) {
-    uint32_t in[SO_PER];
-#pragma unroll
-    for (int k = 0; k < SO_PER; ++k) {
-      const int i = base + k * SO_BLOCK + threadIdx.x;
-      in[k] = i < n ? (uint32_t)offs[i + 1] : 0u;
-    }
-#pragma unroll
-    for (int k = 0; k < SO_PER; ++k) {
-      buf[k * SO_BLOCK + threadIdx.x] = in[k];
-      big = max(big, in[k]);
-      over += in[k] > over_thr ? 1u : 0u;
-    }
-    __syncthreads();
-    uint32_t v[SO_PER], sum = 0;
-#pragma unroll
-    for (int k = 0; k < SO_PER; k += 4) {
-      const uint4 x = *reinterpret_cast<const uint4*>(&buf[threadIdx.x * SO_PER + k]);
-      v[k] = x.x; v[k + 1] = x.y; v[k + 2] = x.z; v[k + 3] = x.w;
-    }
-#pragma unroll
-    for (int k = 0; k < SO_PER; ++k) sum += v[k];
-    const uint32_t incl = wave_incl_scan(sum, lane);
-    if (lane == 63) wave_tot[wave] = incl;
-    __syncthreads();
-    uint32_t run = carry + incl - sum, all = 0;
-#pragma unroll
-    for (int k = 0; k < SO_WAVES; ++k) {
-      const uint32_t t = wave_tot[k];
-      if (k < wave) run += t;
-      all += t;
-    }
-#pragma unroll
-    for (int k = 0; k < SO_PER; ++k) {
-      run += v[k];
-      v[k] = run;
-    }
-#pragma unroll
-    for (int k = 0; k < SO_PER; k += 4)
-      *reinterpret_cast<uint4*>(&buf[threadIdx.x * SO_PER + k]) = make_uint4(v[k], v[k + 1], v[k + 2], v[k + 3]);
-    __syncthreads();
-#pragma unroll
-    for (int k = 0; k < SO_PER; ++k) {
-      const int i = base + k * SO_BLOCK + threadIdx.x;
-      if (i < n) offs[i + 1] = (int32_t)buf[k * SO_BLOCK + threadIdx.x];
-    }
-    carry += all;
-    total += all;
-    __syncthreads();
-  }
-  if (threadIdx.x == 0) offs[0] = 0;
-  if (largest) {
-#pragma unroll
-    for (int m = 1; m < 64; m <<= 1) big = max(big, (uint32_t)__shfl_xor((int)big, m));
-    __syncthreads();
-    if (lane == 0) wave_tot[wave] = big;
-    __syncthreads();
-#pragma unroll
-    for (int k = 0; k < SO_WAVES; ++k) big = max(big, wave_tot[k]);
-    *largest = big;
-  }
-  if (n_over) {
-#pragma unroll
-    for (int m = 1; m < 64; m <<= 1) over += (uint32_t)__shfl_xor((int)over, m);
-    __syncthreads();
-    if (lane == 0) wave_tot[wave] = over;
-    __syncthreads();
-    over = 0;
-#pragma unroll
-    for (int k = 0; k < SO_WAVES; ++k) over += wave_tot[k];
-    *n_over = over;
-  }
-  return total;
-}
-__global__ void __launch_bounds__(SO_BLOCK)
-sb_offsets_kernel(int T, int S, int32_t* __restrict__ tile_offsets, int32_t* __restrict__ st_offsets,
-                  int64_t* __restrict__ count_out, const unsigned long long* __restrict__ area_part, int n_chunks) {
-  __shared__ alignas(16) uint32_t buf[SO_BLOCK * SO_PER];
-  __shared__ uint32_t wave_tot[SO_WAVES];
-  if (blockIdx.x == 1) {
-    uint32_t longest = 0, n_over = 0;
-    scan_counts_in_place(S, st_offsets, buf, wave_tot, &longest, (uint32_t)SB_LONG_SPLIT, &n_over);
-    if (count_out) {
-      __shared__ unsigned long long s_sum[SO_WAVES];
-      unsigned long long a = 0;
-      for (int c = threadIdx.x; c < n_chunks; c += SO_BLOCK) a += area_part[c];
-#pragma unroll
-      for (int m = 1; m < 64; m <<= 1) a += __shfl_xor(a, m);
-      if ((threadIdx.x & 63) == 0) s_sum[threadIdx.x >> 6] = a;
-      __syncthreads();
-      if (threadIdx.x == 0) {
-        unsigned long long all = 0;
-#pragma unroll
-        for (int w = 0; w < SO_WAVES; ++w) all += s_sum[w];
-        __hip_atomic_store(count_out + 14, (int64_t)all, __ATOMIC_RELAXED, __HIP_MEMORY_SCOPE_SYSTEM);
-      }
-    }
-    if (threadIdx.x == 0 && count_out) {
-      __hip_atomic_store(count_out + 3, (int64_t)n_over, __ATOMIC_RELAXED, __HIP_MEMORY_SCOPE_SYSTEM);
-      __hip_atomic_store(count_out + 1, (int64_t)longest, __ATOMIC_RELAXED, __HIP_MEMORY_SCOPE_SYSTEM);
-      __threadfence_system();
-    }
-    return;
-  }
-  uint32_t longest_tile = 0;
-  const uint64_t total = scan_counts_in_place(T, tile_offsets, buf, wave_tot, &longest_tile);
-  if (threadIdx.x == 0 && count_out) {
-    __hip_atomic_store(count_out + 2, (int64_t)longest_tile, __ATOMIC_RELAXED, __HIP_MEMORY_SCOPE_SYSTEM);
-    __hip_atomic_store(count_out, (int64_t)total, __ATOMIC_RELAXED, __HIP_MEMORY_SCOPE_SYSTEM);
-    __threadfence_system();
-  }
+  int32_t* offs = tiles ? tile_offsets : st_offsets;
+  if (col < n && qd == 0) __hip_atomic_store(&offs[col + 1], (int32_t)total, __ATOMIC_RELAXED, __HIP_MEMORY_SCOPE_AGENT);
+  if (threadIdx.x < 64) {
+    asm volatile("s_waitcnt vmcnt(0)" ::: "memory");
+    if (threadIdx.x == 0) {
+      const int b = (int)blockIdx.x - (tiles ? 0 : wg_t), nb = tiles ? wg_t : (int)gridDim.x - wg_t;
+      uint32_t* tk = tickets + (tiles ? 0 : (1 + ticket_groups(wg_t)) * SB_TICKET_STRIDE);
+      const int grp = b / SB_TICKET_GROUP, in_grp = min(SB_TICKET_GROUP, nb - grp * SB_TICKET_GROUP);
+      bool last = __hip_atomic_fetch_add(&tk[(1 + grp) * SB_TICKET_STRIDE], 1u, __ATOMIC_RELAXED, __HIP_MEMORY_SCOPE_AGENT) + 1u ==
+                  (uint32_t)in_grp;
+      if (last)
+        last = __hip_atomic_fetch_add(&tk[0], 1u, __ATOMIC_RELAXED, __HIP_MEMORY_SCOPE_AGENT) + 1u == (uint32_t)ticket_groups(nb);
+      if (last) {
+        __builtin_amdgcn_fence(__ATOMIC_ACQUIRE, "agent");
+        asm volatile("s_waitcnt vmcnt(0)" ::: "memory");
+      }
+      s_last = last ? 1 : 0;
+    }
+  }
+  if (col < n && !tiles) {
+    if (small) {
+#pragma unroll
+      for (int u = 0; u < U; ++u) {
+        if (c0 + u < c1) table_s[(size_t)(c0 + u) * n + col] = run;
+        run += v[u];
+      }
+    } else {
+      for (int c = c0; c < c1; ++c) {
+        const uint32_t x = table_s[(size_t)c * n + col];
+        table_s[(size_t)c * n + col] = run;
+        run += x;
+      }
+    }
+  }
+  __syncthreads();
+  if (!s_last) return;
+  if (tiles)
+    finish_tile_offsets(T, tile_offsets, count_out, s_scan, s_wave_tot);
+  else
+    finish_supertile_offsets(S, st_offsets, count_out, area_part, n_chunks, s_scan, s_wave_tot);
 }
 
 template <int NTH>
@@ -1285,7 +1310,7 @@
                      const int32_t* __restrict__ st_offsets, uint64_t* __restrict__ entries,
                      uint64_t* __restrict__ scratch, long long capacity, int32_t* __restrict__ flatten_ids,
                      int32_t* __restrict__ list_offsets, int32_t* __restrict__ over_list, int job_blocks,
-                     fgjobs::JobBuild jb, const int4* __restrict__ long_list, LongTables lt) {
+                     fgjobs::JobBuild jb, const int4* __restrict__ long_list, LongTables lt, int no_large) {
   __shared__ SortShared<SB_SMALL_WAVES, SB_SMALL_KPT, SB_SMALL_BUCKET_BITS> sh;
   if ((int)blockIdx.x < job_blocks) {
     static_assert(sizeof(sh.img) >= fgjobs::FG_BAND_MAX_ROWS * sizeof(uint32_t), "row sums in the element buffer");
@@ -1299,6 +1324,16 @@
       sh, st, tile_w, tile_h, tile_offsets, st_offsets, entries, scratch, (long long)total > capacity, total, flatten_ids,
       list_offsets, over_list != nullptr);
   if (skewed && threadIdx.x == 0) over_list[2 + atomicAdd(over_list, 1)] = -(st + 1);
+  if (no_large && (long long)total <= capacity && st_offsets[st + 1] - st_offsets[st] > SB_LONG_SPLIT) {
+    int tile_base[4], tile_id[4];
+    supertile_tile_bases(st, tile_w, tile_h, tile_offsets, tile_base, tile_id);
+#pragma unroll
+    for (int j = 0; j < 4; ++j) {
+      if (tile_id[j] < 0) continue;
+      const int end = tile_offsets[tile_id[j] + 1];
+      for (int i = tile_base[j] + (int)threadIdx.x; i < end; i += 64 * SB_SMALL_WAVES) flatten_ids[i] = 0;
+    }
+  }
   if (over_list && (long long)total <= capacity) {
     using Sh = SortShared<SB_SMALL_WAVES, SB_SMALL_KPT, SB_SMALL_BUCKET_BITS>;
     static_assert(Sh::MAXN == SB_LONG_SPLIT, "in long mode no segment is left for the large launch");
@@ -1468,6 +1503,8 @@
   int32_t* large_list;
   int4* long_list;
   unsigned long long* area_part;
+  uint32_t* tickets;
+  int ticket_lines;
   size_t bytes;
 };
 template <typename T>
@@ -1490,6 +1527,9 @@
   o += al256((S + 2) * 16);
   w.area_part = ws_at<unsigned long long>(base, o);
   o += al256(nc * 8);
+  w.tickets = ws_at<uint32_t>(base, o);
+  w.ticket_lines = 2 + ticket_groups((int)((T + SC_COLS - 1) / SC_COLS)) + ticket_groups((int)((S + SC_COLS - 1) / SC_COLS));
+  o += al256((size_t)w.ticket_lines * SB_TICKET_STRIDE * 4);
   w.bytes = o;
   return w;
 }
@@ -1523,11 +1563,10 @@
   const int T = tile_w * tile_h, S = g.sw * g.sh, nc = n_chunks_of(N);
   hipLaunchKernelGGL(sb_count_kernel, dim3(nc), dim3(SC_BLOCK), count_lds_bytes(g), s, N, chunk_rounds(N),
                      reinterpret_cast<const int2*>(tile_rects), reinterpret_cast<const unsigned long long*>(tile_masks), tile_w,
-                     tile_h, count_band_rows(g), w.table_t, w.table_s, w.area_part);
+                     tile_h, count_band_rows(g), w.table_t, w.table_s, w.area_part, w.tickets, w.ticket_lines);
   const int wg_t = (T + SC_COLS - 1) / SC_COLS, wg_s = (S + SC_COLS - 1) / SC_COLS;
   hipLaunchKernelGGL(sb_columns_kernel, dim3(wg_t + wg_s), dim3(SB_BLOCK), 0, s, T, S, nc, wg_t, w.table_t, w.table_s,
-                     tile_offsets, w.st_offsets);
-  hipLaunchKernelGGL(sb_offsets_kernel, dim3(2), dim3(SO_BLOCK), 0, s, T, S, tile_offsets, w.st_offsets, count_out, w.area_part, nc);
+                     tile_offsets, w.st_offsets, w.tickets, count_out, w.area_part);
   FG_RETURN_IF_LAUNCH_FAILED();
   return FG_OK;
 }
@@ -1582,7 +1621,7 @@
   if (N <= 0 || capacity <= 0 || tile_w <= 0 || tile_h <= 0) return FG_ERR_INVALID_ARG;
   if (!depth_keys || !tile_rects || !tile_offsets || !count_workspace || !flatten_ids || !list_offsets || !workspace)
     return FG_ERR_INVALID_ARG;
-  if (flags & ~(FG_STBIN_LONG_SEGMENTS | FG_STBIN_TEST_SMALL_SLABS)) return FG_ERR_INVALID_ARG;
+  if (flags & ~(FG_STBIN_LONG_SEGMENTS | FG_STBIN_TEST_SMALL_SLABS | FG_STBIN_NO_LARGE_SORT)) return FG_ERR_INVALID_ARG;
   if (!fg_stbin_supported(N, tile_w, tile_h)) return FG_ERR_UNSUPPORTED;
   if (workspace_bytes < fg_stbin_fill_workspace_bytes(capacity)) return FG_ERR_WORKSPACE;
   hipStream_t s = fg_hip_stream(stream);
@@ -1632,14 +1671,15 @@
                        long_mode, fw.lt.chunk_seg, fw.lt.bucket_seg, 0, fgjobs::JobBuild{}, fw.lt.over_list);
   }
   if (want_jobs) hipLaunchKernelGGL(sb_build_jobs_kernel, dim3(fgjobs::FG_JOB_BLOCKS), dim3(1024), 0, s, *jobs, tile_offsets);
-  if (!long_mode)
+  if (!long_mode && !(flags & FG_STBIN_NO_LARGE_SORT))
     hipLaunchKernelGGL(sb_sort_large_kernel, dim3(S < SB_LARGE_GRID ? S : SB_LARGE_GRID), dim3(64 * SB_LARGE_WAVES), 0, s,
                        tile_w, tile_h, tile_offsets, w.st_offsets, w.large_list, w.long_list, fw.lt, entries, scratch,
                        (long long)capacity, flatten_ids);
   hipLaunchKernelGGL(sb_sort_small_kernel, dim3(S + (bwd_jobs_in_sort ? 8 : 0)), dim3(64 * SB_SMALL_WAVES), 0, s, tile_w, tile_h,
                      tile_offsets, w.st_offsets, entries, scratch, (long long)capacity, flatten_ids, list_offsets,
                      long_mode ? fw.lt.over_list : nullptr, bwd_jobs_in_sort ? 8 : 0,
-                     bwd_jobs_in_sort ? *jobs : fgjobs::JobBuild{}, w.long_list, fw.lt);
+                     bwd_jobs_in_sort ? *jobs : fgjobs::JobBuild{}, w.long_list, fw.lt,
+                     !long_mode && (flags & FG_STBIN_NO_LARGE_SORT) ? 1 : 0);
   const int slab_limit = (flags & FG_STBIN_TEST_SMALL_SLABS) ? LG_T + 64 : SB_LONG_SLAB;
   if (long_mode) {
     hipLaunchKernelGGL(sb_long_scatter_kernel, dim3(LG_GRID), dim3(LG_BLOCK), 0, s, tile_offsets, T, (long long)capacity,
diff --git a/freegaussian_amd/csrc/step.hip b/freegaussian_amd/csrc/step.hip
--- a/freegaussian_amd/csrc/step.hip
+++ b/freegaussian_amd/csrc/step.hip
@@ -118,7 +118,7 @@
   float* seg_ckpt = at<float>(keep, L, FG_STEP_SEG_CKPT);
   rc = fg_stbin_fill_jobs(N, depth_keys, tile_rects, tile_masks, tile_w, tile_h, d->capacity, tile_offsets, count_ws, flatten_ids,
                           list_offsets, at<char>(tmp, L, FG_STEP_FILL_WS), (size_t)L->nbytes[FG_STEP_FILL_WS], W, H, 16, jobs,
-                          jobs + L->jobs_words, seg_ckpt != nullptr, config, d->flags & (FG_STBIN_LONG_SEGMENTS | FG_STBIN_TEST_SMALL_SLABS), io->ckpt_need_out,
+                          jobs + L->jobs_words, seg_ckpt != nullptr, config, d->flags & (FG_STBIN_LONG_SEGMENTS | FG_STBIN_TEST_SMALL_SLABS | FG_STBIN_NO_LARGE_SORT), io->ckpt_need_out,
                           stream);
   if (rc != FG_OK) return rc;
   float* v_splats = at<float>(keep, L, FG_STEP_V_SPLATS);
diff --git a/freegaussian_amd/ops.py b/freegaussian_amd/ops.py
--- a/freegaussian_amd/ops.py
+++ b/freegaussian_amd/ops.py
@@ -139,6 +139,10 @@
         self.long_shapes = {}
         self.long_calls = 0
         self.test_small_slabs = False
+        self.skip_large_sort = e.get("FG_SKIP_LARGE_SORT", "1") != "0"
+        self.large_clean_calls = 8
+        self.large_clean = {}
+        self.large_redos = 0
         self.heavy_tiles = e.get("FG_HEAVY_TILES", "auto")
         if self.heavy_tiles not in ("auto", "always", "never"):
             raise ValueError(f"FG_HEAVY_TILES={self.heavy_tiles!r}: auto | always | never")
@@ -1517,6 +1521,8 @@
         heavy = rctx.heavy_tiles == "always" or (rctx.heavy_tiles == "auto" and rctx.heavy_shapes.get(lkey, 0) > 0)
         capacity = rctx.capacity_for(ckey, N)
         masked = rctx.masks_on(lkey)
+        no_large = (rctx.skip_large_sort and not long_mode and rctx.large_clean.get(lkey, 0) >= rctx.large_clean_calls
+                    and not (dev.type == "cuda" and torch.cuda.is_current_stream_capturing()))
         while True:
             seg_slots = rctx.seg_slots_for(lkey, capacity, tile_w * tile_h, N) if channels == 3 and want_backward else 0
             cfgp, variant = rctx.cfg_variant(heavy, seg_slots, rctx.even_shape(lkey), rctx.uneven_shape(lkey), rctx.heavy_lens(lkey)[1])
@@ -1524,7 +1530,7 @@
             key = (dev, N, width, height, int(raw), sh_degree, k_stored, n_color, int(with_depth), n_extra, int(antialiased),
                    n_clamp, int(want_backward), int(shares),
                    ((_lib.STBIN_LONG_SEGMENTS | (_lib.STBIN_TEST_SMALL_SLABS if rctx.test_small_slabs else 0)) if long_mode else 0)
-                   | (0 if masked else _lib.STEP_NO_FOOTPRINT_MASKS), capacity, eps2d,
+                   | (0 if masked else _lib.STEP_NO_FOOTPRINT_MASKS) | (_lib.STBIN_NO_LARGE_SORT if no_large else 0), capacity, eps2d,
                    near, far, radius_clip, variant, bytes(rctx.policy))
             d, L, rc = _step_plan(key, cfgp)
             _lib.check(rc, "fg_step_layout_query")
@@ -1533,6 +1539,8 @@
                 rctx.plan_changes += 1
                 for name, i in (("N", 1), ("shares", 13), ("long_mode", 14), ("capacity", 15), ("variant", 20)):
                     if last[i] != key[i]:
+                        if i == 14 and (last[i] ^ key[i]) == _lib.STBIN_NO_LARGE_SORT:
+                            name = "large_sort"
                         rctx.plan_change_reasons[name] = rctx.plan_change_reasons.get(name, 0) + 1
             rctx._last_plan[lkey] = key
             keep = rctx.workspace("keep", (L.keep_bytes + 3) >> 2, torch.float32, dev)
@@ -1574,10 +1582,19 @@
             splats = view(k32, "splats", (N, SPLAT_FLOATS), (SPLAT_FLOATS, 1))
             list_offsets = view(i32, "list_offsets", (tile_w * tile_h + 1,), (1,))
             n_isects = _note_counts(rctx, lkey, ckey, count_slot, shares, N, walks=shares, masked=masked)
-            if n_isects <= capacity:
+            n_over = _poll_count(count_slot, 3)
+            if len(rctx.large_clean) > 256 and lkey not in rctx.large_clean:
+                rctx.large_clean.pop(next(iter(rctx.large_clean)))
+            rctx.large_clean[lkey] = min(rctx.large_clean.get(lkey, 0) + 1, 1 << 20) if n_over == 0 else 0
+            wrong_guess = no_large and n_over > 0
+            if wrong_guess:
+                rctx.large_redos += 1
+                no_large = False
+            if n_isects <= capacity and not wrong_guess:
                 break
-            rctx.capacity_redos += 1
-            capacity = max(n_isects, 1)
+            if n_isects > capacity:
+                rctx.capacity_redos += 1
+                capacity = max(n_isects, 1)
         flatten_ids = view(i32, "flatten_ids", (n_isects,), (1,))
         ctx.save_for_backward(means, quats, d_quats, scales, d_scales, opacities, colors, features_rest, extra, viewmat, K,
                               background, keep)
diff --git a/include/fgraster.h b/include/fgraster.h
--- a/include/fgraster.h
+++ b/include/fgraster.h
@@ -79,6 +79,7 @@
 size_t fg_stbin_fill_workspace_bytes(int64_t capacity);
 #define FG_STBIN_LONG_SEGMENTS 1
 #define FG_STEP_NO_FOOTPRINT_MASKS 2
+#define FG_STBIN_NO_LARGE_SORT 8
 #define FG_STBIN_TEST_SMALL_SLABS 4
 int fg_stbin_fill(int N, const uint32_t* depth_keys, const int32_t* tile_rects, const uint64_t* tile_masks, int tile_w,
                   int tile_h, int64_t capacity, const int32_t* tile_offsets, const void* count_workspace,
```

After: 2779 Mpix/s, median of 6. Within noise of the previous version (+0.4%).
